# Stability-AI/stable-audio-tools

Measured on AMD Instinct MI355X. Metric: train-step samples/sec (47s@44.1kHz), higher is better.
Workload: dtype f32(bf16x3)

## Files before the change

### include/sat_amd.h

```cpp
#ifndef SAT_AMD_H
#define SAT_AMD_H

#ifdef __cplusplus
extern "C" {
#endif

int sat_abi_version(void);
int sat_is_simulator(void);
const char* sat_last_error(void);


int sat_conv1d(const float* x, const float* w_packed, const float* bias, const float* alpha, const float* beta,
               const float* res, float* y, const float* x2, const float* alpha2, const float* beta2,
               float* part_da, float* part_db, int B, int Cin, int Cout, int Tin, int Tout, int K, int stride,
               int dil, int pad, int tanh_out, void* stream);
int sat_conv1d_partial_rows(int B, int Tout);

int sat_conv1d_bf16x3(const float* x, const short* w_hi, const short* w_lo, const float* bias, const float* snake_a,
                      const float* snake_ib, const float* res, float* y, const float* x2, const float* alpha2,
                      const float* beta2, float* part_da, float* part_db, int B, int Cin, int Cout, int Tin, int Tout,
                      int K, int stride, int dil, int pad, int tanh_out, void* stream);
int sat_conv1d_bf16x3_emit(const float* x, const short* w_hi, const short* w_lo, const float* bias, const float* snake_a,
                      const float* snake_ib, const float* res, float* y, const float* x2, const float* alpha2,
                      const float* beta2, float* part_da, float* part_db, int B, int Cin, int Cout, int Tin, int Tout,
                      int K, int stride, int dil, int pad, int tanh_out, void* em_hi, void* em_lo,
                           const float* em_a, const float* em_ib, int em_rows, void* stream);
int sat_residual_unit_fwd(const short* xp_hi, const short* xp_lo, int rows, const short* w7_hi, const short* w7_lo,
                          const float* bias1, const float* a2, const float* ib2, const short* w1_hi, const short* w1_lo,
                          const float* bias2, const float* x, float* h, float* y, int B, int C, int T, int K, int dil, int pad,
                          void* em_hi, void* em_lo, const float* em_a, const float* em_ib, int em_rows, void* stream);
int sat_convtr1d_bf16x3(const float* x, const short* w_hi, const short* w_lo, const float* bias, const float* snake_a,
                        const float* snake_ib, const float* res, float* y, const float* x2, const float* alpha2,
                        const float* beta2, float* part_da, float* part_db, int B, int Cin, int Cout, int Tin, int Tout,
                        int K, int stride, int pad, int tanh_out, void* stream);
int sat_conv1d_bf16x3_partial_rows(int B, int Tout, int K, int stride);

int sat_rows_pack(const float* x, float* buf, int B, int C, int T, int W, int kh, int dil_t, int pad_t, int pad_w, int pitch, int lead,
                  void* stream);
int sat_rows_pack_bwd(const float* dbuf, float* dx, int B, int C, int T, int W, int kh, int dil_t, int pad_t, int pad_w, int pitch,
                      int lead, void* stream);
int sat_rows_unpack(const float* y, float* out, int B, int C, int T, int W, int pad_w, int pitch, float slope, void* stream);
int sat_rows_unpack_bwd(const float* dout, const float* out, float* dy, int B, int C, int T, int W, int pad_w, int pitch, float slope,
                        void* stream);

int sat_disc_geom(int frames, int W, int* P, int* L, int* lead, int* rows);
int sat_disc_planes(const float* src, const float* out, const signed char* fm_sign, const float* fm_coef, float* dst, void* hi, void* lo, int B,
                    int C, int frames, int W, int pitched, float slope, void* stream);
int sat_disc_l1_blocks(void);
int sat_disc_l1_sum(const float* a, const float* b, float* partial, signed char* sign, long long n, void* stream);
long long sat_disc_pack_size(int Cout, int Cin, int kh, int kw, int mode);
int sat_disc_pack_weights(const float* w, short* wq, int Cout, int Cin, int kh, int kw, int mode, void* stream);
int sat_disc_conv(const void* xp_hi, const void* xp_lo, const void* wq, const float* bias, float* y, void* em_hi,
                  void* em_lo, int B, int Cin, int Cout, int frames, int W, int kh, int kw, int dil_t, float slope, const float* lk_src,
                  float lk_slope, void* stream);
int sat_disc_wgrad_nsplit(int B, int M, int Cin, int kh, int frames, int W);
int sat_disc_wgrad(const float* dy, const float* x, float* partial, int B, int M, int Cin, int frames, int W, int kh, int kw, int dil_t,
                   void* stream);

int sat_conv1d_k7_plane_rows(int Tin, int Tout, int pad);
int sat_conv1d_k7_planes(const float* x, const float* snake_a, const float* snake_ib, short* xp_hi, short* xp_lo, int B, int Cin, int Tin,
                         int rows, void* stream);
long long sat_pack_weights_k7q_size(int D0, int D1, int K, int mode);
int sat_pack_weights_k7q(const float* w, short* hi, short* lo, int D0, int D1, int K, int mode, void* stream);
int sat_conv1d_bf16x3_planesq(const short* xp_hi, const short* xp_lo, int rows, const short* w_hi, const short* w_lo, const float* bias,
                             const float* res, float* y, const float* x2, const float* alpha2, const float* beta2, float* part_da,
                             float* part_db, int B, int Cin, int Cout, int Tin, int Tout, int K, int dil, int pad, int tanh_out,
                             int flags, void* stream);
int sat_convtr1d_bf16x3_partial_rows(int B, int Tout, int stride, int pad);
int sat_pack_weights_bf16x3(const float* w, short* hi, short* lo, int D0, int D1, int K, int stride, int mode, void* stream);
long long sat_pack_weights_bf16x3_size(int D0, int D1, int K, int stride, int mode);
int sat_snake_consts(const float* alpha, const float* beta, float* a, float* ib, int C, void* stream);

int sat_convtr1d(const float* x, const float* w_packed, const float* bias, const float* alpha, const float* beta,
                 const float* res, float* y, const float* x2, const float* alpha2, const float* beta2,
                 float* part_da, float* part_db, int B, int Cin, int Cout, int Tin, int Tout, int K, int stride,
                 int pad, int tanh_out, void* stream);
int sat_convtr1d_partial_rows(int B, int Tout, int stride, int pad);

int sat_conv_wgrad(const float* lo, const float* hi, const float* alpha, const float* beta, int snake_on,
                   float* partial, long long so_m, long long so_n, long long so_k, int B, int M, int N, int Tlo,
                   int Thi, int K, int stride, int dil, int pad, void* stream);
int sat_conv_wgrad_nsplit(int B, int M, int N, int Tlo, int K, int stride, int dil);

int sat_conv_wgrad7_bf16x3(const float* dy, const float* x, const float* alpha, const float* beta, float* partial,
                           long long so_m, long long so_n, long long so_k, int B, int M, int N, int T, int dil, int pad,
                           float* dy_rowsum, void* stream);
int sat_conv_wgrad7_bf16x3_nsplit(int B, int M, int N, int T);
int sat_conv_wgrad7_bf16x3_fuses_rowsum(int B, int M, int N, int T);

int sat_conv_wgrad7_planes_ok(int B, int M, int N, int T, int dil, int pad, int rows_dy, int rows_act);
int sat_conv_wgrad7_planes_nsplit(int B, int M, int N, int T);
int sat_conv_wgrad7_planes(const short* dy_hi, const short* dy_lo, int rows_dy, const short* act_hi, const short* act_lo, int rows_act,
                           float* partial, long long so_m, long long so_n, long long so_k, int B, int M, int N, int T, int dil, int pad,
                           void* stream);
int sat_lds_read_tr16_probe(const short* image, const int* lane_off, short* out, void* stream);

int sat_conv_wgrad_bf16x3(const float* lo, const float* hi, const float* alpha, const float* beta, int snake_on,
                          float* partial, long long so_m, long long so_n, long long so_k, int B, int M, int N, int Tlo,
                          int Thi, int K, int stride, int pad, float* lo_rowsum, void* stream);
int sat_conv_wgrad_bf16x3_nsplit(int B, int M, int N, int Tlo, int K, int stride);

int sat_ru_k1_bwd_nsplit(int B, int C, int T);
int sat_ru_k1_pack(const float* w, short* hi, short* lo, int C, void* stream);
int sat_ru_k1_bwd(const float* dy, const float* h, const short* wt_hi, const short* wt_lo, const float* alpha2, const float* beta2,
                  float* dh, short* em_hi, short* em_lo, int em_rows, float* dw_partial, float* part, int B, int C, int T,
                  void* stream);

int sat_reduce_splits(const float* partial, float* out, long long count, int nsplit, float scale, int accumulate,
                      void* stream);
int sat_rowsum(const float* x, float* partial, int B, int C, int T, void* stream);
int sat_rowsum_nsplit(int T);

int sat_wn_fold(const float* v, const float* g, float* w, float* norm, int D0, int R, void* stream);
int sat_wn_grad(const float* v, const float* g, const float* norm, const float* dw, float* dv, float* dg, int D0,
                int R, void* stream);
int sat_wn_grad_splits(const float* partial, int nsplit, long long count, long long so_m, long long so_n, long long so_k,
                       const float* v, const float* g, const float* norm, float* dv, float* dg, int D0, int N, int K,
                       const float* bias_partial, int bias_cols, float* dbias, void* stream);
int sat_edge_conv_ok(int cin, int cout, int k, int stride, int dil, int pad);
int sat_edge_conv_partial_rows(int B, int T);
int sat_edge_conv(const float* x, const float* w, const float* bias, const float* alpha, const float* beta, float* y, const float* x2,
                  const float* alpha2, const float* beta2, float* part_da, float* part_db, short* em_hi, short* em_lo,
                  const float* em_alpha, const float* em_beta, int em_rows, int B, int Cin, int Cout, int T, int K, int pad, int mode,
                  int tanh_out, void* stream);
int sat_edge_conv_wgrad_nsplit(int B, int M, int N, int T);
int sat_edge_conv_wgrad(const float* dy, const float* x, const float* alpha, const float* beta, float* partial, float* rowsum, int B,
                        int M, int N, int T, int K, int pad, void* stream);
int sat_pack_weights(const float* w, float* out, int D0, int D1, int K, int S, int mode, void* stream);

int sat_vae_nblocks(long long n);
int sat_vae_sample_fwd(const float* pre, const float* noise, float* z, float* kl_partial, int B, int C, int T,
                       void* stream);
int sat_vae_sample_bwd(const float* pre, const float* noise, const float* dz, const float* dkl, float* dpre, int B,
                       int C, int T, void* stream);

int sat_fir(const float* x, const float* taps, float* y, int N, int T, int ntaps, int adjoint, void* stream);
int sat_stft_tiles(int n_fft, int hop, int T);
int sat_stft_fwd(const float* x, const float* y, const float* views, float* partial, int NI, int C, int T, int NV,
                 int n_fft, int hop, void* stream);
int sat_stft_bwd(const float* x, const float* y, const float* views, const float* coef, float* dy, int NI, int C,
                 int T, int NV, int n_fft, int hop, int wrt_x, void* stream);

int sat_adamw_step(float* p, const float* g, float* m, float* v, long long n, float lr, float beta1, float beta2,
                   float eps, float weight_decay, int step, float grad_scale, float* ema, float ema_decay,
                   void* stream);
int sat_adamw_step_dev(float* p, const float* g, float* m, float* v, long long n, const float* hyper, float beta1, float beta2,
                       float eps, float weight_decay, float* ema, void* stream);

int sat_multi_copy(const void* entries, int nent, void* stream);

int sat_allreduce_available(void);
int sat_allreduce_unique_id(void* id128);
int sat_allreduce_init(const void* id128, int world, int rank, void** comm);
int sat_allreduce_bucket(void* comm, void* buf, long long count, int dtype, int mode, void* stream);
int sat_allreduce_finalize(void* comm);

int sat_attn_prepare(const void* src, long long sb, long long sh, long long sn, short* rm_hi, short* rm_lo,
                     short* tr_hi, short* tr_lo, int B, int H, int N, int Np, int dtype, void* stream);
int sat_attention_fwd(const short* q_hi, const short* q_lo, const short* k_hi, const short* k_lo, const short* vt_hi,
                      const short* vt_lo, void* o, float* lse, int B, int H, int Hkv, int Nq, int Nk, int Nqp, int Nkp,
                      int head_dim, float scale, int dtype, void* stream);
int sat_attention_rowdot(const void* dout, const void* out, float* dsum, int B, int H, int Nq, int dtype, void* stream);
int sat_attention_bwd(const short* const* planes, const float* lse, const float* dsum, void* dq, void* dk, void* dv,
                      int B, int H, int Hkv, int Nq, int Nk, int Nqp, int Nkp, int head_dim, float scale, int dtype,
                      void* stream);
int sat_attention_cross_ok(int H, int Hkv, int Nk, int head_dim, int dtype);
int sat_attention_cross_fwd(const short* q_rm, const short* k_rm, const short* v_tr, void* o, float* lse, int B, int H, int Hkv,
                            int Nq, int Nk, int Nqp, int Nkp, int head_dim, float scale, void* stream);
long long sat_attention_cross_bwd_ws(int B, int H, int Hkv, int Nq, int Nk);
int sat_attention_cross_bwd(const short* const* planes, const float* lse, const float* dsum, void* dq, void* dk, void* dv,
                            void* ws, long long ws_bytes, int B, int H, int Hkv, int Nq, int Nk, int Nqp, int Nkp, int head_dim,
                            float scale, void* stream);

int sat_layernorm_fwd(const void* x, const float* gamma, const float* beta, const void* scale, const void* shift,
                      long long mod_stride, void* y, float* mean, float* rstd, int rows, int D, int rows_per_batch,
                      float eps, int dtype, void* stream);
int sat_layernorm_fwd_fp8(const void* x, const float* gamma, const float* beta, const void* scale, const void* shift,
                          long long mod_stride, void* q, float* qscale, int rows, int D, int rows_per_batch, float eps,
                          int dtype, void* stream);
int sat_layernorm_bwd_nblocks(int rows, int rows_per_batch);
int sat_layernorm_bwd(const void* dy, const void* x, const float* gamma, const float* beta, const void* scale,
                      long long mod_stride, const float* mean, const float* rstd, void* dx, float* part, int rows, int D,
                      int rows_per_batch, int dtype, void* stream);
int sat_layernorm_bwd_res(const void* dy, const void* x, const float* gamma, const float* beta, const void* scale,
                          long long mod_stride, const float* mean, const float* rstd, const void* dres, void* dx, float* part,
                          int rows, int D, int rows_per_batch, int dtype, void* stream);

int sat_rope_tables(const float* inv_freq, float* cs, int N, int half, float pos_scale, void* stream);
int sat_rope_apply(void* t, const float* cs, long long sb, long long sn, long long sh, int B, int N, int H, int half,
                   int tab_off, int transpose, int dtype, void* stream);

int sat_qk_norm_fwd(const void* x, long long xs, void* y, long long ys, const float* q_gamma, const float* q_beta,
                    const float* k_gamma, const float* k_beta, const float* cs, int tab_off, float* stat, int tokens, int ntok,
                    int nh, int hq, int mode, float eps, int dtype, void* stream);
int sat_qk_norm_bwd_nblocks(long long rows);
int sat_qk_norm_bwd(void* dy, long long ys, const void* x, long long xs, const float* q_gamma, const float* k_gamma,
                    const float* cs, int tab_off, const float* stat, float* part, int tokens, int ntok, int nh, int hq,
                    int mode, int dtype, void* stream);

int sat_swiglu(const void* xin, const void* dout, void* out, long long rows, int F, int backward, int dtype,
               void* stream);
int sat_gate_residual(const void* x, const void* gate, long long gstride, const void* res, void* y, int B, int N, int D,
                      int dtype, void* stream);
int sat_gate_residual_bwd_nchunks(int N);
int sat_gate_residual_bwd(const void* dy, const void* x, const void* gate, long long gstride, void* dx, float* part,
                          int B, int N, int D, int dtype, void* stream);

int sat_cfg_step(const void* out2, const void* x, void* y0, void* y1, int B, int C, int T, int ncond, float scale,
                 float phi, float c0x, float c0v, float c1x, float c1v, int dtype, void* stream);
int sat_sampler_step(const void* out2, const void* x, const void* prev, void* y0, void* y1, int B, int C, int T, int ncond,
                     float scale, float phi, const float* coef, int dtype, void* stream);
int sat_sampler_step_dev(const void* out2, const void* x, const void* prev, void* y0, void* y1, int B, int C, int T, int ncond,
                         float scale, float phi, const float* coef, int dtype, void* stream);
int sat_spec_frames(int n_fft, int hop, int T);
int sat_spec_fwd(const float* x, float* z, int NI, int C, int T, int n_fft, int hop, void* stream);
int sat_spec_bwd(const float* dz, float* dx, int NI, int C, int T, int n_fft, int hop, void* stream);


int sat_gemm_bf16(const void* A, long long lda, const void* B, long long ldb, void* C, long long ldc, const float* bias,
                  const void* res, long long ldr, const void* gate, long long ldg, int rows_per_gate, void* pre,
                  long long ldp, const void* zeros, int M, int N, int K, int epilogue, int out_f32, int splits, int tile,
                  void* stream);

int sat_gemm_qkv_bf16(const void* A, long long lda, const void* B, long long ldb, const float* rope_cs, int rope_off,
                      void* q_rm, void* k_rm, void* v_tr, const void* zeros, int nb, int ntok, int npad, int heads,
                      int K, int sec0, int nsec, int tile, void* stream);
int sat_gemm_qkv_norm_bf16(const void* A, long long lda, const void* B, long long ldb, const float* rope_cs, int rope_off,
                           void* q_rm, void* k_rm, void* v_tr, const void* zeros, int nb, int ntok, int npad, int heads,
                           int K, int sec0, int nsec, int tile, int mode, const float* q_gamma, const float* q_beta,
                           const float* k_gamma, const float* k_beta, float eps, void* stream);

int sat_splitk_epilogue(const float* slabs, int S, const float* bias, const void* res, long long ldr, void* out, long long ldo,
                        int M, int N, int out_f32, void* stream);

int sat_gemm_fp8(const void* A, long long lda, const void* B, long long ldb, void* C, long long ldc, const float* bias,
                 const void* res, long long ldr, const void* gate, long long ldg, int rows_per_gate, void* pre,
                 long long ldp, const void* zeros, const float* alpha, const float* row_alpha, const float* col_alpha, int M, int N,
                 int K, int epilogue, int out_f32, int tile, void* stream);
int sat_gemm_qkv_fp8(const void* A, long long lda, const void* B, long long ldb, const float* rope_cs, int rope_off,
                     void* q_rm, void* k_rm, void* v_tr, const void* zeros, const float* alpha, const float* row_alpha,
                     const float* col_alpha, int nb, int ntok, int npad, int heads, int K, int sec0, int nsec, int tile, void* stream);
int sat_absmax_scale_blocks(int R, int C);
int sat_absmax_scale(const void* src, long long lds, float* work, float* scales, int R, int C, int src_f32, void* stream);
int sat_quant_fp8(const void* src, long long lds, void* dst, long long ldd, const float* qscale, int R, int C, int src_f32,
                  void* stream);
int sat_quant_fp8_rows(const void* src, long long lds, void* dst, long long ldd, float* scale, int R, int C, int src_f32,
                       void* stream);

int sat_cast_bf16(const void* src, long long lds, void* dst, long long ldd, int R, int C, int Rpad, int src_f32,
                  int transpose, void* stream);
int sat_cast_bf16_tpair(const void* src_a, long long lds_a, void* dst_a, long long ldd_a, int Ra, int Ca, int Rpad_a, int a_f32,
                        const void* src_b, long long lds_b, void* dst_b, long long ldd_b, int Rb, int Cb, int Rpad_b, int b_f32,
                        void* stream);
int sat_cast_bf16_dual(const void* src, long long lds, void* dst, long long ldd, void* dst_t, long long ldd_t, int R, int C, int Rpad,
                       int src_f32, void* stream);

int sat_split_bf16x3(const float* src, long long lds, void* dst, long long ldd, int R, int C, int side, void* stream);

#ifdef __cplusplus
}
#endif
#endif
```

### stable_audio_tools_amd/_lib.py

```python
import ctypes
import os

_P = ctypes.c_void_p
_I = ctypes.c_int
_L = ctypes.c_longlong
_F = ctypes.c_float

SIGNATURES = {
    "sat_abi_version": (_I, []),
    "sat_is_simulator": (_I, []),
    "sat_last_error": (ctypes.c_char_p, []),
    "sat_conv1d": (_I, [_P] * 12 + [_I] * 10 + [_P]),
    "sat_conv1d_partial_rows": (_I, [_I, _I]),
    "sat_conv1d_bf16x3": (_I, [_P] * 13 + [_I] * 10 + [_P]),
    "sat_conv1d_bf16x3_emit": (_I, [_P] * 13 + [_I] * 10 + [_P] * 4 + [_I, _P]),
    "sat_convtr1d_bf16x3": (_I, [_P] * 13 + [_I] * 9 + [_P]),
    "sat_conv1d_bf16x3_partial_rows": (_I, [_I] * 4),
    "sat_rows_pack": (_I, [_P, _P] + [_I] * 10 + [_P]),
    "sat_rows_pack_bwd": (_I, [_P, _P] + [_I] * 10 + [_P]),
    "sat_rows_unpack": (_I, [_P, _P] + [_I] * 6 + [_F, _P]),
    "sat_rows_unpack_bwd": (_I, [_P, _P, _P] + [_I] * 6 + [_F, _P]),
    "sat_disc_geom": (_I, [_I, _I, _P, _P, _P, _P]),
    "sat_disc_planes": (_I, [_P] * 7 + [_I] * 5 + [_F, _P]),
    "sat_disc_l1_blocks": (_I, []),
    "sat_disc_l1_sum": (_I, [_P, _P, _P, _P, _L, _P]),
    "sat_disc_pack_size": (_L, [_I] * 5),
    "sat_disc_pack_weights": (_I, [_P] * 2 + [_I] * 5 + [_P]),
    "sat_disc_conv": (_I, [_P] * 7 + [_I] * 8 + [_F, _P, _F, _P]),
    "sat_disc_wgrad_nsplit": (_I, [_I] * 6),
    "sat_disc_wgrad": (_I, [_P] * 3 + [_I] * 8 + [_P]),
    "sat_conv1d_k7_plane_rows": (_I, [_I] * 3),
    "sat_conv1d_k7_planes": (_I, [_P] * 5 + [_I] * 4 + [_P]),
    "sat_conv1d_bf16x3_planesq": (_I, [_P, _P, _I] + [_P] * 10 + [_I] * 10 + [_P]),
    "sat_pack_weights_k7q": (_I, [_P, _P, _P, _I, _I, _I, _I, _P]),
    "sat_residual_unit_fwd": (_I, [_P, _P, _I] + [_P] * 11 + [_I] * 6 + [_P] * 4 + [_I, _P]),
    "sat_pack_weights_k7q_size": (_L, [_I, _I, _I, _I]),
    "sat_convtr1d_bf16x3_partial_rows": (_I, [_I] * 4),
    "sat_pack_weights_bf16x3": (_I, [_P, _P, _P, _I, _I, _I, _I, _I, _P]),
    "sat_pack_weights_bf16x3_size": (_L, [_I, _I, _I, _I, _I]),
    "sat_snake_consts": (_I, [_P, _P, _P, _P, _I, _P]),
    "sat_conv_wgrad7_bf16x3": (_I, [_P] * 5 + [_L] * 3 + [_I] * 6 + [_P, _P]),
    "sat_conv_wgrad7_bf16x3_nsplit": (_I, [_I] * 4),
    "sat_conv_wgrad7_bf16x3_fuses_rowsum": (_I, [_I] * 4),
    "sat_conv_wgrad7_planes_ok": (_I, [_I] * 8),
    "sat_conv_wgrad7_planes_nsplit": (_I, [_I] * 4),
    "sat_conv_wgrad7_planes": (_I, [_P, _P, _I, _P, _P, _I, _P] + [_L] * 3 + [_I] * 6 + [_P]),
    "sat_lds_read_tr16_probe": (_I, [_P] * 4),
    "sat_conv_wgrad_bf16x3": (_I, [_P] * 4 + [_I, _P] + [_L] * 3 + [_I] * 8 + [_P, _P]),
    "sat_conv_wgrad_bf16x3_nsplit": (_I, [_I] * 6),
    "sat_convtr1d": (_I, [_P] * 12 + [_I] * 9 + [_P]),
    "sat_convtr1d_partial_rows": (_I, [_I, _I, _I, _I]),
    "sat_conv_wgrad": (_I, [_P, _P, _P, _P, _I, _P, _L, _L, _L] + [_I] * 9 + [_P]),
    "sat_conv_wgrad_nsplit": (_I, [_I] * 7),
    "sat_reduce_splits": (_I, [_P, _P, _L, _I, _F, _I, _P]),
    "sat_ru_k1_bwd_nsplit": (_I, [_I] * 3),
    "sat_ru_k1_pack": (_I, [_P, _P, _P, _I, _P]),
    "sat_ru_k1_bwd": (_I, [_P] * 9 + [_I, _P, _P, _I, _I, _I, _P]),
    "sat_rowsum": (_I, [_P, _P, _I, _I, _I, _P]),
    "sat_rowsum_nsplit": (_I, [_I]),
    "sat_wn_fold": (_I, [_P, _P, _P, _P, _I, _I, _P]),
    "sat_wn_grad": (_I, [_P, _P, _P, _P, _P, _P, _I, _I, _P]),
    "sat_wn_grad_splits": (_I, [_P, _I, _L, _L, _L, _L, _P, _P, _P, _P, _P, _I, _I, _I, _P, _I, _P, _P]),
    "sat_pack_weights": (_I, [_P, _P, _I, _I, _I, _I, _I, _P]),
    "sat_vae_nblocks": (_I, [_L]),
    "sat_vae_sample_fwd": (_I, [_P, _P, _P, _P, _I, _I, _I, _P]),
    "sat_vae_sample_bwd": (_I, [_P, _P, _P, _P, _P, _I, _I, _I, _P]),
    "sat_multi_copy": (_I, [_P, _I, _P]),
    "sat_adamw_step": (_I, [_P, _P, _P, _P, _L, _F, _F, _F, _F, _F, _I, _F, _P, _F, _P]),
    "sat_adamw_step_dev": (_I, [_P, _P, _P, _P, _L, _P, _F, _F, _F, _F, _P, _P]),
    "sat_allreduce_available": (_I, []),
    "sat_allreduce_unique_id": (_I, [_P]),
    "sat_allreduce_init": (_I, [_P, _I, _I, _P]),
    "sat_allreduce_bucket": (_I, [_P, _P, _L, _I, _I, _P]),
    "sat_allreduce_finalize": (_I, [_P]),
    "sat_fir": (_I, [_P, _P, _P, _I, _I, _I, _I, _P]),
    "sat_stft_tiles": (_I, [_I, _I, _I]),
    "sat_stft_fwd": (_I, [_P, _P, _P, _P, _I, _I, _I, _I, _I, _I, _P]),
    "sat_stft_bwd": (_I, [_P, _P, _P, _P, _P, _I, _I, _I, _I, _I, _I, _I, _P]),
    "sat_spec_frames": (_I, [_I, _I, _I]),
    "sat_spec_fwd": (_I, [_P, _P, _I, _I, _I, _I, _I, _P]),
    "sat_spec_bwd": (_I, [_P, _P, _I, _I, _I, _I, _I, _P]),
    "sat_attn_prepare": (_I, [_P, _L, _L, _L, _P, _P, _P, _P, _I, _I, _I, _I, _I, _P]),
    "sat_attention_fwd": (_I, [_P] * 8 + [_I] * 8 + [_F, _I, _P]),
    "sat_attention_rowdot": (_I, [_P, _P, _P, _I, _I, _I, _I, _P]),
    "sat_attention_bwd": (_I, [_P] * 6 + [_I] * 8 + [_F, _I, _P]),
    "sat_edge_conv_ok": (_I, [_I] * 6),
    "sat_edge_conv_partial_rows": (_I, [_I] * 2),
    "sat_edge_conv": (_I, [_P] * 15 + [_I] * 9 + [_P]),
    "sat_edge_conv_wgrad_nsplit": (_I, [_I] * 4),
    "sat_edge_conv_wgrad": (_I, [_P] * 6 + [_I] * 6 + [_P]),
    "sat_attention_cross_ok": (_I, [_I] * 5),
    "sat_attention_cross_fwd": (_I, [_P] * 5 + [_I] * 8 + [_F, _P]),
    "sat_attention_cross_bwd_ws": (_L, [_I] * 5),
    "sat_attention_cross_bwd": (_I, [_P] * 7 + [_L] + [_I] * 8 + [_F, _P]),
    "sat_gemm_bf16": (_I, [_P, _L, _P, _L, _P, _L, _P, _P, _L, _P, _L, _I, _P, _L, _P] + [_I] * 7 + [_P]),
    "sat_gemm_qkv_bf16": (_I, [_P, _L, _P, _L, _P, _I, _P, _P, _P, _P] + [_I] * 8 + [_P]),
    "sat_gemm_qkv_norm_bf16": (_I, [_P, _L, _P, _L, _P, _I, _P, _P, _P, _P] + [_I] * 9 + [_P] * 4 + [_F, _P]),
    "sat_gemm_fp8": (_I, [_P, _L, _P, _L, _P, _L, _P, _P, _L, _P, _L, _I, _P, _L, _P, _P, _P, _P] + [_I] * 6 + [_P]),
    "sat_gemm_qkv_fp8": (_I, [_P, _L, _P, _L, _P, _I, _P, _P, _P, _P, _P, _P, _P] + [_I] * 8 + [_P]),
    "sat_quant_fp8": (_I, [_P, _L, _P, _L, _P, _I, _I, _I, _P]),
    "sat_quant_fp8_rows": (_I, [_P, _L, _P, _L, _P, _I, _I, _I, _P]),
    "sat_absmax_scale": (_I, [_P, _L, _P, _P, _I, _I, _I, _P]),
    "sat_absmax_scale_blocks": (_I, [_I, _I]),
    "sat_splitk_epilogue": (_I, [_P, _I, _P, _P, _L, _P, _L, _I, _I, _I, _P]),
    "sat_cast_bf16": (_I, [_P, _L, _P, _L, _I, _I, _I, _I, _I, _P]),
    "sat_cast_bf16_tpair": (_I, [_P, _L, _P, _L, _I, _I, _I, _I, _P, _L, _P, _L, _I, _I, _I, _I, _P]),
    "sat_cast_bf16_dual": (_I, [_P, _L, _P, _L, _P, _L, _I, _I, _I, _I, _P]),
    "sat_split_bf16x3": (_I, [_P, _L, _P, _L, _I, _I, _I, _P]),
    "sat_layernorm_fwd": (_I, [_P] * 5 + [_L] + [_P] * 3 + [_I] * 3 + [_F, _I, _P]),
    "sat_layernorm_fwd_fp8": (_I, [_P] * 5 + [_L] + [_P] * 2 + [_I] * 3 + [_F, _I, _P]),
    "sat_layernorm_bwd_nblocks": (_I, [_I, _I]),
    "sat_layernorm_bwd": (_I, [_P] * 5 + [_L] + [_P] * 4 + [_I] * 4 + [_P]),
    "sat_layernorm_bwd_res": (_I, [_P] * 5 + [_L] + [_P] * 5 + [_I] * 4 + [_P]),
    "sat_rope_tables": (_I, [_P, _P, _I, _I, _F, _P]),
    "sat_rope_apply": (_I, [_P, _P, _L, _L, _L] + [_I] * 7 + [_P]),
    "sat_qk_norm_fwd": (_I, [_P, _L, _P, _L, _P, _P, _P, _P, _P, _I, _P] + [_I] * 5 + [_F, _I, _P]),
    "sat_qk_norm_bwd_nblocks": (_I, [_L]),
    "sat_qk_norm_bwd": (_I, [_P, _L, _P, _L, _P, _P, _P, _I, _P, _P] + [_I] * 6 + [_P]),
    "sat_swiglu": (_I, [_P, _P, _P, _L, _I, _I, _I, _P]),
    "sat_gate_residual": (_I, [_P, _P, _L, _P, _P, _I, _I, _I, _I, _P]),
    "sat_gate_residual_bwd_nchunks": (_I, [_I]),
    "sat_cfg_step": (_I, [_P, _P, _P, _P, _I, _I, _I, _I, _F, _F, _F, _F, _F, _F, _I, _P]),
    "sat_sampler_step": (_I, [_P, _P, _P, _P, _P, _I, _I, _I, _I, _F, _F, _P, _I, _P]),
    "sat_sampler_step_dev": (_I, [_P, _P, _P, _P, _P, _I, _I, _I, _I, _F, _F, _P, _I, _P]),
    "sat_gate_residual_bwd": (_I, [_P, _P, _P, _L, _P, _P, _I, _I, _I, _I, _P]),
}

LIB_PATH = os.path.join(os.path.dirname(os.path.abspath(__file__)), "csrc", "libsat_amd.so")


def bind(cdll):
    for name, (res, args) in SIGNATURES.items():
        fn = getattr(cdll, name)
        fn.restype = res
        fn.argtypes = args
    return cdll


_lib = None


def load():
    global _lib
    if _lib is not None:
        return _lib
    if not os.path.exists(LIB_PATH):
        raise RuntimeError(
            f"stable_audio_tools_amd: HIP library not built: {LIB_PATH} is missing. "
            "Run `python -c 'import __graft_entry__ as g; g.build()'` (hipcc --offload-arch=gfx950). "
            "There is no CPU fallback.")
    try:
        cdll = ctypes.CDLL(LIB_PATH)
    except OSError as e:
        raise RuntimeError(f"stable_audio_tools_amd: cannot load {LIB_PATH}: {e}. There is no CPU fallback.") from e
    bind(cdll)
    if cdll.sat_is_simulator():
        raise RuntimeError("stable_audio_tools_amd: refusing to use a simulator build as the product library")
    _lib = cdll
    return _lib
```

### stable_audio_tools_amd/autoencoders.py

```python
import copy
import math

import torch
from torch import nn
from torch.nn.utils.weight_norm import WeightNorm as _TorchWeightNorm

from . import functional as Fn
from .bottleneck import VAEBottleneck


class SnakeBeta(nn.Module):

    def __init__(self, in_features, alpha=1.0, alpha_trainable=True, alpha_logscale=True):
        super().__init__()
        if not alpha_logscale:
            raise NotImplementedError("only alpha_logscale=True (the reference default used by Oobleck) is implemented")
        self.in_features = in_features
        self.alpha_logscale = alpha_logscale
        self.alpha = nn.Parameter(torch.zeros(in_features) * alpha)
        self.beta = nn.Parameter(torch.zeros(in_features) * alpha)
        self.alpha.requires_grad = alpha_trainable
        self.beta.requires_grad = alpha_trainable
        self.no_div_by_zero = 0.000000001

    def forward(self, x):
        c = x.shape[1]
        eye = torch.eye(c, device=x.device, dtype=x.dtype).unsqueeze(-1)
        a, b = (self.alpha, self.beta) if self.alpha.dtype == torch.float32 else (self.alpha.detach().float(), self.beta.detach().float())
        return Fn.SnakeConv1dFn.apply(x, a, b, eye, None, None, 1, 1, 0, False)


class _NativeWeightNorm(_TorchWeightNorm):

    def __init__(self, name="weight", dim=0):
        super().__init__(name, dim)

    def compute_weight(self, module):
        return module._fold_host()

    def remove(self, module):
        if not module.is_folded:
            module._to_folded(module._fold_host().detach())

    def __call__(self, module, inputs):
        return None


def _inference_pass(*tensors):
    return (not torch.is_grad_enabled()) or not any(t is not None and t.requires_grad for t in tensors)


class _WNConvBase(nn.Module):

    transposed = False

    def __init__(self, in_channels, out_channels, kernel_size, stride=1, padding=0, dilation=1, bias=True):
        super().__init__()
        self.in_channels, self.out_channels = in_channels, out_channels
        self.kernel_size, self.stride, self.padding, self.dilation = kernel_size, stride, padding, dilation
        if self.transposed:
            wshape = (in_channels, out_channels, kernel_size)
        else:
            wshape = (out_channels, in_channels, kernel_size)
        v = torch.empty(wshape)
        nn.init.kaiming_uniform_(v, a=math.sqrt(5))
        self.weight_g = nn.Parameter(v.flatten(1).norm(dim=1).view(-1, 1, 1).clone())
        self.weight_v = nn.Parameter(v)
        if bias:
            fan_in = wshape[1] * kernel_size
            bound = 1.0 / math.sqrt(fan_in)
            self.bias = nn.Parameter(torch.empty(out_channels).uniform_(-bound, bound))
        else:
            self.register_parameter("bias", None)
        self.register_forward_pre_hook(_NativeWeightNorm("weight", 0))
        self.__dict__["_derived"] = Fn.DerivedCache()

    @property
    def is_folded(self):
        return "weight" in self._parameters

    def __getattr__(self, name):
        if name == "weight" and "weight_v" in self.__dict__.get("_parameters", ()):
            return self._fold_host()
        return super().__getattr__(name)

    def __deepcopy__(self, memo):
        cls = self.__class__
        new = cls.__new__(cls)
        memo[id(self)] = new
        for k, v in self.__dict__.items():
            new.__dict__[k] = Fn.DerivedCache() if k == "_derived" else copy.deepcopy(v, memo)
        return new

    def _fold_host(self):
        v, g = self._parameters["weight_v"], self._parameters["weight_g"]
        return v * (g / v.flatten(1).norm(dim=1).view(-1, 1, 1))

    def _to_folded(self, w):
        rg = self._parameters["weight_v"].requires_grad
        del self._parameters["weight_g"], self._parameters["weight_v"]
        self._parameters["weight"] = nn.Parameter(w.clone(), requires_grad=rg)

    def _load_from_state_dict(self, state_dict, prefix, local_metadata, strict, missing_keys, unexpected_keys, error_msgs):
        kw, kg, kv = prefix + "weight", prefix + "weight_g", prefix + "weight_v"
        if not self.is_folded and kw in state_dict and kv not in state_dict:
            self._to_folded(torch.empty_like(self._parameters["weight_v"]))
        elif self.is_folded and kw not in state_dict and kv in state_dict and kg in state_dict:
            v, g = state_dict.pop(kv), state_dict.pop(kg)
            state_dict[kw] = v * (g / v.flatten(1).norm(dim=1).view(-1, 1, 1))
        super()._load_from_state_dict(state_dict, prefix, local_metadata, strict, missing_keys, unexpected_keys, error_msgs)

    def p32(self, name, t):
        if t is None or t.dtype == torch.float32:
            return t
        if t.requires_grad and torch.is_grad_enabled():
            raise NotImplementedError("16-bit parameters are inference-only on the HIP conv stack (freeze the model: AutoencoderPretransform does)")
        return self._derived.get("f32/" + name, (t,), lambda: t.detach().float())

    def bias32(self):
        return self.p32("bias", self.bias)

    def folded_weight(self):
        if self.is_folded:
            return self.p32("weight", self._parameters["weight"])
        v, g = self.p32("weight_v", self.weight_v), self.p32("weight_g", self.weight_g)
        if _inference_pass(v, g):
            return self._derived.get("folded", (v, g), lambda: Fn.WeightNormFn.apply(v.detach(), g.detach()))
        return Fn.WeightNormFn.apply(v, g)

    def weight_args(self):
        if not self.is_folded and Fn._ops(None).wn_fused:
            v, g = self.p32("weight_v", self.weight_v), self.p32("weight_g", self.weight_g)
            if not _inference_pass(v, g):
                return v, g
        return self.folded_weight(), None

    def derived_cache(self, *others):
        ps = list(self._parameters.values()) + list(others)
        return self._derived if _inference_pass(*ps) else None


class WNConv1d(_WNConvBase):
    def forward(self, x, snake=None, res=None, tanh_out=False, next_snake=None):
        a, b = (self.p32("alpha", snake.alpha), self.p32("beta", snake.beta)) if snake is not None else (None, None)
        if next_snake is not None and next_snake[0].dtype != torch.float32:
            next_snake = (self.p32("next_alpha", next_snake[0]), self.p32("next_beta", next_snake[1]), next_snake[2])
        w, g = self.weight_args()
        return Fn.SnakeConv1dFn.apply(x, a, b, w, self.bias32(), res, self.stride, self.dilation,
                                      self.padding, tanh_out, None, self.derived_cache(a, b), next_snake, g)


class WNConvTranspose1d(_WNConvBase):
    transposed = True

    def forward(self, x, snake=None):
        a, b = (self.p32("alpha", snake.alpha), self.p32("beta", snake.beta)) if snake is not None else (None, None)
        w, g = self.weight_args()
        return Fn.SnakeConvTr1dFn.apply(x, a, b, w, self.bias32(), self.stride, self.padding, None,
                                        self.derived_cache(a, b), g)


def _require_snake(use_snake, antialias_activation=False):
    if not use_snake:
        raise NotImplementedError("only use_snake=True (SnakeBeta, the Stable Audio Open / 2.0 VAE configuration) is "
                                  "implemented on the HIP path; the ELU variant is out of scope (SURVEY.md §8a V3)")
    if antialias_activation:
        raise NotImplementedError("antialias_activation (alias_free_torch) is out of scope")


class ResidualUnit(nn.Module):
    checkpointing = False
    fuse = None

    def __init__(self, in_channels, out_channels, dilation, use_snake=False, antialias_activation=False):
        super().__init__()
        _require_snake(use_snake, antialias_activation)
        self.dilation = dilation
        padding = (dilation * (7 - 1)) // 2
        self.layers = nn.Sequential(
            SnakeBeta(out_channels),
            WNConv1d(in_channels, out_channels, kernel_size=7, dilation=dilation, padding=padding),
            SnakeBeta(out_channels),
            WNConv1d(out_channels, out_channels, kernel_size=1),
        )

    def entry_snake(self):
        s1 = self.layers[0]
        return (s1.alpha, s1.beta, self.dilation)

    def forward(self, x, next_snake=None):
        s1, c1, s2, c2 = self.layers
        ca, cb = c1.derived_cache(s1.alpha, s1.beta), c2.derived_cache(s2.alpha, s2.beta)
        if next_snake is not None and next_snake[0].dtype != torch.float32:
            next_snake = (c2.p32("next_alpha", next_snake[0]), c2.p32("next_beta", next_snake[1]), next_snake[2])
        (w1, g1), (w2, g2) = c1.weight_args(), c2.weight_args()
        return Fn.ResidualUnitFn.apply(x, c1.p32("alpha", s1.alpha), c1.p32("beta", s1.beta), w1, c1.bias32(),
                                       c2.p32("alpha", s2.alpha), c2.p32("beta", s2.beta), w2, c2.bias32(), self.dilation, None,
                                       self.checkpointing and torch.is_grad_enabled(), (ca, cb) if ca is not None and cb is not None else None,
                                       next_snake, self.fuse if self.fuse is not None else ("nokeep" if not torch.is_grad_enabled() else False),
                                       g1, g2)


class EncoderBlock(nn.Module):
    def __init__(self, in_channels, out_channels, stride, use_snake=False, antialias_activation=False):
        super().__init__()
        _require_snake(use_snake, antialias_activation)
        self.layers = nn.Sequential(
            ResidualUnit(in_channels, in_channels, dilation=1, use_snake=use_snake),
            ResidualUnit(in_channels, in_channels, dilation=3, use_snake=use_snake),
            ResidualUnit(in_channels, in_channels, dilation=9, use_snake=use_snake),
            SnakeBeta(in_channels),
            WNConv1d(in_channels, out_channels, kernel_size=2 * stride, stride=stride, padding=math.ceil(stride / 2)),
        )

    def forward(self, x, next_snake=None):
        r1, r2, r3, snake, down = self.layers
        x = r1(x, next_snake=r2.entry_snake())
        x = r2(x, next_snake=r3.entry_snake())
        return down(r3(x), snake=snake, next_snake=next_snake)


class DecoderBlock(nn.Module):
    def __init__(self, in_channels, out_channels, stride, use_snake=False, antialias_activation=False,
                 use_nearest_upsample=False):
        super().__init__()
        _require_snake(use_snake, antialias_activation)
        if use_nearest_upsample:
            raise NotImplementedError("use_nearest_upsample is out of scope (no in-repo Oobleck config enables it)")
        self.layers = nn.Sequential(
            SnakeBeta(in_channels),
            WNConvTranspose1d(in_channels, out_channels, kernel_size=2 * stride, stride=stride,
                              padding=math.ceil(stride / 2)),
            ResidualUnit(out_channels, out_channels, dilation=1, use_snake=use_snake),
            ResidualUnit(out_channels, out_channels, dilation=3, use_snake=use_snake),
            ResidualUnit(out_channels, out_channels, dilation=9, use_snake=use_snake),
        )

    def forward(self, x):
        snake, up, r1, r2, r3 = self.layers
        x = r1(up(x, snake=snake), next_snake=r2.entry_snake())
        return r3(r2(x, next_snake=r3.entry_snake()))


class OobleckEncoder(nn.Module):
    def __init__(self, in_channels=2, channels=128, latent_dim=32, c_mults=[1, 2, 4, 8], strides=[2, 4, 8, 8],
                 use_snake=False, antialias_activation=False):
        super().__init__()
        _require_snake(use_snake, antialias_activation)
        self.in_channels = in_channels
        c_mults = [1] + list(c_mults)
        self.depth = len(c_mults)
        layers = [WNConv1d(in_channels, c_mults[0] * channels, kernel_size=7, padding=3)]
        for i in range(self.depth - 1):
            layers += [EncoderBlock(c_mults[i] * channels, c_mults[i + 1] * channels, stride=strides[i], use_snake=use_snake)]
        layers += [SnakeBeta(c_mults[-1] * channels),
                   WNConv1d(c_mults[-1] * channels, latent_dim, kernel_size=3, padding=1)]
        self.layers = nn.Sequential(*layers)

    def forward(self, x):
        mods = list(self.layers)
        blocks = mods[1:-2]
        x = mods[0](x, next_snake=blocks[0].layers[0].entry_snake() if blocks else None)
        for i, blk in enumerate(blocks):
            nxt = blocks[i + 1].layers[0].entry_snake() if i + 1 < len(blocks) else None
            x = blk(x, next_snake=nxt)
        return mods[-1](x, snake=mods[-2])


class OobleckDecoder(nn.Module):
    def __init__(self, out_channels=2, channels=128, latent_dim=32, c_mults=[1, 2, 4, 8], strides=[2, 4, 8, 8],
                 use_snake=False, antialias_activation=False, use_nearest_upsample=False, final_tanh=True):
        super().__init__()
        _require_snake(use_snake, antialias_activation)
        self.out_channels = out_channels
        c_mults = [1] + list(c_mults)
        self.depth = len(c_mults)
        layers = [WNConv1d(latent_dim, c_mults[-1] * channels, kernel_size=7, padding=3)]
        for i in range(self.depth - 1, 0, -1):
            layers += [DecoderBlock(c_mults[i] * channels, c_mults[i - 1] * channels, stride=strides[i - 1],
                                    use_snake=use_snake, antialias_activation=antialias_activation,
                                    use_nearest_upsample=use_nearest_upsample)]
        layers += [SnakeBeta(c_mults[0] * channels),
                   WNConv1d(c_mults[0] * channels, out_channels, kernel_size=7, padding=3, bias=False),
                   nn.Tanh() if final_tanh else nn.Identity()]
        self.final_tanh = final_tanh
        self.layers = nn.Sequential(*layers)

    def forward(self, x):
        mods = list(self.layers)
        x = mods[0](x)
        for blk in mods[1:-3]:
            x = blk(x)
        return mods[-2](x, snake=mods[-3], tanh_out=self.final_tanh)


class AudioAutoencoder(nn.Module):

    def __init__(self, encoder, decoder, latent_dim, downsampling_ratio, sample_rate, io_channels=2, bottleneck=None,
                 pretransform=None, in_channels=None, out_channels=None, soft_clip=False):
        super().__init__()
        if pretransform is not None:
            raise NotImplementedError("AudioAutoencoder(pretransform=...) is out of scope for the HIP path")
        self.downsampling_ratio = downsampling_ratio
        self.sample_rate = sample_rate
        self.latent_dim = latent_dim
        self.io_channels = io_channels
        self.in_channels = io_channels if in_channels is None else in_channels
        self.out_channels = io_channels if out_channels is None else out_channels
        self.min_length = self.downsampling_ratio
        self.bottleneck = bottleneck
        self.encoder = encoder
        self.decoder = decoder
        self.pretransform = None
        self.soft_clip = soft_clip
        self.is_discrete = self.bottleneck is not None and self.bottleneck.is_discrete

    def encode(self, audio, skip_bottleneck=False, return_info=False, skip_pretransform=False, iterate_batch=False, **kwargs):
        info = {}
        if iterate_batch:
            latents = torch.cat([self.encoder(audio[i:i + 1]) for i in range(audio.shape[0])], dim=0)
        else:
            latents = self.encoder(audio)
        info["pre_bottleneck_latents"] = latents
        if self.bottleneck is not None and not skip_bottleneck:
            latents, binfo = self.bottleneck.encode(latents, return_info=True, **kwargs)
            info.update(binfo)
        if return_info:
            return latents, info
        return latents

    def decode(self, latents, skip_bottleneck=False, iterate_batch=False, **kwargs):
        if self.bottleneck is not None and not skip_bottleneck:
            latents = self.bottleneck.decode(latents)
        if iterate_batch:
            decoded = torch.cat([self.decoder(latents[i:i + 1]) for i in range(latents.shape[0])], dim=0)
        else:
            decoded = self.decoder(latents, **kwargs)
        if self.soft_clip:
            decoded = torch.tanh(decoded)
        return decoded

    def encode_audio(self, audio, chunked=False, overlap=32, chunk_size=128, **kwargs):
        if not chunked:
            return self.encode(audio, **kwargs)
        r = int(self.downsampling_ratio)
        total = audio.shape[2]
        csz, hop = chunk_size * r, (chunk_size - overlap) * r
        starts = list(range(0, total - csz + 1, hop))
        if not starts:
            raise ValueError("chunked encode needs at least chunk_size latent frames of audio")
        if starts[-1] + csz != total:
            starts.append(total - csz)
        y_size = total // r
        out = torch.zeros((audio.shape[0], self.latent_dim, y_size), device=audio.device, dtype=audio.dtype)
        half = overlap // 2
        chunk_noise = kwargs.pop("noise", None)
        if isinstance(chunk_noise, (list, tuple)) and len(chunk_noise) != len(starts):
            raise ValueError(f"chunked encode: {len(starts)} chunks but {len(chunk_noise)} noise tensors")
        for i, s0 in enumerate(starts):
            if chunk_noise is not None:
                kwargs["noise"] = chunk_noise[i] if isinstance(chunk_noise, (list, tuple)) else chunk_noise
            y = self.encode(audio[:, :, s0:s0 + csz], **kwargs)
            last = i == len(starts) - 1
            t1 = y_size if last else i * hop // r + chunk_size
            t0 = t1 - y.shape[2] if last else i * hop // r
            k0, k1 = 0, y.shape[2]
            if i > 0:
                t0, k0 = t0 + half, k0 + half
            if not last:
                t1, k1 = t1 - half, k1 - half
            out[:, :, t0:t1] = y[:, :, k0:k1]
        return out

    def decode_audio(self, latents, chunked=False, overlap=32, chunk_size=128, **kwargs):
        if not chunked:
            return self.decode(latents, **kwargs)
        r = int(self.downsampling_ratio)
        out = torch.zeros((latents.shape[0], self.out_channels, latents.shape[2] * r), device=latents.device,
                          dtype=latents.dtype)
        for win in _chunk_windows(latents.shape[2], chunk_size, overlap):
            y = self.decode(latents[:, :, win.src0:win.src1])
            out[:, :, win.dst0 * r:win.dst1 * r] = y[:, :, win.keep0 * r:win.keep1 * r]
        return out


class _Win:
    __slots__ = ("src0", "src1", "dst0", "dst1", "keep0", "keep1")


def _chunk_windows(total, chunk, overlap):
    hop = chunk - overlap
    starts = list(range(0, total - chunk + 1, hop))
    if not starts:
        raise ValueError("chunked encode/decode needs at least chunk_size latent frames")
    if starts[-1] + chunk != total:
        starts.append(total - chunk)
    half = overlap // 2
    wins = []
    for n, s0 in enumerate(starts):
        w = _Win()
        last = n == len(starts) - 1
        w.src0, w.src1 = s0, s0 + chunk
        d0 = (total - chunk) if last else n * hop
        w.keep0 = half if n > 0 else 0
        w.keep1 = chunk if last else chunk - half
        w.dst0, w.dst1 = d0 + w.keep0, d0 + w.keep1
        wins.append(w)
    return wins


def create_encoder_from_config(cfg):
    if cfg.get("type") != "oobleck":
        raise NotImplementedError(f"encoder type {cfg.get('type')!r} is out of scope (only 'oobleck' is on the hot path)")
    enc = OobleckEncoder(**cfg["config"])
    if not cfg.get("requires_grad", True):
        for p in enc.parameters():
            p.requires_grad = False
    return enc


def create_decoder_from_config(cfg):
    if cfg.get("type") != "oobleck":
        raise NotImplementedError(f"decoder type {cfg.get('type')!r} is out of scope (only 'oobleck' is on the hot path)")
    dec = OobleckDecoder(**cfg["config"])
    if not cfg.get("requires_grad", True):
        for p in dec.parameters():
            p.requires_grad = False
    return dec


def create_autoencoder_from_config(config):
    ae = config["model"]
    if ae.get("pretransform") is not None:
        raise NotImplementedError("autoencoder-level pretransform is out of scope")
    encoder = create_encoder_from_config(ae["encoder"])
    decoder = create_decoder_from_config(ae["decoder"])
    bottleneck = None
    if ae.get("bottleneck") is not None:
        if ae["bottleneck"]["type"] != "vae":
# ... 7 lines not shown
```

### stable_audio_tools_amd/csrc/conv1d_bf16x3.hip

```cpp
#include "conv_common.h"
#include <type_traits>

#define SAT_K7P_LEAD_ROWS 32
#define SAT_BF_AROWS1 192
#define SAT_BF_AROWSN 136

struct SatConvBfLaunch {
    SatConvParams p;
    const short* w_hi;
    const short* w_lo;
    int cout_pad;
    int cin_v, cout_v;
    int sin_log2;
    int sout_log2;
    int in_shift, out_shift;
    int nq;
    const short* xp_hi = nullptr;
    const short* xp_lo = nullptr;
    int xp_rows = 0, xp_c8 = 0;
    int wq = 0;
    int stagger = 0;
    int persist = 0;
    int dma_in_mfma = 0;
    short* em_hi = nullptr;
    short* em_lo = nullptr;
    const float* em_a = nullptr;
    const float* em_ib = nullptr;
    int em_rows = 0, em_c8 = 0;
    const short* ru_w1_hi = nullptr;
    const short* ru_w1_lo = nullptr;
    const float* ru_bias2 = nullptr;
    const float* ru_a2 = nullptr;
    const float* ru_ib2 = nullptr;
    float* ru_h = nullptr;
};

SAT_DEVICE void sat_split2(float x, short* hi, short* lo) {
    const short h = sat_f32_to_bf16(x);
    *hi = h;
    *lo = sat_f32_to_bf16(x - sat_bf16_to_f32(h));
}

template <int NG, int CS, bool GATHER>
__global__ void __launch_bounds__(256)
#if !defined(SAT_HIPEMU)
__attribute__((amdgpu_waves_per_eu(NG == 4 ? 3 : 2)))
#endif
sat_conv1d_bf16x3_kernel(SatConvBfLaunch a) {
    constexpr int KT = NG / CS;
    constexpr int KROW = NG * 8 + 8;
    constexpr int AROWS = (CS == 1) ? SAT_BF_AROWS1 : SAT_BF_AROWSN;
    constexpr int WPS = 4 / CS;
    constexpr int NU = (CS == 1) ? 1 : 128 / (64 * WPS);
    const SatConvParams& p = a.p;
    constexpr int W_BYTES = 2 * SAT_CO_T * KROW * 2, A_BYTES = 2 * CS * AROWS * 8 * 2, T_BYTES = 4 * 32 * 68 * 4;
    constexpr int POOL = (W_BYTES + A_BYTES) > T_BYTES ? (W_BYTES + A_BYTES) : T_BYTES;
    __shared__ __attribute__((aligned(16))) char lds_pool[POOL];
    short (*w_lds)[SAT_CO_T][KROW] = reinterpret_cast<short (*)[SAT_CO_T][KROW]>(lds_pool);
    short (*a_lds)[CS][AROWS][8] = reinterpret_cast<short (*)[CS][AROWS][8]>(lds_pool + W_BYTES);
    __shared__ float red_lds[2][2][SAT_CO_T];
    __shared__ float ep_lds[5][SAT_CO_T];
    constexpr int SN_MAX = (NG == 4) ? 1024 : 2048;
    __shared__ float sn_lds[2][SN_MAX];

    const int tid = threadIdx.x;
    const int lane = tid & 63, wave = tid >> 6;
    const int l31 = lane & 31, hi = lane >> 5;
    int co_tile, win;
    sat_xcd_tile(blockIdx.x + gridDim.x * (blockIdx.y + gridDim.y * blockIdx.z), gridDim.y, gridDim.x * gridDim.z, &co_tile, &win);
    const int b = win / (int)gridDim.x, t_tile = win - b * (int)gridDim.x;
    const int t0 = t_tile * SAT_T_T;
    const int co0 = co_tile * SAT_CO_T;
    const int co_w = (wave >> 1) * 64, t_w = (wave & 1) * 64;
    const int K = p.K, dil = p.dil;
    const int nrows = SAT_T_T + (K - 1) * dil;
    const int q_in0 = t0 - p.pad;
    const int si = GATHER ? a.sin_log2 : 0, so = a.sout_log2;
    const int smask_i = (1 << si) - 1, smask_o = (1 << so) - 1;
    const float* xb = p.x + (size_t)b * p.Cin * p.Tin;
    const bool wave_on = (co0 + co_w) < a.cout_v;
    const bool mi1_on = (co0 + co_w + 32) < a.cout_v;
    const bool has_snake = p.alpha != nullptr;

    f32x16 acc[2][2];
#pragma unroll
    for (int i = 0; i < 2; ++i)
#pragma unroll
        for (int j = 0; j < 2; ++j)
#pragma unroll
            for (int r = 0; r < 16; ++r) acc[i][j][r] = 0.0f;

    if (tid < SAT_CO_T) {
        const int m = co0 + tid;
        const bool ok = m < a.cout_v;
        const int co = m >> so;
        ep_lds[0][tid] = (ok && p.bias) ? p.bias[co] : 0.0f;
        ep_lds[1][tid] = (ok && p.x2) ? expf(p.alpha2[co]) : 1.0f;
        ep_lds[2][tid] = (ok && p.x2) ? expf(p.beta2[co]) : 1.0f;
        ep_lds[3][tid] = (ok && a.em_a) ? a.em_a[co] : 0.0f;
        ep_lds[4][tid] = (ok && a.em_a) ? a.em_ib[co] : 0.0f;
    }
    if (has_snake) {
        const int nsn = p.Cin < SN_MAX ? p.Cin : SN_MAX;
        for (int i = tid; i < nsn; i += 256) {
            sn_lds[0][i] = p.alpha[i];
            sn_lds[1][i] = p.beta[i];
        }
    }
    __syncthreads();

    const int nchunks = (a.cin_v + 8 * CS - 1) / (8 * CS);
    const int cs_w = SAT_UNIFORM(wave / WPS);
    const int row0 = (wave % WPS) * 64 + lane;
    const int nhalo = (CS > 1) ? (nrows - SAT_T_T) * 8 : 0;
    const bool halo_on = (CS > 1) && (wave % WPS) == 0 && lane < nhalo;
    const int h_row = SAT_T_T + (lane >> 3), h_e = lane & 7;
    constexpr bool DEEP = (NG == 8 && CS == 4);
    constexpr int NSET = DEEP ? 2 : 1;
    float av[NSET][NU][8];
    float hv[NSET];
    bf16x8 wv[NG];
#pragma unroll
    for (int s_ = 0; s_ < NSET; ++s_) hv[s_] = 0.0f;
    auto load_elem = [&](int v, int row, bool* okp) -> float {
        int ch = v >> si;
        ch = ch < p.Cin ? ch : p.Cin - 1;
        const int tin = ((q_in0 + row) << si) + (v & smask_i) - (GATHER ? a.in_shift : 0);
        const bool ok = (unsigned)tin < (unsigned)p.Tin;
        *okp = ok;
        return xb[(size_t)ch * p.Tin + (ok ? tin : 0)];
    };
    unsigned okm[NSET];
#pragma unroll
    for (int s_ = 0; s_ < NSET; ++s_) okm[s_] = 0u;
    auto issue_loads = [&](int c, auto set_c) {
        constexpr int ST = decltype(set_c)::value;
        const int v0 = (c * CS + cs_w) * 8;
        unsigned m = 0u;
#pragma unroll
        for (int u = 0; u < NU; ++u) {
            const int row = row0 + u * 64 * WPS;
            if (CS == 1 && row >= nrows) continue;
#pragma unroll
            for (int e = 0; e < 8; ++e) {
                bool ok;
                av[ST][u][e] = load_elem(v0 + e, row, &ok);
                m |= ok ? (1u << (u * 8 + e)) : 0u;
            }
        }
        static_assert(NU * 8 < 31, "the in-range flags of a staging set are one 32-bit mask (bit 31: the halo element)");
        if (CS > 1 && halo_on) {
            bool ok;
            hv[ST] = load_elem(v0 + h_e, h_row, &ok);
            m |= ok ? (1u << 31) : 0u;
        }
        okm[ST] = m;
    };
    auto issue_w = [&](int c) {
#pragma unroll
        for (int u = 0; u < NG; ++u) {
            const int idx = tid + u * 256;
            const int part = idx % NG, co = (idx / NG) & 127, pl = idx / (NG * 128);
            const short* src = (pl ? a.w_lo : a.w_hi) + (((size_t)c * a.cout_pad + co0 + co) * NG + part) * 8;
            wv[u] = *reinterpret_cast<const bf16x8*>(src);
        }
    };
    auto write_lds = [&](int c, auto set_c) {
        constexpr int ST = decltype(set_c)::value;
        const int v0 = (c * CS + cs_w) * 8;
        float sa[8], sib[8];
        if (has_snake) {
#pragma unroll
            for (int e = 0; e < 8; ++e) {
                int ch = (v0 + e) >> si;
                ch = ch < p.Cin ? ch : p.Cin - 1;
                sa[e] = sn_lds[0][ch];
                sib[e] = sn_lds[1][ch];
            }
        }
#pragma unroll
        for (int u = 0; u < NU; ++u) {
            const int row = row0 + u * 64 * WPS;
            if (CS == 1 && row >= nrows) continue;
            uint32_t ph[4], pl[4];
#pragma unroll
            for (int e = 0; e < 8; e += 2) {
                float o0 = (okm[ST] >> (u * 8 + e)) & 1u ? av[ST][u][e] : 0.0f, o1 = (okm[ST] >> (u * 8 + e + 1)) & 1u ? av[ST][u][e + 1] : 0.0f;
                if (has_snake) {
                    o0 = sat_snake(o0, sa[e], sib[e]);
                    o1 = sat_snake(o1, sa[e + 1], sib[e + 1]);
                }
                sat_split2_pk(o0, o1, &ph[e >> 1], &pl[e >> 1]);
            }
            *reinterpret_cast<u32x4*>(&a_lds[0][cs_w][row][0]) = u32x4{ph[0], ph[1], ph[2], ph[3]};
            *reinterpret_cast<u32x4*>(&a_lds[1][cs_w][row][0]) = u32x4{pl[0], pl[1], pl[2], pl[3]};
// ... 288 lines not shown
#pragma unroll
                for (int ni = 0; ni < 2; ++ni) {
                    const int q = t0 + t_w + ni * 32 + l31;
                    const int t = (q << so) + (m & smask_o) - a.out_shift;
                    const bool ok = m_ok && t >= 0 && t < p.Tout;
                    okb |= ok ? (1u << (2 * r + ni)) : 0u;
                    const size_t o = ((size_t)b * p.Cout + (ok ? co : 0)) * p.Tout + (ok ? t : 0);
                    xv[r][ni] = bwd ? p.x2[o] : 0.0f;
                    rv[r][ni] = p.res ? p.res[o] : 0.0f;
                }
            }
#pragma unroll
            for (int r = 0; r < 16; ++r) {
                const int col = co_w + mi * 32 + (r & 3) + 8 * (r >> 2) + 4 * hi;
                const int m = co0 + col;
                const int co = m >> so;
                const float bias = ep_lds[0][col];
                const float a2 = ep_lds[1][col], b2 = ep_lds[2][col];
                float pda = 0.f, pdb = 0.f;
#pragma unroll
                for (int ni = 0; ni < 2; ++ni) {
                    const int q = t0 + t_w + ni * 32 + l31;
                    const int t = (q << so) + (m & smask_o) - a.out_shift;
                    const bool ok = (okb >> (2 * r + ni)) & 1u;
                    float v = acc[mi][ni][r] + bias;
                    if (bwd) {
                        const SatSnakeGrad g = sat_snake_grad(xv[r][ni], a2, b2);
                        pda += ok ? v * g.dla : 0.0f;
                        pdb += ok ? v * g.dlb : 0.0f;
                        v *= g.dx;
                    }
                    v += rv[r][ni];
                    if (p.tanh_out) v = tanhf(v);
                    if (ok) p.y[((size_t)b * p.Cout + co) * p.Tout + t] = v;
                }
                if (bwd) {
                    pda = sat_half_sum(pda);
                    pdb = sat_half_sum(pdb);
                    if (l31 == 0) {
                        red_lds[0][wave & 1][col] = pda;
                        red_lds[1][wave & 1][col] = pdb;
                    }
                }
            }
        }
    }
    if (bwd) {
        __syncthreads();
        const int m = co0 + tid;
        if (tid < SAT_CO_T && (tid & smask_o) == 0 && m < a.cout_v) {
            float sa = 0.f, sb = 0.f;
            for (int r = 0; r <= smask_o; ++r) {
                sa += red_lds[0][0][tid + r] + red_lds[0][1][tid + r];
                sb += red_lds[1][0][tid + r] + red_lds[1][1][tid + r];
            }
            const size_t row = (size_t)b * gridDim.x + t_tile;
            const size_t nrows_p = (size_t)p.B * gridDim.x;
            p.part_da[(size_t)(m >> so) * nrows_p + row] = sa;
            p.part_db[(size_t)(m >> so) * nrows_p + row] = sb;
        }
    }
}

struct SatBfPlan { int ng, cs, kv; };
static bool sat_bf_plan(int K, int stride, int mode, SatBfPlan* pl) {
    if (mode == 2 || stride > 1) {
        if (K != 2 * stride || (stride & (stride - 1)) || stride > 64) return false;
        *pl = SatBfPlan{8, 4, 2};
        return true;
    }
    if (stride != 1 || K < 1 || K > 8) return false;
    if (K == 1) *pl = SatBfPlan{4, 4, 1};
    else if (K == 2) *pl = SatBfPlan{8, 4, K};
    else if (K <= 4) *pl = SatBfPlan{8, 2, K};
    else *pl = SatBfPlan{8, 1, K};
    return true;
}
static int sat_log2i(int s) { int l = 0; while ((1 << l) < s) ++l; return l; }

struct SatPackBfParams {
    const float* w;
    short* hi;
    short* lo;
    int D0, D1, K, S, mode, ng, cs, kv, m_v, v_v, out_pad;
    long long total;
};
__global__ void __launch_bounds__(256) sat_pack_bf16x3_kernel(SatPackBfParams p) {
    const long long o = (long long)blockIdx.x * 256 + threadIdx.x;
    if (o >= p.total) return;
    const int e = (int)(o & 7);
    long long q = o >> 3;
    const int g = (int)(q % p.ng);
    q /= p.ng;
    const int m = (int)(q % p.out_pad), chunk = (int)(q / p.out_pad);
    const int kt = p.ng / p.cs;
    const int v = (chunk * p.cs + g / kt) * 8 + e, tap = g % kt;
    float val = 0.0f;
    if (tap < p.kv && m < p.m_v && v < p.v_v) {
        if (p.mode == 0) val = p.w[((size_t)m * p.D1 + v / p.S) * p.K + tap * p.S + v % p.S];
        else if (p.mode == 1) val = p.w[((size_t)v * p.D1 + m) * p.K + (p.K - 1 - tap)];
        else val = p.w[((size_t)v * p.D1 + m / p.S) * p.K + (m % p.S) + (tap == 0 ? p.S : 0)];
    }
    short h, l;
    sat_split2(val, &h, &l);
    p.hi[o] = h;
    p.lo[o] = l;
}

static bool sat_pack_bf_geometry(int D0, int D1, int K, int stride, int mode, SatPackBfParams* p) {
    SatBfPlan pl;
    if (mode < 0 || mode > 2 || D0 <= 0 || D1 <= 0 || !sat_bf_plan(K, stride, mode, &pl)) return false;
    if (mode == 1 && stride != 1) return false;
    p->D0 = D0; p->D1 = D1; p->K = K; p->S = stride; p->mode = mode;
    p->ng = pl.ng; p->cs = pl.cs; p->kv = pl.kv;
    if (mode == 0) { p->m_v = D0; p->v_v = D1 * stride; }
    else if (mode == 1) { p->m_v = D1; p->v_v = D0; }
    else { p->m_v = D1 * stride; p->v_v = D0; }
    p->out_pad = sat_cdiv(p->m_v, SAT_CO_T) * SAT_CO_T;
    p->total = (long long)sat_cdiv(p->v_v, 8 * pl.cs) * p->out_pad * pl.ng * 8;
    return true;
}
extern "C" long long sat_pack_weights_bf16x3_size(int D0, int D1, int K, int stride, int mode) {
    SatPackBfParams p{};
    return sat_pack_bf_geometry(D0, D1, K, stride, mode, &p) ? p.total : -1;
}
extern "C" int sat_pack_weights_bf16x3(const float* w, short* hi, short* lo, int D0, int D1, int K, int stride, int mode, void* stream) {
    SatPackBfParams p{};
    if (!sat_pack_bf_geometry(D0, D1, K, stride, mode, &p)) {
        sat_set_error("sat_pack_weights_bf16x3: needs stride 1 with K <= 8, or K == 2*stride with a power-of-two stride; mode 0|1|2");
        return 1;
    }
    p.w = w; p.hi = hi; p.lo = lo;
    SAT_LAUNCH(sat_pack_bf16x3_kernel, dim3((unsigned)sat_cdivll(p.total, 256)), dim3(256), stream, p);
    return sat_check_launch("sat_pack_weights_bf16x3");
}

struct SatSnakeConstParams { const float* alpha; const float* beta; float* a; float* ib; int C; };
__global__ void __launch_bounds__(256) sat_snake_consts_kernel(SatSnakeConstParams p) {
    const int i = blockIdx.x * 256 + threadIdx.x;
    if (i >= p.C) return;
    p.a[i] = expf(p.alpha[i]);
    p.ib[i] = 1.0f / (expf(p.beta[i]) + 1e-9f);
}
extern "C" int sat_snake_consts(const float* alpha, const float* beta, float* a, float* ib, int C, void* stream) {
    if (C <= 0) { sat_set_error("sat_snake_consts: empty"); return 1; }
    SatSnakeConstParams p{alpha, beta, a, ib, C};
    SAT_LAUNCH(sat_snake_consts_kernel, dim3(sat_cdiv(C, 256)), dim3(256), stream, p);
    return sat_check_launch("sat_snake_consts");
}

#include "conv1d_bf16x3_k7.h"
#include "conv1d_planes.h"
#include "conv1d_bf16x3_k7q.h"

static int sat_bf_launch(const char* what, SatConvBfLaunch& a, const SatBfPlan& pl, void* stream) {
    if (pl.ng == 8 && pl.cs == 1 && a.sin_log2 == 0 && a.sout_log2 == 0) {
        if (a.xp_hi && a.wq) sat_bf_launch_k7q(a, stream);
        else sat_bf_launch_k7(a, stream);
        return sat_check_launch(what);
    }
    if (a.p.alpha && a.p.Cin > ((pl.ng == 4) ? 1024 : 2048)) {
        sat_set_error("conv1d_bf16x3: an activated input of more than 2048 channels (1024 for K <= 4 at stride 1) is not served by the bf16x3 kernels (ops.use_bf16x3 = False takes the fp32-MFMA ones)");
        return 1;
    }
    dim3 grid(sat_cdiv(a.nq, SAT_T_T), a.cout_pad / SAT_CO_T, a.p.B);
    if (a.sin_log2 > 0) { SAT_LAUNCH((sat_conv1d_bf16x3_kernel<8, 4, true>), grid, dim3(256), stream, a); }
    else if (pl.ng == 8 && pl.cs == 1) { SAT_LAUNCH((sat_conv1d_bf16x3_kernel<8, 1, false>), grid, dim3(256), stream, a); }
    else if (pl.ng == 8 && pl.cs == 2) { SAT_LAUNCH((sat_conv1d_bf16x3_kernel<8, 2, false>), grid, dim3(256), stream, a); }
    else if (pl.ng == 8 && pl.cs == 4) { SAT_LAUNCH((sat_conv1d_bf16x3_kernel<8, 4, false>), grid, dim3(256), stream, a); }
    else { SAT_LAUNCH((sat_conv1d_bf16x3_kernel<4, 4, false>), grid, dim3(256), stream, a); }
    return sat_check_launch(what);
}

static int sat_conv1d_bf16x3_impl(const char* what, const float* x, const short* w_hi, const short* w_lo, const float* bias,
                                  const float* snake_a, const float* snake_ib, const float* res, float* y,
                                  const float* x2, const float* alpha2, const float* beta2, float* part_da,
                                  float* part_db, int B, int Cin, int Cout, int Tin, int Tout, int K, int stride, int dil,
                                  int pad, int tanh_out, short* em_hi, short* em_lo, const float* em_a, const float* em_ib, int em_rows,
                                  void* stream) {
    if (B <= 0 || Cin <= 0 || Cout <= 0 || Tin <= 0 || Tout <= 0) { sat_set_error("sat_conv1d_bf16x3: empty shape"); return 1; }
    SatBfPlan pl;
    if (!sat_bf_plan(K, stride, 0, &pl) || dil < 1 || (stride > 1 && dil != 1)) {
        sat_set_error("sat_conv1d_bf16x3: needs stride 1 with K <= 8, or K == 2*stride (power-of-two stride, dilation 1)");
        return 1;
    }
    if ((pl.kv - 1) * dil > (pl.cs == 1 ? 62 : SAT_BF_AROWSN - SAT_T_T)) { sat_set_error("sat_conv1d_bf16x3: receptive field too large for the LDS slab"); return 1; }
    if ((snake_a == nullptr) != (snake_ib == nullptr)) { sat_set_error("sat_conv1d_bf16x3: snake constants must both be given"); return 1; }
    if (x2 && (!alpha2 || !beta2 || !part_da || !part_db)) { sat_set_error("sat_conv1d_bf16x3: backward epilogue needs alpha2/beta2/partials"); return 1; }
    SatConvBfLaunch a;
    a.p = SatConvParams{x, nullptr, bias, snake_a, snake_ib, res, y, x2, alpha2, beta2, part_da, part_db,
                        B, Cin, Cout, Tin, Tout, pl.kv, 1, dil, stride == 1 ? pad : 0, tanh_out};
    a.w_hi = w_hi;
    a.w_lo = w_lo;
    a.cout_v = Cout;
    a.cout_pad = sat_cdiv(Cout, SAT_CO_T) * SAT_CO_T;
    a.cin_v = Cin * stride;
    a.sin_log2 = sat_log2i(stride);
    a.sout_log2 = 0;
    a.in_shift = stride == 1 ? 0 : pad;
    a.out_shift = 0;
    a.nq = Tout;
    if (em_hi) {
        const bool generic = !(pl.ng == 8 && pl.cs == 1);
        const bool vec4 = (Tout & 3) == 0 && (((uintptr_t)y | (uintptr_t)x2 | (uintptr_t)res) & 15) == 0;
        if (!generic || !vec4 || !em_lo || (em_a == nullptr) != (em_ib == nullptr) || em_rows < SAT_K7P_LEAD_ROWS + Tout ||
            (((uintptr_t)em_hi | (uintptr_t)em_lo) & 15)) {
            sat_set_error("sat_conv1d_bf16x3_emit: emission needs K <= 4 or a strided conv, Tout % 4 == 0, 16-byte aligned tensors, rows >= 32 + Tout");
            return 1;
        }
        a.em_hi = em_hi; a.em_lo = em_lo; a.em_a = em_a; a.em_ib = em_ib; a.em_rows = em_rows; a.em_c8 = sat_cdiv(Cout, 8);
    }
    return sat_bf_launch(what, a, pl, stream);
}
extern "C" int sat_conv1d_bf16x3(const float* x, const short* w_hi, const short* w_lo, const float* bias,
                                 const float* snake_a, const float* snake_ib, const float* res, float* y,
                                 const float* x2, const float* alpha2, const float* beta2, float* part_da,
                                 float* part_db, int B, int Cin, int Cout, int Tin, int Tout, int K, int stride, int dil,
                                 int pad, int tanh_out, void* stream) {
    return sat_conv1d_bf16x3_impl("sat_conv1d_bf16x3", x, w_hi, w_lo, bias, snake_a, snake_ib, res, y, x2, alpha2, beta2, part_da, part_db,
                                  B, Cin, Cout, Tin, Tout, K, stride, dil, pad, tanh_out, nullptr, nullptr, nullptr, nullptr, 0, stream);
}
extern "C" int sat_conv1d_bf16x3_emit(const float* x, const short* w_hi, const short* w_lo, const float* bias,
                                      const float* snake_a, const float* snake_ib, const float* res, float* y,
                                      const float* x2, const float* alpha2, const float* beta2, float* part_da,
                                      float* part_db, int B, int Cin, int Cout, int Tin, int Tout, int K, int stride, int dil,
                                      int pad, int tanh_out, void* em_hi, void* em_lo, const float* em_a, const float* em_ib, int em_rows,
                                      void* stream) {
    if (!em_hi) { sat_set_error("sat_conv1d_bf16x3_emit: planes missing"); return 1; }
    return sat_conv1d_bf16x3_impl("sat_conv1d_bf16x3_emit", x, w_hi, w_lo, bias, snake_a, snake_ib, res, y, x2, alpha2, beta2, part_da, part_db,
                                  B, Cin, Cout, Tin, Tout, K, stride, dil, pad, tanh_out, (short*)em_hi, (short*)em_lo, em_a, em_ib, em_rows, stream);
}

extern "C" int sat_conv1d_k7_plane_rows(int Tin, int Tout, int pad) {
    if (Tin <= 0 || Tout <= 0 || pad < 0 || pad > SAT_K7P_LEAD) return -1;
    const int need = sat_cdiv(Tout, SAT_K7_T) * SAT_K7_T - pad + SAT_K7_AROWS;
    const int body = need > Tin ? need : Tin;
    return SAT_K7P_LEAD + sat_cdiv(body, 64) * 64;
}
extern "C" int sat_conv1d_k7_planes(const float* x, const float* snake_a, const float* snake_ib, short* xp_hi, short* xp_lo, int B,
                                    int Cin, int Tin, int rows, void* stream) {
    if (B <= 0 || Cin <= 0 || Tin <= 0 || rows < SAT_K7P_LEAD + Tin) { sat_set_error("sat_conv1d_k7_planes: bad shape"); return 1; }
    if ((snake_a == nullptr) != (snake_ib == nullptr)) { sat_set_error("sat_conv1d_k7_planes: snake constants must both be given"); return 1; }
    SatK7PlaneParams p{x, snake_a, snake_ib, xp_hi, xp_lo, B, Cin, Tin, rows, sat_cdiv(Cin, 8)};
    SAT_LAUNCH(sat_k7_planes_kernel, dim3(sat_cdiv(rows, 256), p.c8, B), dim3(256), stream, p);
    return sat_check_launch("sat_conv1d_k7_planes");
}
extern "C" int sat_conv1d_bf16x3_planesq(const short* xp_hi, const short* xp_lo, int rows, const short* w_hi, const short* w_lo,
                                         const float* bias, const float* res, float* y, const float* x2, const float* alpha2,
                                         const float* beta2, float* part_da, float* part_db, int B, int Cin, int Cout, int Tin, int Tout,
                                         int K, int dil, int pad, int tanh_out, int flags, void* stream) {
    if (B <= 0 || Cin <= 0 || Cout <= 0 || Tin <= 0 || Tout <= 0) { sat_set_error("sat_conv1d_bf16x3_planesq: empty shape"); return 1; }
    if (K < 5 || K > SAT_K7Q_TAPS || dil < 1 || (K - 1) * dil > 62) {
        sat_set_error("sat_conv1d_bf16x3_planesq: needs stride 1, 5 <= K <= 7, (K-1)*dil <= 62");
        return 1;
    }
    if (rows < sat_conv1d_k7_plane_rows(Tin, Tout, pad)) { sat_set_error("sat_conv1d_bf16x3_planesq: rows must be >= sat_conv1d_k7_plane_rows(Tin, Tout, pad)"); return 1; }
    if (x2 && (!alpha2 || !beta2 || !part_da || !part_db)) { sat_set_error("sat_conv1d_bf16x3_planesq: backward epilogue needs alpha2/beta2/partials"); return 1; }
    SatConvBfLaunch a;
    a.p = SatConvParams{nullptr, nullptr, bias, nullptr, nullptr, res, y, x2, alpha2, beta2, part_da, part_db,
                        B, Cin, Cout, Tin, Tout, K, 1, dil, pad, tanh_out};
    a.w_hi = w_hi;
    a.w_lo = w_lo;
    a.cout_v = Cout;
    a.cout_pad = sat_cdiv(Cout, SAT_CO_T) * SAT_CO_T;
    a.cin_v = Cin;
    a.sin_log2 = 0;
    a.sout_log2 = 0;
    a.in_shift = 0;
    a.out_shift = 0;
    a.nq = Tout;
    a.xp_hi = xp_hi;
    a.xp_lo = xp_lo;
    a.xp_rows = rows;
    a.xp_c8 = sat_cdiv(Cin, 8);
    a.wq = 1;
    a.dma_in_mfma = (flags & 4) ? 1 : 0;
    a.persist = (flags & 1) ? 0 : ((flags & 2) ? 2 : 1);
    SatBfPlan pl{8, 1, K};
    return sat_bf_launch("sat_conv1d_bf16x3_planesq", a, pl, stream);
}

extern "C" int sat_residual_unit_fwd(const short* xp_hi, const short* xp_lo, int rows, const short* w7_hi, const short* w7_lo,
                                     const float* bias1, const float* a2, const float* ib2, const short* w1_hi, const short* w1_lo,
                                     const float* bias2, const float* x, float* h, float* y, int B, int C, int T, int K, int dil, int pad,
                                     void* em_hi, void* em_lo, const float* em_a, const float* em_ib, int em_rows, void* stream) {
    if (B <= 0 || C <= 0 || T <= 0 || C > SAT_K7_CO) { sat_set_error("sat_residual_unit_fwd: needs 1 <= C <= 128"); return 1; }
    if (K < 5 || K > SAT_K7Q_TAPS || dil < 1 || (K - 1) * dil > 62 || 2 * pad != (K - 1) * dil) {
        sat_set_error("sat_residual_unit_fwd: needs 5 <= K <= 7, (K-1)*dil <= 62, 'same' padding");
        return 1;
    }
    if (rows < sat_conv1d_k7_plane_rows(T, T, pad)) { sat_set_error("sat_residual_unit_fwd: rows must be >= sat_conv1d_k7_plane_rows(T, T, pad)"); return 1; }
    if (!xp_hi || !xp_lo || !w7_hi || !w7_lo || !w1_hi || !w1_lo || !a2 || !ib2 || !x || !y) { sat_set_error("sat_residual_unit_fwd: missing operand"); return 1; }
    if ((T & 3) || (((uintptr_t)y | (uintptr_t)x) & 15)) { sat_set_error("sat_residual_unit_fwd: T % 4 == 0 and 16-byte aligned x / y"); return 1; }
    SatConvBfLaunch a;
    a.p = SatConvParams{nullptr, nullptr, bias1, nullptr, nullptr, x, y, nullptr, nullptr, nullptr, nullptr, nullptr,
                        B, C, C, T, T, K, 1, dil, pad, 0};
    a.w_hi = w7_hi;
    a.w_lo = w7_lo;
    a.cout_v = C;
    a.cout_pad = SAT_CO_T;
    a.cin_v = C;
    a.sin_log2 = 0; a.sout_log2 = 0; a.in_shift = 0; a.out_shift = 0;
    a.nq = T;
    a.xp_hi = xp_hi; a.xp_lo = xp_lo; a.xp_rows = rows; a.xp_c8 = sat_cdiv(C, 8);
    a.wq = 1;
    a.ru_w1_hi = w1_hi; a.ru_w1_lo = w1_lo; a.ru_bias2 = bias2; a.ru_a2 = a2; a.ru_ib2 = ib2; a.ru_h = h;
// ... 47 lines not shown
```

### stable_audio_tools_amd/csrc/elementwise.hip

```cpp
#include "sat_device.h"

#include <string.h>

static thread_local char g_sat_err[512] = "";
void sat_set_error(const char* msg) {
    strncpy(g_sat_err, msg, sizeof(g_sat_err) - 1);
    g_sat_err[sizeof(g_sat_err) - 1] = 0;
}
int sat_check_launch(const char* what) {
    const auto e = hipGetLastError();
    if (e != hipSuccess) {
        char buf[512];
        snprintf(buf, sizeof(buf), "%s: kernel launch failed: %s", what, hipGetErrorString(e));
        sat_set_error(buf);
        return 2;
    }
    return 0;
}
extern "C" const char* sat_last_error() { return g_sat_err; }
#if defined(SAT_HIPEMU)
static int g_sat_emu_cus = 256;
extern "C" void sat_emu_set_cu_count(int n) { g_sat_emu_cus = n > 0 ? n : 256; }
#endif
int sat_cu_count() {
#if defined(SAT_HIPEMU)
    return g_sat_emu_cus;
#else
    static thread_local int dev_cached = -1, cus = 0;
    int dev = 0;
    if (hipGetDevice(&dev) != hipSuccess) return 256;
    if (dev != dev_cached) {
        int n = 0;
        if (hipDeviceGetAttribute(&n, hipDeviceAttributeMultiprocessorCount, dev) != hipSuccess || n <= 0) n = 256;
        cus = n;
        dev_cached = dev;
    }
    return cus;
#endif
}

extern "C" int sat_abi_version() { return 1; }
extern "C" int sat_is_simulator() {
#if defined(SAT_HIPEMU)
    return 1;
#else
    return 0;
#endif
}

struct SatWnParams {
    const float* v;
    const float* g;
    const float* dw;
    float* w;
    float* norm;
    float* dg;
    int D0, R;
};

SAT_DEVICE float sat_block_sum_256(float s, float* red) {
    s = sat_wave_sum(s);
    __syncthreads();
    if ((threadIdx.x & 63) == 0) red[threadIdx.x >> 6] = s;
    __syncthreads();
    return red[0] + red[1] + red[2] + red[3];
}

__global__ void __launch_bounds__(256) sat_wn_fold_kernel(SatWnParams p) {
    __shared__ float red[4];
    const int d = blockIdx.x;
    const float* v = p.v + (size_t)d * p.R;
    float s = 0.f;
    for (int i = threadIdx.x; i < p.R; i += 256) s += v[i] * v[i];
    s = sat_block_sum_256(s, red);
    const float nrm = sqrtf(s);
    const float sc = p.g[d] / nrm;
    float* w = p.w + (size_t)d * p.R;
    for (int i = threadIdx.x; i < p.R; i += 256) w[i] = v[i] * sc;
    if (threadIdx.x == 0) p.norm[d] = nrm;
}

__global__ void __launch_bounds__(256) sat_wn_grad_kernel(SatWnParams p) {
    __shared__ float red[4];
    const int d = blockIdx.x;
    const float* v = p.v + (size_t)d * p.R;
    const float* dw = p.dw + (size_t)d * p.R;
    float s = 0.f;
    for (int i = threadIdx.x; i < p.R; i += 256) s += v[i] * dw[i];
    s = sat_block_sum_256(s, red);
    const float nrm = p.norm[d];
    const float g = p.g[d];
    const float dgv = s / nrm;
    const float c1 = g / nrm, c2 = g * s / (nrm * nrm * nrm);
    float* dv = p.w + (size_t)d * p.R;
    for (int i = threadIdx.x; i < p.R; i += 256) dv[i] = c1 * dw[i] - c2 * v[i];
    if (threadIdx.x == 0) p.dg[d] = dgv;
}

#define SAT_WN_ROW_CAP 16384
struct SatWnSplitParams {
    const float* partial;
    const float* v;
    const float* g;
    const float* norm;
    float* dv;
    float* dg;
    long long count, so_m, so_n, so_k;
    int nsplit, D0, N, K;
    const float* bias_partial;
    float* dbias;
    int bias_cols;
};
#define SAT_WN_THREADS 1024
SAT_DEVICE float sat_wn_slab_sum(const float* base, long long count, int z0, int zstep, int nsplit) {
    float s0 = 0.f, s1 = 0.f, s2 = 0.f, s3 = 0.f;
    int z = z0;
    for (; z + 3 * zstep < nsplit; z += 4 * zstep) {
        s0 += base[(size_t)z * count];
        s1 += base[(size_t)(z + zstep) * count];
        s2 += base[(size_t)(z + 2 * zstep) * count];
        s3 += base[(size_t)(z + 3 * zstep) * count];
    }
    for (; z < nsplit; z += zstep) s0 += base[(size_t)z * count];
    return (s0 + s1) + (s2 + s3);
}
SAT_DEVICE f32x4 sat_wn_slab_sum4(const float* base, long long count, int z0, int zstep, int nsplit) {
    const f32x4 zero = {0.f, 0.f, 0.f, 0.f};
    f32x4 s[8] = {zero, zero, zero, zero, zero, zero, zero, zero};
    int z = z0;
    for (; z + 7 * zstep < nsplit; z += 8 * zstep) {
#pragma unroll
        for (int u = 0; u < 8; ++u) s[u] += *reinterpret_cast<const f32x4*>(base + (size_t)(z + u * zstep) * count);
    }
    for (; z < nsplit; z += zstep) s[0] += *reinterpret_cast<const f32x4*>(base + (size_t)z * count);
    return ((s[0] + s[1]) + (s[2] + s[3])) + ((s[4] + s[5]) + (s[6] + s[7]));
}
SAT_DEVICE float sat_block_sum_1024(float s, float* red) {
    s = sat_wave_sum(s);
    __syncthreads();
    if ((threadIdx.x & 63) == 0) red[threadIdx.x >> 6] = s;
    __syncthreads();
    float t = 0.f;
#pragma unroll
    for (int w = 0; w < SAT_WN_THREADS / 64; ++w) t += red[w];
    return t;
}
__global__ void __launch_bounds__(SAT_WN_THREADS) sat_wn_grad_splits_kernel(SatWnSplitParams p) {
    __shared__ float row[SAT_WN_ROW_CAP];
    __shared__ float red[SAT_WN_THREADS / 64];
    const int d = blockIdx.x;
    const int R = p.N * p.K;
    const float* base = p.partial + (size_t)d * p.so_m;
    const float* v = p.v + (size_t)d * R;
    const bool staged = R <= SAT_WN_ROW_CAP;
    const bool tap_major = p.so_n == 1 && p.K > 1;
    const bool torch_order = p.so_k == 1 && p.so_n == p.K;
    const bool vec = ((p.count | p.so_m) & 3) == 0 && (((uintptr_t)p.partial) & 15) == 0 &&
                     (tap_major ? ((p.N | p.so_k) & 3) == 0 : (torch_order && (R & 3) == 0));
    float s = 0.f;
    if (staged) {
        const int items = vec ? (R >> 2) : R;
        int nparts = SAT_WN_THREADS / items;
        if (nparts > 8) nparts = 8;
        if (nparts > p.nsplit) nparts = p.nsplit;
        if (nparts < 1) nparts = 1;
        while (nparts > 1 && (long long)nparts * R > SAT_WN_ROW_CAP) --nparts;
        for (int idx = threadIdx.x; idx < items * nparts; idx += SAT_WN_THREADS) {
            const int zp = idx / items, it = idx - zp * items;
            float* dst = row + (size_t)zp * R;
            if (vec) {
                if (tap_major) {
                    const int nq = p.N >> 2;
                    const int k = it / nq, n = (it - k * nq) << 2;
                    const f32x4 a = sat_wn_slab_sum4(base + (size_t)k * p.so_k + n, p.count, zp, nparts, p.nsplit);
                    dst[(n + 0) * p.K + k] = a[0];
                    dst[(n + 1) * p.K + k] = a[1];
                    dst[(n + 2) * p.K + k] = a[2];
                    dst[(n + 3) * p.K + k] = a[3];
                } else {
                    const f32x4 a = sat_wn_slab_sum4(base + 4 * it, p.count, zp, nparts, p.nsplit);
                    *reinterpret_cast<f32x4*>(dst + 4 * it) = a;
                }
            } else {
                int n, k;
                if (tap_major) { k = it / p.N; n = it - k * p.N; }
                else           { n = it / p.K; k = it - n * p.K; }
                dst[n * p.K + k] = sat_wn_slab_sum(base + (size_t)n * p.so_n + (size_t)k * p.so_k, p.count, zp, nparts, p.nsplit);
            }
        }
        __syncthreads();
        for (int r = threadIdx.x; r < R; r += SAT_WN_THREADS) {
            float a = row[r];
            for (int zp = 1; zp < nparts; ++zp) a += row[(size_t)zp * R + r];
            row[r] = a;
            s += v[r] * a;
        }
    } else {
        for (int r = threadIdx.x; r < R; r += SAT_WN_THREADS) {
            const int n = r / p.K, k = r - n * p.K;
            s += v[r] * sat_wn_slab_sum(base + (size_t)n * p.so_n + (size_t)k * p.so_k, p.count, 0, 1, p.nsplit);
        }
    }
    s = sat_block_sum_1024(s, red);
    const float nrm = p.norm[d];
    const float g = p.g[d];
    const float c1 = g / nrm, c2 = g * s / (nrm * nrm * nrm);
    float* dv = p.dv + (size_t)d * R;
    for (int r = threadIdx.x; r < R; r += SAT_WN_THREADS) {
        float dw;
        if (staged) dw = row[r];
        else {
            const int n = r / p.K, k = r - n * p.K;
            dw = sat_wn_slab_sum(base + (size_t)n * p.so_n + (size_t)k * p.so_k, p.count, 0, 1, p.nsplit);
        }
        dv[r] = c1 * dw - c2 * v[r];
    }
    if (threadIdx.x == 0) p.dg[d] = s / nrm;
    if (p.bias_partial) {
        const float* bp = p.bias_partial + (size_t)d * p.bias_cols;
// ... 429 lines not shown
```

### stable_audio_tools_amd/csrc/sat_device.h

```cpp
#pragma once

#if defined(SAT_HIPEMU)
#include "hipemu.h"
#define SAT_DEVICE static inline
#else
#include <hip/hip_runtime.h>
#define SAT_DEVICE __device__ __forceinline__
#endif

#include <stdint.h>

typedef float f32x4 __attribute__((ext_vector_type(4)));
typedef float f32x16 __attribute__((ext_vector_type(16)));
typedef short bf16x8 __attribute__((ext_vector_type(8)));
typedef uint32_t u32x4 __attribute__((ext_vector_type(4)));
typedef int i32x8 __attribute__((ext_vector_type(8)));

#define SAT_WAVE 64

#if defined(SAT_HIPEMU)
static inline float hipemu_bf16_to_f32(short s) {
    uint32_t u = ((uint32_t)(uint16_t)s) << 16;
    float f;
    memcpy(&f, &u, 4);
    return f;
}
static inline f32x16 sat_mfma_32x32x2_f32(float a, float b, f32x16 c) {
    struct { float a, b; } mine = {a, b};
    const char* all = hipemu::wave_exchange(&mine, sizeof(mine));
    const int l = hipemu::lane_id();
    const int col = l & 31, hi = l >> 5;
    f32x16 d = c;
    for (int r = 0; r < 16; ++r) {
        const int row = (r & 3) + 8 * (r >> 2) + 4 * hi;
        float acc = c[r];
        for (int k = 0; k < 2; ++k) {
            float av, bv;
            memcpy(&av, all + (size_t)(row + 32 * k) * hipemu::kSlotBytes, 4);
            memcpy(&bv, all + (size_t)(col + 32 * k) * hipemu::kSlotBytes + 4, 4);
            acc = fmaf(av, bv, acc);
        }
        d[r] = acc;
    }
    return d;
}
static inline f32x16 sat_mfma_32x32x16_bf16(bf16x8 a, bf16x8 b, f32x16 c) {
    struct { bf16x8 a, b; } mine = {a, b};
    const char* all = hipemu::wave_exchange(&mine, sizeof(mine));
    const int l = hipemu::lane_id();
    const int col = l & 31, hi = l >> 5;
    f32x16 d = c;
    for (int r = 0; r < 16; ++r) {
        const int row = (r & 3) + 8 * (r >> 2) + 4 * hi;
        float acc = c[r];
        for (int g = 0; g < 2; ++g) {
            bf16x8 av, bv;
            memcpy(&av, all + (size_t)(row + 32 * g) * hipemu::kSlotBytes, 16);
            memcpy(&bv, all + (size_t)(col + 32 * g) * hipemu::kSlotBytes + 16, 16);
            for (int e = 0; e < 8; ++e) acc += hipemu_bf16_to_f32(av[e]) * hipemu_bf16_to_f32(bv[e]);
        }
        d[r] = acc;
    }
    return d;
}
static inline f32x4 sat_mfma_16x16x32_bf16(bf16x8 a, bf16x8 b, f32x4 c) {
    struct { bf16x8 a, b; } mine = {a, b};
    const char* all = hipemu::wave_exchange(&mine, sizeof(mine));
    const int l = hipemu::lane_id();
    const int col = l & 15, grp = l >> 4;
    f32x4 d = c;
    for (int r = 0; r < 4; ++r) {
        const int row = 4 * grp + r;
        float acc = c[r];
        for (int g = 0; g < 4; ++g) {
            bf16x8 av, bv;
            memcpy(&av, all + (size_t)(row + 16 * g) * hipemu::kSlotBytes, 16);
            memcpy(&bv, all + (size_t)(col + 16 * g) * hipemu::kSlotBytes + 16, 16);
            for (int e = 0; e < 8; ++e) acc += hipemu_bf16_to_f32(av[e]) * hipemu_bf16_to_f32(bv[e]);
        }
        d[r] = acc;
    }
    return d;
}
static inline float hipemu_e4m3_to_f32(uint8_t v) {
    const int s = v >> 7, e = (v >> 3) & 15, m = v & 7;
    float f;
    if (e == 15 && m == 7) f = NAN;
    else if (e == 0) f = ldexpf((float)m, -9);
    else f = ldexpf((float)(8 + m), e - 10);
    return s ? -f : f;
}
static inline f32x16 sat_mfma_32x32x64_fp8(i32x8 a, i32x8 b, f32x16 c) {
    struct { i32x8 a, b; } mine = {a, b};
    const char* all = hipemu::wave_exchange(&mine, sizeof(mine));
    const int l = hipemu::lane_id();
    const int col = l & 31, hi = l >> 5;
    f32x16 d = c;
    for (int r = 0; r < 16; ++r) {
        const int row = (r & 3) + 8 * (r >> 2) + 4 * hi;
        float acc = c[r];
        for (int g = 0; g < 2; ++g) {
            uint8_t av[32], bv[32];
            memcpy(av, all + (size_t)(row + 32 * g) * hipemu::kSlotBytes, 32);
            memcpy(bv, all + (size_t)(col + 32 * g) * hipemu::kSlotBytes + 32, 32);
            for (int e = 0; e < 32; ++e) acc += hipemu_e4m3_to_f32(av[e]) * hipemu_e4m3_to_f32(bv[e]);
        }
        d[r] = acc;
    }
    return d;
}
#else
SAT_DEVICE f32x16 sat_mfma_32x32x64_fp8(i32x8 a, i32x8 b, f32x16 c) {
    return __builtin_amdgcn_mfma_scale_f32_32x32x64_f8f6f4(a, b, c, 0, 0, 0, 127, 0, 127);
}
SAT_DEVICE f32x16 sat_mfma_32x32x2_f32(float a, float b, f32x16 c) {
    return __builtin_amdgcn_mfma_f32_32x32x2f32(a, b, c, 0, 0, 0);
}
SAT_DEVICE f32x16 sat_mfma_32x32x16_bf16(bf16x8 a, bf16x8 b, f32x16 c) {
    typedef __bf16 bf16x8_t __attribute__((ext_vector_type(8)));
    return __builtin_amdgcn_mfma_f32_32x32x16_bf16(__builtin_bit_cast(bf16x8_t, a), __builtin_bit_cast(bf16x8_t, b), c, 0, 0, 0);
}
SAT_DEVICE f32x4 sat_mfma_16x16x32_bf16(bf16x8 a, bf16x8 b, f32x4 c) {
    typedef __bf16 bf16x8_t __attribute__((ext_vector_type(8)));
    return __builtin_amdgcn_mfma_f32_16x16x32_bf16(__builtin_bit_cast(bf16x8_t, a), __builtin_bit_cast(bf16x8_t, b), c, 0, 0, 0);
}
#endif

SAT_DEVICE uint32_t sat_f32x4_to_fp8(float a, float b, float c, float d) {
#if defined(SAT_HIPEMU)
    auto enc = [](float x) -> uint32_t {
        if (x != x) return 0x7fu;
        const uint32_t sign = x < 0.f ? 0x80u : 0u;
        float ax = fabsf(x);
        if (ax > 448.f) ax = 448.f;
        if (ax < ldexpf(1.0f, -10)) return sign;
        int e;
        frexpf(ax, &e);
        int ue = e - 1;
        if (ue < -6) ue = -6;
        const float q = ldexpf(1.0f, ue - 3);
        float m = nearbyintf(ax / q);
        float v = m * q;
        if (v > 448.f) v = 448.f;
        if (v == 0.f) return sign;
        frexpf(v, &e);
        ue = e - 1;
        uint32_t bits;
        if (ue < -6) bits = (uint32_t)nearbyintf(v / ldexpf(1.0f, -9));
        else bits = ((uint32_t)(ue + 7) << 3) | ((uint32_t)nearbyintf(v / ldexpf(1.0f, ue - 3)) - 8u);
        return sign | bits;
    };
    return enc(a) | (enc(b) << 8) | (enc(c) << 16) | (enc(d) << 24);
#else
    const float lim = 448.0f;
    a = fminf(fmaxf(a, -lim), lim); b = fminf(fmaxf(b, -lim), lim); c = fminf(fmaxf(c, -lim), lim); d = fminf(fmaxf(d, -lim), lim);
    int w = 0;
    w = __builtin_amdgcn_cvt_pk_fp8_f32(a, b, w, false);
    w = __builtin_amdgcn_cvt_pk_fp8_f32(c, d, w, true);
    return (uint32_t)w;
#endif
}

SAT_DEVICE short sat_f32_to_bf16(float f) {
    uint32_t u;
    memcpy(&u, &f, 4);
    if ((u & 0x7fffffffu) > 0x7f800000u) return (short)0x7fc0;
    u += 0x7fffu + ((u >> 16) & 1u);
    return (short)(u >> 16);
}
SAT_DEVICE float sat_bf16_to_f32(short s) {
    uint32_t u = ((uint32_t)(uint16_t)s) << 16;
    float f;
    memcpy(&f, &u, 4);
    return f;
}

SAT_DEVICE void sat_split2_pk(float a, float b, uint32_t* hi, uint32_t* lo) {
#if defined(SAT_HIPEMU)
    const short ha = sat_f32_to_bf16(a), hb = sat_f32_to_bf16(b);
    const short la = sat_f32_to_bf16(a - sat_bf16_to_f32(ha)), lb = sat_f32_to_bf16(b - sat_bf16_to_f32(hb));
    *hi = ((uint32_t)(uint16_t)hb << 16) | (uint16_t)ha;
    *lo = ((uint32_t)(uint16_t)lb << 16) | (uint16_t)la;
#else
    typedef __bf16 sat_bf2 __attribute__((ext_vector_type(2)));
    typedef float sat_f2 __attribute__((ext_vector_type(2)));
    const sat_f2 v = {a, b};
    const sat_bf2 h = __builtin_convertvector(v, sat_bf2);
    const sat_f2 d = v - __builtin_convertvector(h, sat_f2);
    const sat_bf2 l = __builtin_convertvector(d, sat_bf2);
    *hi = __builtin_bit_cast(uint32_t, h);
    *lo = __builtin_bit_cast(uint32_t, l);
#endif
}

SAT_DEVICE uint32_t sat_cvt2_pk(float a, float b) {
#if defined(SAT_HIPEMU)
    return ((uint32_t)(uint16_t)sat_f32_to_bf16(b) << 16) | (uint16_t)sat_f32_to_bf16(a);
#else
    typedef __bf16 sat_bf2 __attribute__((ext_vector_type(2)));
    typedef float sat_f2 __attribute__((ext_vector_type(2)));
    const sat_f2 v = {a, b};
    return __builtin_bit_cast(uint32_t, __builtin_convertvector(v, sat_bf2));
#endif
}

#if defined(SAT_HIPEMU)
#define SAT_UNIFORM(x) (x)
#else
#define SAT_UNIFORM(x) __builtin_amdgcn_readfirstlane(x)
#endif

SAT_DEVICE void sat_xcd_tile(int L, int nshare, int nouter, int* share_idx, int* outer_idx) {
    const int ngroups = nouter >> 3;
    const int per_group = 8 * nshare;
    if (L < ngroups * per_group) {
        const int grp = L / per_group, rem = L - grp * per_group;
        *share_idx = rem >> 3;
        *outer_idx = grp * 8 + (rem & 7);
    } else {
        const int R = L - ngroups * per_group;
        *share_idx = R % nshare;
        *outer_idx = ngroups * 8 + R / nshare;
    }
}

template <int B, class T>
SAT_DEVICE T& sat_pick(T& a, T& b) {
    if constexpr (B == 0) return a;
    else return b;
}

SAT_DEVICE float sat_wave_sum(float v) {
    for (int m = 32; m >= 1; m >>= 1) v += __shfl_xor(v, m);
    return v;
}
SAT_DEVICE float sat_half_sum(float v) {
    for (int m = 16; m >= 1; m >>= 1) v += __shfl_xor(v, m);
    return v;
}

SAT_DEVICE void sat_sincos2(float y, float* s2y, float* c2y) {
    const float hi = y * 0.31830987334251404f;
    float lo = fmaf(y, 0.31830987334251404f, -hi);
    lo = fmaf(y, 1.2841276486e-08f, lo);
#if defined(SAT_HIPEMU)
    const float f = (hi - floorf(hi)) + lo;
    *s2y = sinf(6.283185307179586f * f);
    *c2y = cosf(6.283185307179586f * f);
#else
    const float f = __builtin_amdgcn_fractf(hi) + lo;
    *s2y = __builtin_amdgcn_sinf(f);
    *c2y = __builtin_amdgcn_cosf(f);
#endif
}
SAT_DEVICE float sat_sin2(float y) {
    float s, c;
    sat_sincos2(y, &s, &c);
    return fmaf(-0.5f, c, 0.5f);
}

SAT_DEVICE float sat_snake(float x, float a, float ib) {
    return fmaf(ib, sat_sin2(x * a), x);
}
SAT_DEVICE float sat_snake_sc(float x, float ib, float c2) {
    return fmaf(ib, fmaf(-0.5f, c2, 0.5f), x);
}

#if defined(SAT_HIPEMU)
static inline void sat_glds16(const void* g, void* lds_wave_base) { memcpy((char*)lds_wave_base + 16 * hipemu::lane_id(), g, 16); }
static inline void sat_glds4(const void* g, void* lds_wave_base) { memcpy((char*)lds_wave_base + 4 * hipemu::lane_id(), g, 4); }
static inline void sat_glds16_raw(const void* g, void* lds_wave_base) { sat_glds16(g, lds_wave_base); }
#define SAT_WAIT_VMCNT(n)
#define SAT_RAW_BARRIER() hipemu::block_barrier()
#define SAT_WAIT_LGKM0()
#define SAT_SCHED_FENCE()
static inline void sat_wave_sync() { int z = 0; (void)hipemu::wave_exchange(&z, sizeof(z)); }
#define SAT_SETPRIO(x)
#define SAT_SCHED_GROUP(mask, n)
static inline bool sat_wave_any(bool v) {
    int x = v ? 1 : 0;
    for (int m = 32; m >= 1; m >>= 1) x |= __shfl_xor(x, m);
    return x != 0;
}
#else
SAT_DEVICE void sat_glds16(const void* g, void* lds_wave_base) {
    __builtin_amdgcn_global_load_lds((const __attribute__((address_space(1))) void*)g,
                                     (__attribute__((address_space(3))) void*)lds_wave_base, 16, 0, 0);
}
SAT_DEVICE void sat_glds4(const void* g, void* lds_wave_base) {
    __builtin_amdgcn_global_load_lds((const __attribute__((address_space(1))) void*)g,
                                     (__attribute__((address_space(3))) void*)lds_wave_base, 4, 0, 0);
}
SAT_DEVICE void sat_glds16_raw(const void* g, void* lds_wave_base) {
    const unsigned m0v = __builtin_amdgcn_readfirstlane((unsigned)(uintptr_t)(__attribute__((address_space(3))) void*)lds_wave_base);
    unsigned keep;
    asm volatile("s_mov_b32 %0, m0\n\ts_mov_b32 m0, %2\n\ts_nop 0\n\tglobal_load_lds_dwordx4 %1, off\n\ts_mov_b32 m0, %0" : "=&s"(keep) : "v"(g), "s"(m0v) : "memory");
}
#define SAT_WAIT_VMCNT(n) asm volatile("s_waitcnt vmcnt(%0)" ::"n"(n) : "memory")
#define SAT_RAW_BARRIER() __builtin_amdgcn_s_barrier()
#define SAT_WAIT_LGKM0() asm volatile("s_waitcnt lgkmcnt(0)" ::: "memory")
#define SAT_SCHED_FENCE() __builtin_amdgcn_sched_barrier(0)
SAT_DEVICE void sat_wave_sync() { __builtin_amdgcn_wave_barrier(); }
#define SAT_SETPRIO(x) __builtin_amdgcn_s_setprio(x)
#define SAT_SCHED_GROUP(mask, n) __builtin_amdgcn_sched_group_barrier(mask, n, 0)
SAT_DEVICE bool sat_wave_any(bool v) { return __builtin_amdgcn_ballot_w64(v) != 0; }
#endif

typedef short bf16x4 __attribute__((ext_vector_type(4)));
#if defined(SAT_HIPEMU)
static inline bf16x4 sat_lds_read_tr16_b64(const void* lane_addr) {
    const void* mine = lane_addr;
    const char* all = hipemu::wave_exchange(&mine, (int)sizeof(mine));
    const int l = hipemu::lane_id(), g0 = l & ~15, i = l & 15;
    bf16x4 r;
    for (int q = 0; q < 4; ++q) {
        const char* src;
        memcpy(&src, all + (size_t)(g0 + 4 * q + (i >> 2)) * hipemu::kSlotBytes, sizeof(src));
        short v;
        memcpy(&v, src + 2 * (i & 3), 2);
        r[q] = v;
    }
    return r;
}
#else
SAT_DEVICE bf16x4 sat_lds_read_tr16_b64(const void* lane_addr) {
    return __builtin_amdgcn_ds_read_tr16_b64_v4i16((__attribute__((address_space(3))) bf16x4*)lane_addr);
}
#endif

#if defined(SAT_WITH_MFMA_PRIO)
#define SAT_MFMA_PRIO(x) SAT_SETPRIO(x)
#else
#define SAT_MFMA_PRIO(x)
#endif

void sat_set_error(const char* msg);
int sat_check_launch(const char* what);
int sat_cu_count();

#if defined(SAT_HIPEMU)
#define SAT_LAUNCH(kernel, grid, block, stream, params) \
    hipemu::launch((grid), (block), [=]() { kernel(params); })
#else
#define SAT_LAUNCH(kernel, grid, block, stream, params) \
    hipLaunchKernelGGL(kernel, (grid), (block), 0, (hipStream_t)(stream), params)
#endif

static inline int sat_cdiv(int a, int b) { return (a + b - 1) / b; }
static inline long long sat_cdivll(long long a, long long b) { return (a + b - 1) / b; }
```

### stable_audio_tools_amd/functional.py

```python
import torch

from . import ops as _ops_mod
from .ops import PACK_CONV_DGRAD, PACK_CONV_FWD, PACK_POLYPHASE


def _ops(ops):
    return ops if ops is not None else _ops_mod.get_ops()


class SumAllFn(torch.autograd.Function):

    @staticmethod
    def forward(ctx, x, ops=None):
        ctx.in_shape, ctx.in_dtype = x.shape, x.dtype
        return _ops(ops).sum_all(x.detach())

    @staticmethod
    def backward(ctx, g):
        return g.to(ctx.in_dtype).expand(ctx.in_shape), None


def sum_all(x, ops=None):
    return SumAllFn.apply(x, ops)


def mean_all(x, ops=None):
    return SumAllFn.apply(x, ops) / x.numel()


class DerivedCache:

    def __init__(self):
        self.items = {}

    def get(self, name, sources, make):
        from . import _caches
        if not _caches.trackable(*sources):
            return make()
        key = tuple((t.data_ptr(), _caches.version_of(t), t.device) for t in sources if t is not None) + _caches.epoch_of(*sources)
        hit = self.items.get(name)
        if hit is None or hit[0] != key:
            hit = (key, make())
            self.items[name] = hit
        return hit[1]


def _cached(cache, name, sources, make):
    return make() if cache is None else cache.get(name, sources, make)


class WeightNormFn(torch.autograd.Function):
    @staticmethod
    def forward(ctx, v, g, ops=None):
        ops = _ops(ops)
        v = v.contiguous()
        gf = g.contiguous().view(-1)
        w, norm = ops.wn_fold(v, gf)
        ctx.save_for_backward(v, gf, norm)
        ctx.ops = ops
        ctx.g_shape = g.shape
        return w

    @staticmethod
    def backward(ctx, dw):
        v, gf, norm = ctx.saved_tensors
        dv, dg = ctx.ops.wn_grad(v, gf, norm, dw.contiguous())
        return dv, dg.view(ctx.g_shape), None


def _conv_dgrad(ops, dy, w, k, stride, dil, pad, cin, tin, dsnake, res=None, out=None, emit=None):
    if stride == 1:
        if (res is None and out is None and not emit and ops.edge_ok(w.shape[0], cin, k, 1, dil, (k - 1) * dil - pad) and tin == dy.shape[2]
                and (dsnake is None or w.shape[0] <= 2)):
            return ops.edge_conv(dy, w, (k - 1) * dil - pad, mode=1, dsnake=dsnake)
        if ops.bf16x3_ok(k, 1, dil):
            q = ops.k7q_applicable(w.shape[0], k, 1, dil, (k - 1) * dil - pad, cin)
            return ops.conv1d_bf16x3(dy, ops.pack_bf16x3(w, mode=1, q=q), cin, k, 1, dil, (k - 1) * dil - pad, tout=tin,
                                     dsnake=dsnake, res=res, out=out, emit=emit)
        wpb = ops.pack(w, PACK_CONV_DGRAD)
        return ops.conv1d(dy, wpb, cin, k, 1, dil, (k - 1) * dil - pad, tout=tin, dsnake=dsnake, res=res, out=out)
    if out is not None:
        raise NotImplementedError("_conv_dgrad(out=...) is only plumbed through the stride-1 kernels")
    if ops.bf16x3_ok(k, stride, dil, transposed=True):
        return ops.convtr1d_bf16x3(dy, ops.pack_bf16x3(w, mode=2, stride=stride), cin, k, stride, pad, tout=tin,
                                   dsnake=dsnake, res=res)
    wpb = ops.pack(w, PACK_POLYPHASE, stride)
    return ops.convtr1d(dy, wpb, cin, k, stride, pad, tout=tin, dsnake=dsnake, res=res)


def _conv_wgrad(ops, dy, x, k, stride, dil, pad, snake, bias_grad=False, raw=False):
    if ops.edge_ok(x.shape[1], dy.shape[1], k, stride, dil, pad) and dy.shape[2] == x.shape[2] and (snake is None or dy.shape[1] <= 2):
        return ops.edge_conv_wgrad(dy, x, k, pad, snake=snake, dy_rowsum=bias_grad, raw=raw)
    if ops.wgrad7_bf16x3_ok(x.shape[1], k, stride, dil):
        return ops.conv_wgrad7_bf16x3(dy, x, dil, pad, snake=snake, dy_rowsum=bias_grad, raw=raw)
    return ops.conv_wgrad(dy, x, k, stride, dil, pad, snake=snake, snake_on=2, lo_rowsum=bias_grad, raw=raw)


def _wn_forward(ops, v, g):
    v = v.contiguous()
    gf = g.contiguous().view(-1)
    w, norm = ops.wn_fold(v, gf)
    return w, (v, gf, norm)


def _wn_backward(ops, slabs, saved, g_shape, bias_partial=None):
    v, gf, norm = saved
    out = ops.wn_grad_splits(slabs, v, gf, norm, bias_partial=bias_partial)
    return (out[0], out[1].view(g_shape)) + tuple(out[2:])


def _conv_fwd(ops, x, w, stride, dil, pad, bias=None, snake=None, res=None, tanh_out=False, dsnake=None, tout=None, cache=None, emit=None,
              keep_planes=False):
    cout, cin, k = w.shape
    if (res is None and ops.edge_ok(cin, cout, k, stride, dil, pad) and (tout is None or tout == x.shape[2])
            and (snake is None or cout <= 2) and (dsnake is None or cin <= 2) and (not emit or cin <= 2)):
        y = ops.edge_conv(x, w, pad, bias=bias, snake=snake, tanh_out=tanh_out, dsnake=dsnake, emit=emit)
    elif ops.bf16x3_ok(k, stride, dil):
        q = ops.k7q_applicable(cin, k, stride, dil, pad, cout)
        planes = _cached(cache, "pack_fwd_q" if q else "pack_fwd", (w,), lambda: ops.pack_bf16x3(w, stride=stride, q=q))
        sconsts = _cached(cache, "snake", snake, lambda: ops.snake_consts(snake[0], snake[1])) if snake is not None else None
        return ops.conv1d_bf16x3(x, planes, cout, k, stride, dil, pad, tout=tout, bias=bias,
                                 snake=snake, res=res, tanh_out=tanh_out, dsnake=dsnake, sconsts=sconsts, emit=emit, keep_planes=keep_planes)
    else:
        y = ops.conv1d(x, _cached(cache, "pack_fwd32", (w,), lambda: ops.pack(w, PACK_CONV_FWD)), cout, k, stride, dil, pad, tout=tout,
                       bias=bias, snake=snake, res=res, tanh_out=tanh_out, dsnake=dsnake)
    return (y, None) if keep_planes else y


def _convtr_fwd(ops, x, w, stride, pad, bias=None, snake=None, cache=None):
    cin, cout, k = w.shape
    if ops.bf16x3_ok(k, stride, 1, transposed=True):
        planes = _cached(cache, "pack_tr", (w,), lambda: ops.pack_bf16x3(w, mode=2, stride=stride))
        sconsts = _cached(cache, "snake", snake, lambda: ops.snake_consts(snake[0], snake[1])) if snake is not None else None
        return ops.convtr1d_bf16x3(x, planes, cout, k, stride, pad, bias=bias, snake=snake, sconsts=sconsts)
    return ops.convtr1d(x, _cached(cache, "pack_tr32", (w,), lambda: ops.pack(w, PACK_POLYPHASE, stride)), cout, k, stride, pad,
                        bias=bias, snake=snake)


class SnakeConv1dFn(torch.autograd.Function):

    @staticmethod
    def forward(ctx, x, alpha, beta, w, bias, res, stride, dil, pad, tanh_out, ops=None, cache=None, next_snake=None, g=None):
        ops = _ops(ops)
        x = x.contiguous()
        wn = ()
        if g is not None:
            w, wn = _wn_forward(ops, w, g)
        w = w.contiguous()
        cout, cin, k = w.shape
        snake = (alpha.contiguous(), beta.contiguous()) if alpha is not None else None
        emit = None
        if next_snake is not None and not tanh_out:
            tout_ = (x.shape[2] + 2 * pad - dil * (k - 1) - 1) // stride + 1
            if ((ops.emit_ok(cout, k, stride, tout_, next_snake[2]) and ops.bf16x3_ok(k, stride, dil))
                    or (res is None and snake is None and ops.edge_emit_ok(cin, cout, k, stride, dil, pad, next_snake[2]))):
                emit = (next_snake[0].detach(), next_snake[1].detach())
        y = _conv_fwd(ops, x, w, stride, dil, pad, bias=bias, snake=snake,
                      res=res.contiguous() if res is not None else None, tanh_out=tanh_out, cache=cache, emit=emit)
        ctx.ops = ops
        ctx.cfg = (stride, dil, pad, tanh_out, bias is not None, res is not None, alpha is not None)
        ctx.g_shape = g.shape if g is not None else None
        ctx.save_for_backward(x, alpha, beta, w, y if tanh_out else None, *wn)
        return y

    @staticmethod
    def backward(ctx, dy):
        ops = ctx.ops
        stride, dil, pad, tanh_out, has_bias, has_res, has_snake = ctx.cfg
        x, alpha, beta, w, y = ctx.saved_tensors[:5]
        wn = ctx.saved_tensors[5:]
        cout, cin, k = w.shape
        dy = dy.contiguous()
        if tanh_out:
            dy = dy * (1.0 - y * y)
        snake = (alpha, beta) if has_snake else None
        dres = dy if has_res else None
        dw = dbias = dg = None
        if ctx.needs_input_grad[3] or (wn and ctx.needs_input_grad[13]):
            dw = _conv_wgrad(ops, dy, x, k, stride, dil, pad, snake, bias_grad=has_bias, raw=bool(wn))
            if has_bias:
                dw, dbias = dw
            if wn:
                dw, dg, *rest = _wn_backward(ops, dw, wn, ctx.g_shape, bias_partial=dbias)
                if has_bias:
                    dbias = rest[0]
        elif has_bias:
            dbias = ops.rowsum(dy)
        dx = da = db = None
        if has_snake:
            dx, da, db = _conv_dgrad(ops, dy, w, k, stride, dil, pad, cin, x.shape[2], (x, alpha, beta))
        elif ctx.needs_input_grad[0]:
            dx = _conv_dgrad(ops, dy, w, k, stride, dil, pad, cin, x.shape[2], None)
        return dx, da, db, dw, dbias, dres, None, None, None, None, None, None, None, dg


class SnakeConvTr1dFn(torch.autograd.Function):

    @staticmethod
    def forward(ctx, x, alpha, beta, w, bias, stride, pad, ops=None, cache=None, g=None):
        ops = _ops(ops)
        x = x.contiguous()
        wn = ()
        if g is not None:
            w, wn = _wn_forward(ops, w, g)
        w = w.contiguous()
        cin, cout, k = w.shape
        snake = (alpha.contiguous(), beta.contiguous()) if alpha is not None else None
        y = _convtr_fwd(ops, x, w, stride, pad, bias=bias, snake=snake, cache=cache)
        ctx.ops = ops
        ctx.cfg = (stride, pad, bias is not None, alpha is not None)
        ctx.g_shape = g.shape if g is not None else None
        ctx.save_for_backward(x, alpha, beta, w, *wn)
        return y

    @staticmethod
    def backward(ctx, dy):
        ops = ctx.ops
        stride, pad, has_bias, has_snake = ctx.cfg
        x, alpha, beta, w = ctx.saved_tensors[:4]
        wn = ctx.saved_tensors[4:]
        cin, cout, k = w.shape
        dy = dy.contiguous()
        snake = (alpha, beta) if has_snake else None
        dbias = ops.rowsum(dy) if has_bias else None
        dw = ops.conv_wgrad(x, dy, k, stride, 1, pad, snake=snake, snake_on=1, raw=bool(wn))
        dg = None
        if wn:
            dw, dg = _wn_backward(ops, dw, wn, ctx.g_shape)
        dx = da = db = None
        if has_snake:
            dx, da, db = _conv_fwd(ops, dy, w, stride, 1, pad, dsnake=(x, alpha, beta), tout=x.shape[2])
        elif ctx.needs_input_grad[0]:
            dx = _conv_fwd(ops, dy, w, stride, 1, pad, tout=x.shape[2])
        return dx, da, db, dw, dbias, None, None, None, None, dg


class ResidualUnitFn(torch.autograd.Function):

    @staticmethod
    def forward(ctx, x, a1, b1, w1, bias1, a2, b2, w2, bias2, dil, ops=None, recompute=False, caches=None, next_snake=None, fuse=False,
                g1=None, g2=None):
        ops = _ops(ops)
        x = x.contiguous()
        wn1 = wn2 = ()
        if g1 is not None:
            w1, wn1 = _wn_forward(ops, w1, g1)
        if g2 is not None:
            w2, wn2 = _wn_forward(ops, w2, g2)
        w1 = w1.contiguous()
        w2 = w2.contiguous()
        c = x.shape[1]
        k1 = w1.shape[2]
        pad = dil * (k1 - 1) // 2
        c1, c2 = caches if caches is not None else (None, None)
        emit = ctx.k7_planes = None
        if next_snake is not None and ops.emit_ok(c, w2.shape[2], 1, x.shape[2], next_snake[2]):
            emit = (next_snake[0].detach(), next_snake[1].detach())
        if fuse and w2.shape[2] == 1 and w1.shape[0] == c and ops.ru_fused_ok(c, k1, dil, x.shape[2]):
            w7q = _cached(c1, "pack_q7", (w1,), lambda: ops.pack_k7q(w1))
            w1q = _cached(c2, "pack_q1", (w2,), lambda: ops.pack_k7q(w2))
            sc = None
            if c1 is not None and c2 is not None:
                sc = (_cached(c1, "snake", (a1, b1), lambda: ops.snake_consts(a1, b1)), _cached(c2, "snake", (a2, b2), lambda: ops.snake_consts(a2, b2)))
            h, y = ops.residual_unit_fwd(x, (a1, b1), w7q, bias1, (a2, b2), w1q, bias2, k1, dil, keep_h=ctx is not None and not recompute and fuse != "nokeep",
                                         emit=emit, sconsts=sc)
        else:
            keep = bool(ops.wgrad7_planes and not recompute and any(ctx.needs_input_grad))
            h = _conv_fwd(ops, x, w1, 1, dil, pad, bias=bias1, snake=(a1, b1), cache=c1, keep_planes=keep)
            if keep:
                h, ctx.k7_planes = h
            y = _conv_fwd(ops, h, w2, 1, 1, 0, bias=bias2, snake=(a2, b2), res=x, cache=c2, emit=emit)
        ctx.ops = ops
        ctx.dil = dil
        ctx.recompute = bool(recompute)
        ctx.g_shapes = (g1.shape if g1 is not None else None, g2.shape if g2 is not None else None)
        ctx.save_for_backward(x, None if recompute else h, a1, b1, w1, a2, b2, w2, bias1 if recompute else None, *wn1, *wn2)
        return y

    @staticmethod
    def backward(ctx, dy):
        ops = ctx.ops
        x, h, a1, b1, w1, a2, b2, w2, bias1 = ctx.saved_tensors[:9]
        gs1, gs2 = ctx.g_shapes
        rest = ctx.saved_tensors[9:]
        wn1 = rest[:3] if gs1 is not None else ()
        wn2 = rest[len(wn1):] if gs2 is not None else ()
        dil = ctx.dil
        c = x.shape[1]
        k1, k2 = w1.shape[2], w2.shape[2]
        pad1 = dil * (k1 - 1) // 2
        t = x.shape[2]
        dy = dy.contiguous()
        if ctx.recompute:
            h = _conv_fwd(ops, x, w1, 1, dil, pad1, bias=bias1, snake=(a1, b1))
        want_emit = ops.emit_ok(w1.shape[0], k2, 1, t, dil) and ops.k7q_applicable(w1.shape[0], k1, 1, dil, pad1, c)
        kept = ctx.k7_planes if not ctx.recompute and want_emit and ops.kept_planes_valid(ctx.k7_planes, x, (a1, b1), dil, pad1) else None
        skip_dh = False

        def wgrad1(dh, bias_grad):
            dw = ops.conv_wgrad7_from_planes(dh, kept, x, (a1, b1), dil, pad1, raw=bool(wn1))
            if dw is None:
                return _conv_wgrad(ops, dh, x, k1, 1, dil, pad1, (a1, b1), bias_grad=bias_grad, raw=bool(wn1))
            return (dw, ops.rowsum(dh, partial=bool(wn1))) if bias_grad else dw
        if k2 == 1 and w2.shape[0] == c and w1.shape[0] == c and ops.ru_k1_bwd_ok(dy.shape[0], c, t):
            skip_dh = bool(kept is not None and ops.ru_k1_bwd_skip_dh)
            dh, da2, db2, dw2, dbias2, dbias1 = ops.ru_k1_bwd(dy, h, w2, (a2, b2), emit=want_emit, raw=bool(wn2), skip_dh=skip_dh)
            try:
                dw1 = wgrad1(dh, False)
                if skip_dh:
                    dx, da1, db1 = _conv_dgrad(ops, dh, w1, k1, 1, dil, pad1, c, t, (x, a1, b1), res=dy)
            finally:
                ops.dh_written()
        else:
            dw2, dbias2 = ops.conv_wgrad(dy, h, k2, 1, 1, 0, snake=(a2, b2), snake_on=2, lo_rowsum=True, raw=bool(wn2))
            dh, da2, db2 = _conv_dgrad(ops, dy, w2, k2, 1, 1, 0, c, t, (h, a2, b2), emit=want_emit)
            dw1, dbias1 = wgrad1(dh, True)
        dg1 = dg2 = None
        if wn1:
            if dbias1.dim() == 2:
                dw1, dg1, dbias1 = _wn_backward(ops, dw1, wn1, gs1, bias_partial=dbias1)
            else:
                dw1, dg1 = _wn_backward(ops, dw1, wn1, gs1)
        if wn2:
            if dbias2.dim() == 2:
                dw2, dg2, dbias2 = _wn_backward(ops, dw2, wn2, gs2, bias_partial=dbias2)
            else:
                dw2, dg2 = _wn_backward(ops, dw2, wn2, gs2)
        if not skip_dh:
            dx, da1, db1 = _conv_dgrad(ops, dh, w1, k1, 1, dil, pad1, c, t, (x, a1, b1), res=dy)
        return dx, da1, db1, dw1, dbias1, da2, db2, dw2, dbias2, None, None, None, None, None, None, dg1, dg2


class VaeSampleFn(torch.autograd.Function):

    @staticmethod
    def forward(ctx, pre, noise, ops=None):
        ops = _ops(ops)
        pre = pre.contiguous()
        noise = noise.contiguous()
        z, kl = ops.vae_sample_fwd(pre, noise)
        ctx.ops = ops
        ctx.save_for_backward(pre, noise)
        return z, kl

    @staticmethod
    def backward(ctx, dz, dkl):
        pre, noise = ctx.saved_tensors
        dpre = ctx.ops.vae_sample_bwd(pre, noise, dz.contiguous() if dz is not None else None,
                                      dkl.contiguous() if dkl is not None else None)
        return dpre, None, None
```

### stable_audio_tools_amd/ops.py

```python
import ctypes

import torch

from . import _caches, _lib

PACK_CONV_FWD = 0
PACK_CONV_DGRAD = 1
PACK_POLYPHASE = 2


def _ptr(t):
    if t is None:
        return None
    return ctypes.c_void_p(t.data_ptr())


def _keep_zeros(shape, dtype, device):
    with torch.inference_mode(False):
        return torch.zeros(shape, dtype=dtype, device=device)


def _keep_empty(shape, dtype, device):
    with torch.inference_mode(False):
        return torch.empty(shape, dtype=dtype, device=device)
# ... 194 lines not shown
        rows = self.lib.sat_edge_conv_partial_rows(b, t) if dsnake is not None else 0
        x2, a2, b2, pda, pdb = self._dsnake_args(dsnake, cout, rows, x.device)
        ep, ela, elb = self._emit_args(emit, b, cout, t, x.device, self._stream(x), consts=False)
        self._chk(self.lib.sat_edge_conv(_ptr(x), _ptr(w), _ptr(bias), _ptr(alpha), _ptr(beta), _ptr(y), _ptr(x2), _ptr(a2), _ptr(b2),
                                         _ptr(pda), _ptr(pdb), _ptr(ep.hi), _ptr(ep.lo), _ptr(ela), _ptr(elb), ep.rows, b, cin, cout, t, k, pad, mode,
                                         int(tanh_out), self._stream(x)))
        self._emit_done(emit, y, ep)
        return self._dsnake_result(y, pda, pdb)

    def edge_conv_wgrad(self, dy, x, k, pad, snake=None, dy_rowsum=False, raw=False):
        b, m, t = dy.shape
        n = x.shape[1]
        alpha, beta = snake if snake is not None else (None, None)
        self._f32(dy, x, alpha, beta)
        nsplit = self.lib.sat_edge_conv_wgrad_nsplit(b, m, n, t)
        partial = torch.empty(nsplit, m * n * k, dtype=torch.float32, device=dy.device)
        fused = dy_rowsum and n <= 2
        rs = torch.empty(m, nsplit, dtype=torch.float32, device=dy.device) if fused else None
        self._chk(self.lib.sat_edge_conv_wgrad(_ptr(dy), _ptr(x), _ptr(alpha), _ptr(beta), _ptr(partial), _ptr(rs), b, m, n, t, k, pad,
                                               self._stream(dy)))
        return self._wgrad_result(WgradSlabs(partial, nsplit, (m, n, k), (n * k, k, 1)), raw, dy, dy_rowsum, rs)

    def _wgrad_result(self, slabs, raw, dy, dy_rowsum, rs):
        dw = slabs if raw else slabs.reduce(self)
        if not dy_rowsum:
            return dw
        if raw:
            return dw, (rs if rs is not None else self.rowsum(dy, partial=True))
        return dw, (self._sum_last(rs) if rs is not None else self.rowsum(dy))

    def bf16x3_ok(self, k, stride, dil, transposed=False):
        if not self.use_bf16x3:
            return False
        if transposed or stride > 1:
            return k == 2 * stride and stride & (stride - 1) == 0 and dil == 1
        return k == 1 or (2 <= k <= 4 and dil == 1) or (5 <= k <= 8 and (k - 1) * dil <= 62)

    k7q = True
    k7q_persist = True
    k7q_dma_in_mfma = True
    k7q_min_cin = 64
    k7q_min_cout = 128
    k7q_wide_cin = 512

    def k7q_applicable(self, cin, k, stride, dil, pad, cout=None):
        return (self.k7q and self.use_bf16x3 and stride == 1 and 5 <= k <= 7 and 0 <= pad <= 32
                and (k - 1) * dil <= 62 and cin >= self.k7q_min_cin
                and (cout is None or cout >= self.k7q_min_cout or cin >= self.k7q_wide_cin))

    def pack_bf16x3(self, w, mode=0, stride=1, q=False):
        if q:
            if stride != 1:
                raise RuntimeError("sat_pack_weights_k7q: unsupported shape")
            return (*self.pack_k7q(w, mode), "q")
        self._f32(w)
        d0, d1, k = w.shape
        n = self.lib.sat_pack_weights_bf16x3_size(d0, d1, k, stride, mode)
        if n <= 0:
            raise RuntimeError("sat_pack_weights_bf16x3: unsupported shape")
        hi = torch.empty(n, dtype=torch.int16, device=w.device)
        lo = torch.empty(n, dtype=torch.int16, device=w.device)
        self._chk(self.lib.sat_pack_weights_bf16x3(_ptr(w), _ptr(hi), _ptr(lo), d0, d1, k, stride, mode, self._stream(w)))
        return hi, lo

    def snake_consts(self, alpha, beta):
        self._f32(alpha, beta)
        a = torch.empty_like(alpha)
        ib = torch.empty_like(beta)
        self._chk(self.lib.sat_snake_consts(_ptr(alpha), _ptr(beta), _ptr(a), _ptr(ib), alpha.numel(), self._stream(alpha)))
        return a, ib

    def _conv_out(self, out, b, cout, tout, device):
        if out is None:
            return torch.empty(b, cout, tout, dtype=torch.float32, device=device)
        if tuple(out.shape) != (b, cout, tout) or not out.is_contiguous():
            raise ValueError("conv out= must be a dense (B, Cout, Tout) tensor")
        self._f32(out)
        return out

    def _bf16x3_call(self, fn, rows, x, w_planes, cout, tout, dims, bias, snake, res, tanh_out, dsnake, out=None, sconsts=None, emit=None):
        b, cin, tin = x.shape
        self._f32(x, bias, res)
        sa = sib = None
        if snake is not None:
            sa, sib = sconsts if sconsts is not None else self.snake_consts(snake[0], snake[1])
        y = self._conv_out(out, b, cout, tout, x.device)
        x2, a2, b2, pda, pdb = self._dsnake_args(dsnake, cout, rows, x.device)
        ep, ea, eib = self._emit_args(emit, b, cout, tout, x.device, self._stream(x))
        args = (_ptr(x), _ptr(w_planes[0]), _ptr(w_planes[1]), _ptr(bias), _ptr(sa), _ptr(sib),
                _ptr(res), _ptr(y), _ptr(x2), _ptr(a2), _ptr(b2), _ptr(pda), _ptr(pdb),
                b, cin, cout, tin, tout, *dims, int(tanh_out))
        if emit:
            self._chk(self.lib.sat_conv1d_bf16x3_emit(*args, _ptr(ep.hi), _ptr(ep.lo), _ptr(ea), _ptr(eib), ep.rows, self._stream(x)))
        else:
            self._chk(fn(*args, self._stream(x)))
        self._emit_done(emit, y, ep)
        return self._dsnake_result(y, pda, pdb)

    ru_fused = True

    def ru_fused_ok(self, c, k, dil, t):
        return (self.ru_fused and self.use_bf16x3 and self.k7q and self.k7q_min_cin <= c <= 128
                and 5 <= k <= 7 and (k - 1) * dil <= 62 and (k - 1) * dil % 2 == 0 and (k - 1) * dil // 2 <= 32 and t % 4 == 0)

    def pack_k7q(self, w, mode=0):
        self._f32(w)
        d0, d1, k = w.shape
        n = self.lib.sat_pack_weights_k7q_size(d0, d1, k, mode)
        if n <= 0:
            raise RuntimeError("sat_pack_weights_k7q: unsupported shape")
        hi = torch.empty(n, dtype=torch.int16, device=w.device)
        lo = torch.empty(n, dtype=torch.int16, device=w.device)
        self._chk(self.lib.sat_pack_weights_k7q(_ptr(w), _ptr(hi), _ptr(lo), d0, d1, k, mode, self._stream(w)))
        return hi, lo

    def residual_unit_fwd(self, x, snake1, w7q, bias1, snake2, w1q, bias2, k, dil, keep_h=True, emit=None, sconsts=None):
        b, c, t = x.shape
        self._f32(x, bias1, bias2)
        pad = (k - 1) * dil // 2
        st = self._stream(x)
        sa1, sib1 = sconsts[0] if sconsts is not None else self.snake_consts(snake1[0], snake1[1])
        sa2, sib2 = sconsts[1] if sconsts is not None else self.snake_consts(snake2[0], snake2[1])
        xp = self._take_emitted(x, snake1) or self._k7_prepass(x, sa1, sib1, t, pad, st)
        h = torch.empty_like(x) if keep_h else None
        y = torch.empty_like(x)
        ep, ea, eib = self._emit_args(emit, b, c, t, x.device, st, owned=False)
        if emit and ep.hi.data_ptr() == xp.hi.data_ptr():
            ep = self._emit_planes(b, c, t, x.device, st, alt=True)
        self._chk(self.lib.sat_residual_unit_fwd(_ptr(xp.hi), _ptr(xp.lo), xp.rows, _ptr(w7q[0]), _ptr(w7q[1]), _ptr(bias1), _ptr(sa2), _ptr(sib2),
                                                 _ptr(w1q[0]), _ptr(w1q[1]), _ptr(bias2), _ptr(x), _ptr(h), _ptr(y), b, c, t, k, dil, pad,
                                                 _ptr(ep.hi), _ptr(ep.lo), _ptr(ea), _ptr(eib), ep.rows, st))
        self._emit_done(emit, y, ep)
        return h, y

    _NO_PLANES = Planes(None, None, 0)
    k7_emit = True
    wgrad7_planes = True
    wgrad7_planes_budget_gib = 16.0
    ru_k1_bwd_skip_dh = True

    def emit_ok(self, cout, k, stride, tout, consumer_dil):
        if not (self.k7_emit and self.use_bf16x3 and self.k7q_applicable(cout, 7, 1, consumer_dil, 3 * consumer_dil, cout)):
            return False
        generic = (stride == 1 and k <= 4) or stride > 1
        return generic and tout % 4 == 0

    def edge_emit_ok(self, cin, cout, k, stride, dil, pad, consumer_dil):
        return (self.k7_emit and self.use_bf16x3 and cin <= 2 and self.edge_ok(cin, cout, k, stride, dil, pad)
                and self.k7q_applicable(cout, 7, 1, consumer_dil, 3 * consumer_dil, cout))

    def _emit_args(self, emit, b, c, t, device, st, consts=True, owned=True):
        if not emit:
            return self._NO_PLANES, None, None
        snake = None if emit is True else emit
        ea, eb = (None, None) if snake is None else self.snake_consts(*snake) if consts else snake
        self._f32(ea, eb)
        return self._emit_planes(b, c, t, device, st, owner=snake if owned else None), ea, eb

    def _emit_done(self, emit, y, planes):
        if emit:
            snake = None if emit is True else emit
            self._emitted = planes.of(y, snake) if _caches.trackable(y, *(snake or ())) else None

    def _take_emitted(self, x, snake, peek=False):
        e = self._emitted
        if not peek:
            self._emitted = None
        return e if e is not None and e.holds(x, snake) else None

    def _emit_planes(self, b, c, t, device, st, alt=False, owner=None):
        own = self._owned_planes(owner, b, c, t, device, st)
        if own is not None:
            return own.rewrite()
        rows = self.lib.sat_conv1d_k7_plane_rows(t, t, 0)
        key = ("emit", b, c, t, device, st.value if st is not None else 0, alt)
        n = b * ((c + 7) // 8) * rows * 8
        return Planes(self._workspace(key + ("hi",), n, torch.int16, device, zero=True),
                      self._workspace(key + ("lo",), n, torch.int16, device, zero=True), rows)

    def _k7_prepass(self, x, sa, sib, tout, pad, st):
        b, c, t = x.shape
        rows = self.lib.sat_conv1d_k7_plane_rows(t, tout, pad)
        need = 2 * b * ((c + 7) // 8) * rows * 8
        ws = self._workspace(("k7p", x.device, st.value if st is not None else 0), need, torch.int16, x.device, grow=True)
        hi, lo = ws[:need // 2], ws[need // 2:need]
        self._chk(self.lib.sat_conv1d_k7_planes(_ptr(x), _ptr(sa), _ptr(sib), _ptr(hi), _ptr(lo), b, c, t, rows, st))
        return Planes(hi, lo, rows)

    def _owned_planes(self, snake, b, c, t, device, st, create=False):
        if snake is None or not self.wgrad7_planes:
            return None
        key = (snake[0].data_ptr(), snake[1].data_ptr(), b, c, t, device)
        own = self._own_planes.get(key)
        capturing = device.type == "cuda" and torch.cuda.is_current_stream_capturing()
        sv = st.value if st is not None else 0
        if own is not None and own.stream != sv and not capturing:
            return None
        if own is None and create and not capturing:
            rows = self.lib.sat_conv1d_k7_plane_rows(t, t, 0)
            n = b * ((c + 7) // 8) * rows * 8
            if sum(4 * o.hi.numel() for o in self._own_planes.values()) + 4 * n <= self.wgrad7_planes_budget_gib * 2 ** 30:
                own = self._own_planes[key] = OwnedPlanes(n, rows, device, sv)
        return own

    def release_owned_planes(self):
        self._own_planes.clear()

    def kept_planes_valid(self, kept, x, snake, dil, pad):
        b, c, t = x.shape
        return bool(kept is not None and self.wgrad7_planes and kept.holds(x, snake) and self.conv_wgrad7_planes_ok(b, c, c, t, dil, pad, kept.rows, kept.rows))

    def conv_wgrad7_from_planes(self, dh, kept, x, snake, dil, pad, raw=False):
        em = self._take_emitted(dh, None, peek=True) if kept is not None and self.wgrad7_planes and kept.holds(x, snake) else None
        b, c, t = x.shape
        if em is None or not self.conv_wgrad7_planes_ok(b, c, c, t, dil, pad, em.rows, kept.rows):
            return None
        return self.conv_wgrad7_planes((em.hi, em.lo, em.rows), (kept.hi, kept.lo, kept.rows), b, c, c, t, dil, pad, raw=raw)

    def _check_written(self, t):
        if t is not None and self._dh_unwritten is not None and t.data_ptr() == self._dh_unwritten:
            raise RuntimeError("this tensor is a dh that sat_ru_k1_bwd did not write (skip_dh): only its planes exist")

    def dh_written(self):
        self._dh_unwritten = None

    def conv1d_bf16x3(self, x, w_planes, cout, k, stride=1, dil=1, pad=0, tout=None, bias=None, snake=None, res=None,
                      tanh_out=False, dsnake=None, out=None, sconsts=None, emit=None, keep_planes=False):
        b, cin, tin = x.shape
        if tout is None:
            tout = (tin + 2 * pad - dil * (k - 1) - 1) // stride + 1
        rows = self.lib.sat_conv1d_bf16x3_partial_rows(b, tout, k, stride)
        if len(w_planes) == 3:
            if not (stride == 1 and 5 <= k <= 7 and 0 <= pad <= 32 and (k - 1) * dil <= 62):
                raise ValueError("conv1d_bf16x3: q-packed weights need stride 1, 5 <= K <= 7, pad <= 32, (K-1)*dil <= 62")
            return self._k7_planes_call(rows, x, w_planes, cout, tout, k, dil, pad, bias, snake, res, tanh_out, dsnake, out, sconsts, keep_planes)
        y = self._bf16x3_call(self.lib.sat_conv1d_bf16x3, rows, x, w_planes, cout, tout, (k, stride, dil, pad),
                              bias, snake, res, tanh_out, dsnake, out, sconsts, emit)
        return (y, None) if keep_planes else y

    def _k7_planes_call(self, prows, x, w_planes, cout, tout, k, dil, pad, bias, snake, res, tanh_out, dsnake, out=None, sconsts=None,
                        keep_planes=False):
        b, cin, tin = x.shape
        self._f32(x, bias, res)
        sa = sib = None
        if snake is not None:
            sa, sib = sconsts if sconsts is not None else self.snake_consts(snake[0], snake[1])
        st = self._stream(x)
        xp = self._take_emitted(x, snake)
        if xp is None:
            self._check_written(x)
        own = self._owned_planes(snake, b, cin, tin, x.device, st, create=True) if keep_planes and tin == tout and _caches.trackable(x) else None
        if xp is None and own is not None:
            xp = own.rewrite().of(x, snake)
            self._chk(self.lib.sat_conv1d_k7_planes(_ptr(x), _ptr(sa), _ptr(sib), _ptr(xp.hi), _ptr(xp.lo), b, cin, tin, xp.rows, st))
        elif xp is None:
            xp = self._k7_prepass(x, sa, sib, tout, pad, st)
        kept = xp if own is not None and xp.own is own and k == 7 and cout == cin else None
        y = self._conv_out(out, b, cout, tout, x.device)
        x2, a2, b2, pda, pdb = self._dsnake_args(dsnake, cout, prows, x.device)
        self._chk(self.lib.sat_conv1d_bf16x3_planesq(_ptr(xp.hi), _ptr(xp.lo), xp.rows, _ptr(w_planes[0]), _ptr(w_planes[1]), _ptr(bias), _ptr(res),
                                                     _ptr(y), _ptr(x2), _ptr(a2), _ptr(b2), _ptr(pda), _ptr(pdb), b, cin, cout, tin, tout,
                                                     k, dil, pad, int(tanh_out), {True: 0, False: 1, "force": 2}[self.k7q_persist] | (4 if self.k7q_dma_in_mfma else 0), st))
        y = self._dsnake_result(y, pda, pdb)
        return (y, kept) if keep_planes else y

    def convtr1d_bf16x3(self, x, w_planes, cout, k, stride, pad, tout=None, bias=None, snake=None, res=None,
                        tanh_out=False, dsnake=None, sconsts=None):
        b, cin, tin = x.shape
        if tout is None:
            tout = (tin - 1) * stride - 2 * pad + k
        rows = self.lib.sat_convtr1d_bf16x3_partial_rows(b, tout, stride, pad)
        return self._bf16x3_call(self.lib.sat_convtr1d_bf16x3, rows, x, w_planes, cout, tout, (k, stride, pad),
                                 bias, snake, res, tanh_out, dsnake, None, sconsts)

    def convtr1d(self, x, w_packed, cout, k, stride, pad, tout=None, bias=None, snake=None, res=None,
                 tanh_out=False, dsnake=None):
        b, cin, tin = x.shape
        if tout is None:
            tout = (tin - 1) * stride - 2 * pad + k
        alpha, beta = snake if snake is not None else (None, None)
        self._f32(x, w_packed, bias, alpha, beta, res)
        y = torch.empty(b, cout, tout, dtype=torch.float32, device=x.device)
        rows = self.lib.sat_convtr1d_partial_rows(b, tout, stride, pad) if dsnake is not None else 0
        if rows < 0:
            raise RuntimeError("sat_convtr1d: unsupported stride")
        x2, a2, b2, pda, pdb = self._dsnake_args(dsnake, cout, rows, x.device)
        self._chk(self.lib.sat_convtr1d(_ptr(x), _ptr(w_packed), _ptr(bias), _ptr(alpha), _ptr(beta), _ptr(res), _ptr(y),
                                        _ptr(x2), _ptr(a2), _ptr(b2), _ptr(pda), _ptr(pdb),
                                        b, cin, cout, tin, tout, k, stride, pad, int(tanh_out), self._stream(x)))
        return self._dsnake_result(y, pda, pdb)

    def conv_wgrad(self, lo, hi, k, stride=1, dil=1, pad=0, snake=None, snake_on=0, lo_rowsum=False, raw=False):
        bsz, m, tlo = lo.shape
        _, n, thi = hi.shape
        alpha, beta = snake if snake is not None else (None, None)
        self._f32(lo, hi, alpha, beta)
        x3 = self.use_bf16x3 and dil == 1 and self.lib.sat_conv_wgrad_bf16x3_nsplit(bsz, m, n, tlo, k, stride) > 0
        if x3:
            nsplit = self.lib.sat_conv_wgrad_bf16x3_nsplit(bsz, m, n, tlo, k, stride)
        else:
            nsplit = self.lib.sat_conv_wgrad_nsplit(bsz, m, n, tlo, k, stride, dil)
        if nsplit < 0:
            raise RuntimeError("sat_conv_wgrad: receptive field too large")
        partial = torch.empty(nsplit, m * n * k, dtype=torch.float32, device=lo.device)
        so_m, so_n, so_k = n * k, k, 1
        rs = None
        if x3:
            fused = lo_rowsum and not (snake is not None and snake_on == 1)
            rs = torch.empty(m, nsplit, dtype=torch.float32, device=lo.device) if fused else None
            self._chk(self.lib.sat_conv_wgrad_bf16x3(_ptr(lo), _ptr(hi), _ptr(alpha), _ptr(beta),
                                                     snake_on if snake is not None else 0, _ptr(partial), so_m, so_n, so_k,
                                                     bsz, m, n, tlo, thi, k, stride, pad, _ptr(rs), self._stream(lo)))
        else:
            self._chk(self.lib.sat_conv_wgrad(_ptr(lo), _ptr(hi), _ptr(alpha), _ptr(beta), snake_on if snake is not None else 0,
# ... 736 lines not shown

    def quant_fp8_rows(self, src):
        dt = self._dt(src)
        if src.dim() != 2 or src.stride(1) != 1 or src.shape[1] % 8 or src.stride(0) % 8 or src.shape[1] > 8192:
            raise ValueError("quant_fp8_rows takes a 2-D tensor with a contiguous last dim, C % 8 == 0, C <= 8192")
        q = torch.empty(src.shape, dtype=torch.uint8, device=src.device)
        scale = torch.empty(src.shape[0], dtype=torch.float32, device=src.device)
        self._chk(self.lib.sat_quant_fp8_rows(_ptr(src), src.stride(0), _ptr(q), q.stride(0), _ptr(scale), src.shape[0], src.shape[1],
                                              int(dt == 0), self._stream(src)))
        return q, scale

    gemm_fp8_tile = None

    def _pick_tile_fp8(self, m, n, k):
        if self.gemm_fp8_tile is not None:
            return self.gemm_fp8_tile
        return min(self._TILE_MODEL, key=lambda t: (self._tile_cost(t, m, n, (k + 1) // 2), t))

    def gemm_fp8(self, a, b, alpha, bias=None, res=None, gate=None, rows_per_gate=0, epilogue=0, out_dtype=torch.bfloat16, want_pre=False,
                 out=None, row_alpha=None, col_alpha=None):
        if a.dtype != torch.uint8 or b.dtype != torch.uint8 or a.stride(1) != 1 or b.stride(1) != 1 or a.shape[1] != b.shape[1]:
            raise TypeError("gemm_fp8 takes (rows, K) uint8 operands")
        m, k = a.shape
        n = b.shape[0]
        f32 = out_dtype == torch.float32
        if bias is not None:
            self._f32(bias)
        nout = n // 2 if epilogue == self.EPI_SWIGLU else n
        c = out if out is not None else torch.empty(m, nout, dtype=out_dtype, device=a.device)
        pre = torch.empty(m, n, dtype=out_dtype, device=a.device) if (want_pre and epilogue == self.EPI_SWIGLU) else None
        alpha, col_alpha = self._fp8_alphas(alpha, col_alpha, n)
        if row_alpha is not None and (row_alpha.dtype != torch.float32 or row_alpha.numel() != m or not row_alpha.is_contiguous()):
            raise TypeError("gemm_fp8: row_alpha is (M,) fp32")
        self._chk(self.lib.sat_gemm_fp8(_ptr(a), a.stride(0), _ptr(b), b.stride(0), _ptr(c), nout, _ptr(bias),
                                        _ptr(res), res.stride(0) if res is not None else 0, _ptr(gate), gate.stride(0) if gate is not None else 0,
                                        rows_per_gate, _ptr(pre), n, _ptr(self._zeros_page(a.device)), _ptr(alpha), _ptr(row_alpha), _ptr(col_alpha),
                                        m, n, k, epilogue, int(f32), self._pick_tile_fp8(m, n, k), self._stream(a)))
        return (c, pre) if want_pre and epilogue == self.EPI_SWIGLU else c

    @staticmethod
    def _fp8_alphas(alpha, col_alpha, n):
        if alpha is None and col_alpha is None:
            raise TypeError("fp8 GEMM: alpha (per-tensor de-quantisation scale) or col_alpha (per output channel) is required")
        if alpha is not None:
            alpha = alpha.float().reshape(1).contiguous()
        if col_alpha is not None and (col_alpha.dtype != torch.float32 or col_alpha.numel() != n or not col_alpha.is_contiguous()):
            raise TypeError("fp8 GEMM: col_alpha is (N,) fp32, one factor per row of b")
        return alpha, col_alpha

    def gemm_heads_fp8(self, x, w, alpha, cs, heads, nb, ntok, sec0, nsec, reuse=None, row_alpha=None, col_alpha=None):
        out = self._head_planes(nb, heads, ntok, sec0, nsec, reuse, x.device)
        npad = out["np"]
        alpha, col_alpha = self._fp8_alphas(alpha, col_alpha, w.shape[0])
        self._chk(self.lib.sat_gemm_qkv_fp8(_ptr(x), x.stride(0), _ptr(w), w.stride(0), _ptr(cs), (cs.shape[0] - ntok) if cs is not None else 0,
                                            _ptr(out.get("q")), _ptr(out.get("k")), _ptr(out.get("v_tr")), _ptr(self._zeros_page(x.device)),
                                            _ptr(alpha), _ptr(row_alpha), _ptr(col_alpha), nb, ntok, npad, heads, x.shape[1], sec0, nsec,
                                            self._pick_tile_fp8(nb * ntok, nsec * heads * 64, x.shape[1]), self._stream(x)))
        return out

    def cast_bf16(self, src, transpose=False, row_pad=1, out=None):
        dt = self._dt(src)
        if src.dim() != 2 or src.stride(1) != 1:
            raise ValueError("cast_bf16 takes a 2-D tensor with a contiguous last dim")
        r, c = src.shape
        rp = (r + row_pad - 1) // row_pad * row_pad
        shape = (c, rp) if transpose else (r, c)
        dst = out if out is not None else torch.empty(shape, dtype=torch.bfloat16, device=src.device)
        if tuple(dst.shape) != shape or dst.dtype != torch.bfloat16 or dst.stride(1) != 1:
            raise ValueError("cast_bf16: bad destination")
        self._chk(self.lib.sat_cast_bf16(_ptr(src), src.stride(0), _ptr(dst), dst.stride(0), r, c, rp, int(dt == 0), int(transpose),
                                         self._stream(src)))
        return dst

    def cast_bf16_tpair(self, a, b, row_pad=8, out_b=None):
        da, db = self._dt(a), self._dt(b)
        if a.dim() != 2 or b.dim() != 2 or a.stride(1) != 1 or b.stride(1) != 1:
            raise ValueError("cast_bf16_tpair takes 2-D tensors with a contiguous last dim")
        (ra, ca), (rb, cb) = a.shape, b.shape
        rpa, rpb = (ra + row_pad - 1) // row_pad * row_pad, (rb + row_pad - 1) // row_pad * row_pad
        ta = torch.empty(ca, rpa, dtype=torch.bfloat16, device=a.device)
        tb = out_b if out_b is not None else torch.empty(cb, rpb, dtype=torch.bfloat16, device=b.device)
        if tuple(tb.shape) != (cb, rpb) or tb.dtype != torch.bfloat16 or tb.stride(1) != 1:
            raise ValueError("cast_bf16_tpair: bad destination")
        self._chk(self.lib.sat_cast_bf16_tpair(_ptr(a), a.stride(0), _ptr(ta), ta.stride(0), ra, ca, rpa, int(da == 0),
                                               _ptr(b), b.stride(0), _ptr(tb), tb.stride(0), rb, cb, rpb, int(db == 0), self._stream(a)))
        return ta, tb

    def cast_bf16_dual(self, src, row_pad=8):
        dt = self._dt(src)
        if src.dim() != 2 or src.stride(1) != 1:
            raise ValueError("cast_bf16_dual takes a 2-D tensor with a contiguous last dim")
        r, c = src.shape
        rp = (r + row_pad - 1) // row_pad * row_pad
        if c % 8 or rp % 8 or src.stride(0) % (4 if dt == 0 else 8) or src.data_ptr() % 16:
            return None
        dst = torch.empty(r, c, dtype=torch.bfloat16, device=src.device)
        dst_t = torch.empty(c, rp, dtype=torch.bfloat16, device=src.device)
        self._chk(self.lib.sat_cast_bf16_dual(_ptr(src), src.stride(0), _ptr(dst), dst.stride(0), _ptr(dst_t), dst_t.stride(0), r, c, rp,
                                              int(dt == 0), self._stream(src)))
        return dst, dst_t

    def split_bf16x3(self, src, side):
        self._f32(src)
        r, c = src.shape
        dst = torch.empty(r, 3 * c, dtype=torch.bfloat16, device=src.device)
        self._chk(self.lib.sat_split_bf16x3(_ptr(src), src.stride(0), _ptr(dst), 3 * c, r, c, side, self._stream(src)))
        return dst

    def adamw_step_dev(self, p, g, m, v, hyper, beta1, beta2, eps, weight_decay, ema=None):
        self._f32(p, g, m, v, ema, hyper)
        if hyper.numel() < 5:
            raise ValueError("adamw_step_dev: hyper holds 5 fp32 values")
        self._chk(self.lib.sat_adamw_step_dev(_ptr(p), _ptr(g), _ptr(m), _ptr(v), p.numel(), _ptr(hyper), beta1, beta2, eps, weight_decay,
                                              _ptr(ema), self._stream(p)))

    def allreduce_available(self):
        return bool(self.lib.sat_allreduce_available())

    def allreduce_unique_id(self):
        buf = ctypes.create_string_buffer(128)
        self._chk(self.lib.sat_allreduce_unique_id(buf))
        return buf.raw

    def allreduce_init(self, uid, world, rank):
        if len(uid) != 128:
            raise ValueError("allreduce_init: the unique id is 128 bytes")
        comm = ctypes.c_void_p()
        self._chk(self.lib.sat_allreduce_init(ctypes.create_string_buffer(bytes(uid), 128), int(world), int(rank), ctypes.byref(comm)))
        return comm

    def allreduce_bucket(self, comm, buf, mode=0):
        if buf.dtype not in (torch.float32, torch.bfloat16) or not buf.is_contiguous():
            raise TypeError("allreduce_bucket takes a contiguous fp32 or bf16 tensor")
        if not self.simulator and not buf.is_cuda:
            raise RuntimeError("stable_audio_tools_amd kernels need CUDA(HIP) tensors; there is no CPU path")
        self._chk(self.lib.sat_allreduce_bucket(comm, _ptr(buf), buf.numel(), 0 if buf.dtype == torch.float32 else 1, int(mode), self._stream(buf)))

    def allreduce_finalize(self, comm):
        self._chk(self.lib.sat_allreduce_finalize(comm))

    def multi_copy(self, srcs, dsts):
        import numpy as np
        n = len(srcs)
        if n == 0:
            return
        tab = np.empty((n, 3), dtype=np.int64)
        for i, (src, dst) in enumerate(zip(srcs, dsts)):
            if src.dtype != torch.float32 or dst.dtype != torch.float32 or not src.is_contiguous() or not dst.is_contiguous() \
                    or src.numel() != dst.numel() or src.device != dst.device:
                raise ValueError("multi_copy: sources and destinations must be contiguous fp32 tensors of equal sizes on one device")
            tab[i] = (src.data_ptr(), dst.data_ptr(), src.numel())
        self._chk(self.lib.sat_multi_copy(tab.ctypes.data, n, self._stream(srcs[0])))

    def adamw_step(self, p, g, m, v, lr, beta1, beta2, eps, weight_decay, step, grad_scale=1.0, ema=None, ema_decay=0.0):
        self._f32(p, g, m, v, ema)
        self._chk(self.lib.sat_adamw_step(_ptr(p), _ptr(g), _ptr(m), _ptr(v), p.numel(), lr, beta1, beta2, eps,
                                          weight_decay, step, grad_scale, _ptr(ema), ema_decay, self._stream(p)))


_ops = None


def get_ops():
    global _ops
    if _ops is None:
        _ops = SatOps(_lib.load())
    return _ops
```

Before: 8.150.

## Batch per-step parameter preparation into grouped fold, snake and pack kernels

Adds a per-stack parameter plan that, once per training step, runs weight-norm folding, snake constant computation and bf16x3 weight packing for all conv layers in three grouped launches driven by entry tables. Forward and backward reuse these prepared results through per-module plan slots instead of launching many small per-layer kernels. This targets launch and Python overhead from the many tiny parameter-derived ops. In exchange it adds plan bookkeeping and cache-validity tracking, which could return stale derived weights if invalidation is wrong.

```diff
diff --git a/include/sat_amd.h b/include/sat_amd.h
--- a/include/sat_amd.h
+++ b/include/sat_amd.h
@@ -149,6 +149,10 @@
 
 int sat_multi_copy(const void* entries, int nent, void* stream);
 
+int sat_prep_fold(const void* entries, int nent, void* stream);
+int sat_prep_snake(const void* entries, int nent, void* stream);
+int sat_prep_pack(const void* entries, int nent, void* stream);
+
 int sat_allreduce_available(void);
 int sat_allreduce_unique_id(void* id128);
 int sat_allreduce_init(const void* id128, int world, int rank, void** comm);
diff --git a/stable_audio_tools_amd/_lib.py b/stable_audio_tools_amd/_lib.py
--- a/stable_audio_tools_amd/_lib.py
+++ b/stable_audio_tools_amd/_lib.py
@@ -66,6 +66,9 @@
     "sat_vae_sample_fwd": (_I, [_P, _P, _P, _P, _I, _I, _I, _P]),
     "sat_vae_sample_bwd": (_I, [_P, _P, _P, _P, _P, _I, _I, _I, _P]),
     "sat_multi_copy": (_I, [_P, _I, _P]),
+    "sat_prep_fold": (_I, [_P, _I, _P]),
+    "sat_prep_snake": (_I, [_P, _I, _P]),
+    "sat_prep_pack": (_I, [_P, _I, _P]),
     "sat_adamw_step": (_I, [_P, _P, _P, _P, _L, _F, _F, _F, _F, _F, _I, _F, _P, _F, _P]),
     "sat_adamw_step_dev": (_I, [_P, _P, _P, _P, _L, _P, _F, _F, _F, _F, _P, _P]),
     "sat_allreduce_available": (_I, []),
diff --git a/stable_audio_tools_amd/autoencoders.py b/stable_audio_tools_amd/autoencoders.py
--- a/stable_audio_tools_amd/autoencoders.py
+++ b/stable_audio_tools_amd/autoencoders.py
@@ -137,14 +137,16 @@
 
     def derived_cache(self, *others):
         ps = list(self._parameters.values()) + list(others)
-        return self._derived if _inference_pass(*ps) else None
+        if _inference_pass(*ps):
+            return self._derived
+        return self.__dict__.get("_plan_slot") if Fn._ops(None).param_prep else None
 
 
 class WNConv1d(_WNConvBase):
     def forward(self, x, snake=None, res=None, tanh_out=False, next_snake=None):
         a, b = (self.p32("alpha", snake.alpha), self.p32("beta", snake.beta)) if snake is not None else (None, None)
         if next_snake is not None and next_snake[0].dtype != torch.float32:
-            next_snake = (self.p32("next_alpha", next_snake[0]), self.p32("next_beta", next_snake[1]), next_snake[2])
+            next_snake = (self.p32("next_alpha", next_snake[0]), self.p32("next_beta", next_snake[1]), *next_snake[2:])
         w, g = self.weight_args()
         return Fn.SnakeConv1dFn.apply(x, a, b, w, self.bias32(), res, self.stride, self.dilation,
                                       self.padding, tanh_out, None, self.derived_cache(a, b), next_snake, g)
@@ -158,6 +160,13 @@
         w, g = self.weight_args()
         return Fn.SnakeConvTr1dFn.apply(x, a, b, w, self.bias32(), self.stride, self.padding, None,
                                         self.derived_cache(a, b), g)
+
+
+def _attach_plan(stack):
+    plan = stack.__dict__["_prep"] = Fn.ParamPlan()
+    for name, m in stack.named_modules():
+        if isinstance(m, _WNConvBase):
+            m.__dict__["_plan_slot"] = plan.slot(name)
 
 
 def _require_snake(use_snake, antialias_activation=False):
@@ -185,14 +194,14 @@
         )
 
     def entry_snake(self):
-        s1 = self.layers[0]
-        return (s1.alpha, s1.beta, self.dilation)
+        s1, c1 = self.layers[0], self.layers[1]
+        return (s1.alpha, s1.beta, self.dilation, c1.derived_cache(s1.alpha, s1.beta))
 
     def forward(self, x, next_snake=None):
         s1, c1, s2, c2 = self.layers
         ca, cb = c1.derived_cache(s1.alpha, s1.beta), c2.derived_cache(s2.alpha, s2.beta)
         if next_snake is not None and next_snake[0].dtype != torch.float32:
-            next_snake = (c2.p32("next_alpha", next_snake[0]), c2.p32("next_beta", next_snake[1]), next_snake[2])
+            next_snake = (c2.p32("next_alpha", next_snake[0]), c2.p32("next_beta", next_snake[1]), *next_snake[2:])
         (w1, g1), (w2, g2) = c1.weight_args(), c2.weight_args()
         return Fn.ResidualUnitFn.apply(x, c1.p32("alpha", s1.alpha), c1.p32("beta", s1.beta), w1, c1.bias32(),
                                        c2.p32("alpha", s2.alpha), c2.p32("beta", s2.beta), w2, c2.bias32(), self.dilation, None,
@@ -256,6 +265,7 @@
         layers += [SnakeBeta(c_mults[-1] * channels),
                    WNConv1d(c_mults[-1] * channels, latent_dim, kernel_size=3, padding=1)]
         self.layers = nn.Sequential(*layers)
+        _attach_plan(self)
 
     def forward(self, x):
         mods = list(self.layers)
@@ -285,6 +295,7 @@
                    nn.Tanh() if final_tanh else nn.Identity()]
         self.final_tanh = final_tanh
         self.layers = nn.Sequential(*layers)
+        _attach_plan(self)
 
     def forward(self, x):
         mods = list(self.layers)
diff --git a/stable_audio_tools_amd/csrc/conv1d_bf16x3.hip b/stable_audio_tools_amd/csrc/conv1d_bf16x3.hip
--- a/stable_audio_tools_amd/csrc/conv1d_bf16x3.hip
+++ b/stable_audio_tools_amd/csrc/conv1d_bf16x3.hip
@@ -35,12 +35,6 @@
     float* ru_h = nullptr;
 };
 
-SAT_DEVICE void sat_split2(float x, short* hi, short* lo) {
-    const short h = sat_f32_to_bf16(x);
-    *hi = h;
-    *lo = sat_f32_to_bf16(x - sat_bf16_to_f32(h));
-}
-
 template <int NG, int CS, bool GATHER>
 __global__ void __launch_bounds__(256)
 #if !defined(SAT_HIPEMU)
@@ -635,6 +629,27 @@
 #include "conv1d_bf16x3_k7.h"
 #include "conv1d_planes.h"
 #include "conv1d_bf16x3_k7q.h"
+#include "param_prep.h"
+
+bool sat_prep_pack_geometry(int layout, int D0, int D1, int K, int stride, SatPrepGeom* g) {
+    if (layout >= SAT_PREP_BF_MODE0 && layout <= SAT_PREP_BF_MODE2) {
+        SatPackBfParams p{};
+        if (!sat_pack_bf_geometry(D0, D1, K, stride, layout - SAT_PREP_BF_MODE0, &p)) return false;
+        *g = SatPrepGeom{p.D1, p.K, p.S, p.ng, p.ng / p.cs, p.kv, p.m_v, p.v_v, p.out_pad, p.total};
+        return true;
+    }
+    if (layout == SAT_PREP_Q_MODE0 || layout == SAT_PREP_Q_MODE1) {
+        SatPackQParams p{};
+        if (stride != 1 || !sat_pack_q_geometry(D0, D1, K, layout - SAT_PREP_Q_MODE0, &p)) return false;
+        *g = SatPrepGeom{p.D1, p.K, 1, 2, 1, p.K, p.m_v, p.v_v, p.out_pad, p.total};
+        return true;
+    }
+    if (layout == SAT_PREP_K1T && D0 > 0 && D0 == D1 && K == 1 && stride == 1) {
+        *g = SatPrepGeom{D1, 1, 1, 1, 1, 1, D0, D0, D0, (long long)D0 * D0};
+        return true;
+    }
+    return false;
+}
 
 static int sat_bf_launch(const char* what, SatConvBfLaunch& a, const SatBfPlan& pl, void* stream) {
     if (pl.ng == 8 && pl.cs == 1 && a.sin_log2 == 0 && a.sout_log2 == 0) {
diff --git a/stable_audio_tools_amd/csrc/elementwise.hip b/stable_audio_tools_amd/csrc/elementwise.hip
--- a/stable_audio_tools_amd/csrc/elementwise.hip
+++ b/stable_audio_tools_amd/csrc/elementwise.hip
@@ -57,14 +57,6 @@
     float* dg;
     int D0, R;
 };
-
-SAT_DEVICE float sat_block_sum_256(float s, float* red) {
-    s = sat_wave_sum(s);
-    __syncthreads();
-    if ((threadIdx.x & 63) == 0) red[threadIdx.x >> 6] = s;
-    __syncthreads();
-    return red[0] + red[1] + red[2] + red[3];
-}
 
 __global__ void __launch_bounds__(256) sat_wn_fold_kernel(SatWnParams p) {
     __shared__ float red[4];
diff --git a/stable_audio_tools_amd/csrc/param_prep.h b/stable_audio_tools_amd/csrc/param_prep.h
--- /dev/null
+++ b/stable_audio_tools_amd/csrc/param_prep.h
@@ -0,0 +1,14 @@
+#pragma once
+
+#define SAT_PREP_BF_MODE0 0
+#define SAT_PREP_BF_MODE1 1
+#define SAT_PREP_BF_MODE2 2
+#define SAT_PREP_Q_MODE0 3
+#define SAT_PREP_Q_MODE1 4
+#define SAT_PREP_K1T 5
+
+struct SatPrepGeom {
+    int D1, K, S, ng, kt, kv, m_v, v_v, out_pad;
+    long long total;
+};
+bool sat_prep_pack_geometry(int layout, int D0, int D1, int K, int stride, SatPrepGeom* g);
diff --git a/stable_audio_tools_amd/csrc/param_prep.hip b/stable_audio_tools_amd/csrc/param_prep.hip
--- /dev/null
+++ b/stable_audio_tools_amd/csrc/param_prep.hip
@@ -0,0 +1,245 @@
+#include "sat_device.h"
+#include "param_prep.h"
+
+struct SatPrepFoldEntry { const float* v; const float* g; float* w; float* norm; long long D0, R; };
+struct SatPrepFoldArg { const float* v; const float* g; float* w; float* norm; unsigned R, block0; };
+#define SAT_PREP_FOLD_ARGS 96
+struct SatPrepFoldParams { SatPrepFoldArg e[SAT_PREP_FOLD_ARGS]; int nent; };
+static_assert(sizeof(SatPrepFoldParams) <= 4096, "kernel arguments are limited to 4 KiB");
+
+__global__ void __launch_bounds__(256) sat_prep_fold_kernel(SatPrepFoldParams p) {
+    __shared__ float red[4];
+    const unsigned b = blockIdx.x;
+    int lo = 0, hi = p.nent - 1;
+    while (lo < hi) {
+        const int mid = (lo + hi + 1) >> 1;
+        if (p.e[mid].block0 <= b) lo = mid;
+        else hi = mid - 1;
+    }
+    const int R = (int)p.e[lo].R;
+    const unsigned d = b - p.e[lo].block0;
+    const float* v = p.e[lo].v + (size_t)d * R;
+    float* w = p.e[lo].w + (size_t)d * R;
+    float s = 0.f;
+    for (int i = threadIdx.x; i < R; i += 256) s += v[i] * v[i];
+    s = sat_block_sum_256(s, red);
+    const float nrm = sqrtf(s);
+    const float sc = p.e[lo].g[d] / nrm;
+    if ((R & 3) == 0 && (((uintptr_t)v | (uintptr_t)w) & 15) == 0) {
+        const f32x4* v4 = reinterpret_cast<const f32x4*>(v);
+        f32x4* w4 = reinterpret_cast<f32x4*>(w);
+        for (int i = threadIdx.x; i < (R >> 2); i += 256) {
+            const f32x4 x = v4[i];
+            f32x4 y;
+            for (int j = 0; j < 4; ++j) y[j] = x[j] * sc;
+            w4[i] = y;
+        }
+    } else {
+        for (int i = threadIdx.x; i < R; i += 256) w[i] = v[i] * sc;
+    }
+    if (threadIdx.x == 0) p.e[lo].norm[d] = nrm;
+}
+
+extern "C" int sat_prep_fold(const void* entries, int nent, void* stream) {
+    if (nent <= 0) return 0;
+    if (!entries) { sat_set_error("sat_prep_fold: no table"); return 1; }
+    const SatPrepFoldEntry* tab = (const SatPrepFoldEntry*)entries;
+    for (int base = 0; base < nent; base += SAT_PREP_FOLD_ARGS) {
+        SatPrepFoldParams p;
+        const int cnt = nent - base < SAT_PREP_FOLD_ARGS ? nent - base : SAT_PREP_FOLD_ARGS;
+        unsigned blocks = 0;
+        int used = 0;
+        for (int i = 0; i < cnt; ++i) {
+            const SatPrepFoldEntry& e = tab[base + i];
+            if (e.D0 <= 0 || e.R <= 0) continue;
+            if (!e.v || !e.g || !e.w || !e.norm || e.R > 0x7fffffffLL || e.D0 > 0x7fffffffLL - (long long)blocks) {
+                sat_set_error("sat_prep_fold: bad entry");
+                return 1;
+            }
+            p.e[used] = SatPrepFoldArg{e.v, e.g, e.w, e.norm, (unsigned)e.R, blocks};
+            blocks += (unsigned)e.D0;
+            ++used;
+        }
+        if (!used) continue;
+        for (int i = used; i < SAT_PREP_FOLD_ARGS; ++i) p.e[i] = SatPrepFoldArg{nullptr, nullptr, nullptr, nullptr, 0u, 0u};
+        p.nent = used;
+        SAT_LAUNCH(sat_prep_fold_kernel, dim3(blocks), dim3(256), stream, p);
+        if (int rc = sat_check_launch("sat_prep_fold")) return rc;
+    }
+    return 0;
+}
+
+struct SatPrepSnakeEntry { const float* alpha; const float* beta; float* a; float* ib; long long C; };
+struct SatPrepSnakeArg { const float* alpha; const float* beta; float* a; float* ib; unsigned C, block0; };
+#define SAT_PREP_SNAKE_ARGS 96
+struct SatPrepSnakeParams { SatPrepSnakeArg e[SAT_PREP_SNAKE_ARGS]; int nent; };
+static_assert(sizeof(SatPrepSnakeParams) <= 4096, "kernel arguments are limited to 4 KiB");
+
+__global__ void __launch_bounds__(256) sat_prep_snake_kernel(SatPrepSnakeParams p) {
+    const unsigned b = blockIdx.x;
+    int lo = 0, hi = p.nent - 1;
+    while (lo < hi) {
+        const int mid = (lo + hi + 1) >> 1;
+        if (p.e[mid].block0 <= b) lo = mid;
+        else hi = mid - 1;
+    }
+    const unsigned i = (b - p.e[lo].block0) * 256 + threadIdx.x;
+    if (i >= p.e[lo].C) return;
+    p.e[lo].a[i] = expf(p.e[lo].alpha[i]);
+    p.e[lo].ib[i] = 1.0f / (expf(p.e[lo].beta[i]) + 1e-9f);
+}
+
+extern "C" int sat_prep_snake(const void* entries, int nent, void* stream) {
+    if (nent <= 0) return 0;
+    if (!entries) { sat_set_error("sat_prep_snake: no table"); return 1; }
+    const SatPrepSnakeEntry* tab = (const SatPrepSnakeEntry*)entries;
+    for (int base = 0; base < nent; base += SAT_PREP_SNAKE_ARGS) {
+        SatPrepSnakeParams p;
+        const int cnt = nent - base < SAT_PREP_SNAKE_ARGS ? nent - base : SAT_PREP_SNAKE_ARGS;
+        unsigned blocks = 0;
+        int used = 0;
+        for (int i = 0; i < cnt; ++i) {
+            const SatPrepSnakeEntry& e = tab[base + i];
+            if (e.C <= 0) continue;
+            if (!e.alpha || !e.beta || !e.a || !e.ib || e.C > 0x7fffffffLL) { sat_set_error("sat_prep_snake: bad entry"); return 1; }
+            p.e[used] = SatPrepSnakeArg{e.alpha, e.beta, e.a, e.ib, (unsigned)e.C, blocks};
+            blocks += (unsigned)((e.C + 255) / 256);
+            ++used;
+        }
+        if (!used) continue;
+        for (int i = used; i < SAT_PREP_SNAKE_ARGS; ++i) p.e[i] = SatPrepSnakeArg{nullptr, nullptr, nullptr, nullptr, 0u, 0u};
+        p.nent = used;
+        SAT_LAUNCH(sat_prep_snake_kernel, dim3(blocks), dim3(256), stream, p);
+        if (int rc = sat_check_launch("sat_prep_snake")) return rc;
+    }
+    return 0;
+}
+
+struct SatPrepPackEntry { const float* w; short* hi; short* lo; long long layout, D0, D1, K, stride; };
+struct SatPrepPackArg {
+    const float* w;
+    short* hi;
+    short* lo;
+    int D1, K, S, ng, kt, kv, m_v, v_v, out_pad, layout;
+    unsigned total, block0;
+};
+#define SAT_PREP_PACK_ARGS 56
+struct SatPrepPackParams { SatPrepPackArg e[SAT_PREP_PACK_ARGS]; int nent; };
+static_assert(sizeof(SatPrepPackParams) <= 4096, "kernel arguments are limited to 4 KiB");
+#define SAT_PREP_PACK_CHUNK 8192
+
+__global__ void __launch_bounds__(256) sat_prep_pack_kernel(SatPrepPackParams p) {
+    const unsigned b = blockIdx.x;
+    int lo = 0, hi = p.nent - 1;
+    while (lo < hi) {
+        const int mid = (lo + hi + 1) >> 1;
+        if (p.e[mid].block0 <= b) lo = mid;
+        else hi = mid - 1;
+    }
+    const SatPrepPackArg& a = p.e[lo];
+    const float* w = a.w;
+    const int D1 = a.D1, K = a.K, S = a.S, layout = a.layout;
+    const unsigned total = a.total;
+    const unsigned beg = (b - a.block0) * SAT_PREP_PACK_CHUNK;
+    for (unsigned o8 = beg + threadIdx.x * 8; o8 < beg + SAT_PREP_PACK_CHUNK && o8 < total; o8 += 256 * 8) {
+        float val[8];
+        unsigned q = o8 >> 3;
+        if (layout <= SAT_PREP_BF_MODE2) {
+            const int g = (int)(q % (unsigned)a.ng);
+            q /= (unsigned)a.ng;
+            const int m = (int)(q % (unsigned)a.out_pad), chunk = (int)(q / (unsigned)a.out_pad);
+            const int tap = g % a.kt, v0 = (chunk * (a.ng / a.kt) + g / a.kt) * 8;
+            const bool row_ok = tap < a.kv && m < a.m_v;
+            for (int e = 0; e < 8; ++e) {
+                const int v = v0 + e;
+                float x = 0.0f;
+                if (row_ok && v < a.v_v) {
+                    if (layout == SAT_PREP_BF_MODE0) x = w[((size_t)m * D1 + v / S) * K + tap * S + v % S];
+                    else if (layout == SAT_PREP_BF_MODE1) x = w[((size_t)v * D1 + m) * K + (K - 1 - tap)];
+                    else x = w[((size_t)v * D1 + m / S) * K + (m % S) + (tap == 0 ? S : 0)];
+                }
+                val[e] = x;
+            }
+        } else if (layout <= SAT_PREP_Q_MODE1) {
+            const int m = (int)(q % (unsigned)a.out_pad);
+            q /= (unsigned)a.out_pad;
+            const int g = (int)(q & 1u);
+            q >>= 1;
+            const int tap = (int)(q % (unsigned)K), chunk = (int)(q / (unsigned)K);
+            const int v0 = (chunk * 2 + g) * 8;
+            for (int e = 0; e < 8; ++e) {
+                const int v = v0 + e;
+                float x = 0.0f;
+                if (m < a.m_v && v < a.v_v) {
+                    if (layout == SAT_PREP_Q_MODE0) x = w[((size_t)m * D1 + v) * K + tap];
+                    else x = w[((size_t)v * D1 + m) * K + (K - 1 - tap)];
+                }
+                val[e] = x;
+            }
+        } else {
+            for (int e = 0; e < 8; ++e) {
+                const unsigned i = o8 + e;
+                float x = 0.0f;
+                if (i < total) {
+                    const unsigned ci = i / (unsigned)D1, co = i - ci * (unsigned)D1;
+                    x = w[(size_t)co * D1 + ci];
+                }
+                val[e] = x;
+            }
+        }
+        bf16x8 h, l;
+        for (int e = 0; e < 8; ++e) {
+            short hs, ls;
+            sat_split2(val[e], &hs, &ls);
+            h[e] = hs;
+            l[e] = ls;
+        }
+        if (o8 + 8 <= total) {
+            *reinterpret_cast<bf16x8*>(a.hi + o8) = h;
+            *reinterpret_cast<bf16x8*>(a.lo + o8) = l;
+        } else {
+            for (unsigned e = 0; o8 + e < total; ++e) {
+                a.hi[o8 + e] = h[e];
+                a.lo[o8 + e] = l[e];
+            }
+        }
+    }
+}
+
+extern "C" int sat_prep_pack(const void* entries, int nent, void* stream) {
+    if (nent <= 0) return 0;
+    if (!entries) { sat_set_error("sat_prep_pack: no table"); return 1; }
+    const SatPrepPackEntry* tab = (const SatPrepPackEntry*)entries;
+    for (int base = 0; base < nent; base += SAT_PREP_PACK_ARGS) {
+        SatPrepPackParams p;
+        const int cnt = nent - base < SAT_PREP_PACK_ARGS ? nent - base : SAT_PREP_PACK_ARGS;
+        unsigned blocks = 0;
+        int used = 0;
+        for (int i = 0; i < cnt; ++i) {
+            const SatPrepPackEntry& e = tab[base + i];
+            if (e.D0 == 0 || e.D1 == 0 || e.K == 0) continue;
+            SatPrepGeom g;
+            if (e.D0 < 0 || e.D1 < 0 || e.K < 0 || e.D0 > 0x7fffffffLL || e.D1 > 0x7fffffffLL || e.K > 0x7fffffffLL || e.stride > 0x7fffffffLL
+                    || !sat_prep_pack_geometry((int)e.layout, (int)e.D0, (int)e.D1, (int)e.K, (int)e.stride, &g)) {
+                sat_set_error("sat_prep_pack: an entry's layout does not serve its shape");
+                return 1;
+            }
+            const long long nb = sat_cdivll(g.total, SAT_PREP_PACK_CHUNK);
+            if (!e.w || !e.hi || !e.lo || ((((uintptr_t)e.hi) | ((uintptr_t)e.lo)) & 15) != 0 || g.total > 0x7fffffffLL
+                    || nb > 0x7fffffffLL - (long long)blocks) {
+                sat_set_error("sat_prep_pack: bad entry (null or unaligned planes, or more than 2^31 elements)");
+                return 1;
+            }
+            p.e[used] = SatPrepPackArg{e.w, e.hi, e.lo, g.D1, g.K, g.S, g.ng, g.kt, g.kv, g.m_v, g.v_v, g.out_pad, (int)e.layout,
+                                       (unsigned)g.total, blocks};
+            blocks += (unsigned)nb;
+            ++used;
+        }
+        if (!used) continue;
+        for (int i = used; i < SAT_PREP_PACK_ARGS; ++i) p.e[i] = SatPrepPackArg{nullptr, nullptr, nullptr, 1, 1, 1, 1, 1, 1, 0, 0, 1, 0, 0u, 0u};
+        p.nent = used;
+        SAT_LAUNCH(sat_prep_pack_kernel, dim3(blocks), dim3(256), stream, p);
+        if (int rc = sat_check_launch("sat_prep_pack")) return rc;
+    }
+    return 0;
+}
diff --git a/stable_audio_tools_amd/csrc/sat_device.h b/stable_audio_tools_amd/csrc/sat_device.h
--- a/stable_audio_tools_amd/csrc/sat_device.h
+++ b/stable_audio_tools_amd/csrc/sat_device.h
@@ -175,6 +175,12 @@
     return f;
 }
 
+SAT_DEVICE void sat_split2(float x, short* hi, short* lo) {
+    const short h = sat_f32_to_bf16(x);
+    *hi = h;
+    *lo = sat_f32_to_bf16(x - sat_bf16_to_f32(h));
+}
+
 SAT_DEVICE void sat_split2_pk(float a, float b, uint32_t* hi, uint32_t* lo) {
 #if defined(SAT_HIPEMU)
     const short ha = sat_f32_to_bf16(a), hb = sat_f32_to_bf16(b);
@@ -233,6 +239,13 @@
 SAT_DEVICE float sat_wave_sum(float v) {
     for (int m = 32; m >= 1; m >>= 1) v += __shfl_xor(v, m);
     return v;
+}
+SAT_DEVICE float sat_block_sum_256(float s, float* red) {
+    s = sat_wave_sum(s);
+    __syncthreads();
+    if ((threadIdx.x & 63) == 0) red[threadIdx.x >> 6] = s;
+    __syncthreads();
+    return red[0] + red[1] + red[2] + red[3];
 }
 SAT_DEVICE float sat_half_sum(float v) {
     for (int m = 16; m >= 1; m >>= 1) v += __shfl_xor(v, m);
diff --git a/stable_audio_tools_amd/functional.py b/stable_audio_tools_amd/functional.py
--- a/stable_audio_tools_amd/functional.py
+++ b/stable_audio_tools_amd/functional.py
@@ -33,7 +33,10 @@
     def __init__(self):
         self.items = {}
 
-    def get(self, name, sources, make):
+    def view(self):
+        return None
+
+    def get(self, name, sources, make, ops=None):
         from . import _caches
         if not _caches.trackable(*sources):
             return make()
@@ -45,8 +48,130 @@
         return hit[1]
 
 
-def _cached(cache, name, sources, make):
-    return make() if cache is None else cache.get(name, sources, make)
+def _cached(cache, name, sources, make, ops=None):
+    return make() if cache is None else cache.get(name, sources, make, ops)
+
+
+FOLD = ("fold",)
+SNAKE = ("snake",)
+K1T = ("k1t",)
+
+
+def _src_key(sources):
+    from . import _caches
+    return tuple((t.data_ptr(), _caches.version_of(t), t.device) for t in sources if t is not None) + _caches.epoch_of(*sources)
+
+
+class _PrepRequest:
+    __slots__ = ("name", "roots", "parent", "key", "ident", "value")
+
+    def __init__(self, name, roots, parent, key, value):
+        self.name, self.roots, self.parent, self.key, self.value = name, roots, parent, key, value
+        self.ident = tuple((t.data_ptr(), tuple(t.shape)) for t in roots)
+
+
+class ParamPlan:
+
+    def __init__(self):
+        self.reqs = {}
+        self.gen = {}
+
+    def __reduce__(self):
+        return (ParamPlan, ())
+
+    def slot(self, layer):
+        return PlanSlot(self, layer)
+
+    @staticmethod
+    def _batched(name, sources):
+        from . import _caches
+        return name[0] in ("fold", "snake", "bf", "q", "k1t") and _caches.trackable(*sources)
+
+    def _resolve(self, layer, name, sources, gen):
+        if name[0] in ("bf", "q", "k1t"):
+            fold = gen.get((layer, FOLD))
+            parent = self.reqs.get((layer, FOLD))
+            w = sources[0]
+            if fold is not None and parent is not None and fold[0].data_ptr() == w.data_ptr() and fold[0].shape == w.shape:
+                return parent.roots, parent
+        return tuple(sources), None
+
+    def request(self, layer, name, sources, make, ops):
+        if not self._batched(name, sources):
+            return make()
+        rid = (layer, name)
+        roots, parent = self._resolve(layer, name, sources, self.gen)
+        req = self.reqs.get(rid)
+        key = _src_key(roots)
+        if req is None or req.parent is not parent or req.ident != tuple((t.data_ptr(), tuple(t.shape)) for t in roots):
+            if name == FOLD:
+                for other in [r for r in self.reqs if r[0] == layer]:
+                    del self.reqs[other]
+                    self.gen.pop(other, None)
+            value = make()
+            self.reqs[rid] = _PrepRequest(name, roots, parent, key, value)
+            self.gen[rid] = value
+            return value
+        if req.key != key:
+            self.refresh(ops)
+        return req.value
+
+    def learn(self, view, name, sources, value):
+        if not self._batched(name, sources):
+            return
+        layer = view.slot.layer
+        roots, parent = self._resolve(layer, name, sources, view.gen)
+        current = view.gen is self.gen
+        key = None
+        if current:
+            key = parent.key if parent is not None else _src_key(roots)
+        self.reqs[(layer, name)] = _PrepRequest(name, roots, parent, key, value)
+        view.gen[(layer, name)] = value
+
+    def refresh(self, ops):
+        stale = [r for r in self.reqs.values() if r.key != _src_key(r.roots)]
+        folds = [r for r in stale if r.name == FOLD]
+        for r, value in zip(folds, ops.prep_fold([r.roots for r in folds])):
+            r.value = value
+        packs = [r for r in stale if r.name[0] in ("bf", "q", "k1t")]
+        items = []
+        for r in packs:
+            w = r.parent.value[0] if r.parent is not None else r.roots[0]
+            kind = r.name[0]
+            items.append((w.contiguous(), kind, r.name[1] if kind != "k1t" else 0, r.name[2] if kind == "bf" else 1))
+        for r, planes in zip(packs, ops.prep_pack(items)):
+            r.value = (*planes, "q") if r.name[0] == "q" and r.name[2] else planes
+        snakes = [r for r in stale if r.name == SNAKE]
+        for r, value in zip(snakes, ops.prep_snake([r.roots for r in snakes])):
+            r.value = value
+        for r in stale:
+            r.key = _src_key(r.roots)
+        self.gen = {rid: r.value for rid, r in self.reqs.items()}
+
+
+class PlanSlot:
+
+    def __init__(self, plan, layer):
+        self.plan, self.layer = plan, layer
+
+    def get(self, name, sources, make, ops=None):
+        return self.plan.request(self.layer, name, sources, make, _ops(ops))
+
+    def view(self):
+        return PlanView(self, self.plan.gen)
+
+
+class PlanView:
+
+    def __init__(self, slot, gen):
+        self.slot, self.gen = slot, gen
+
+    def get(self, name, sources, make, ops=None):
+        hit = self.gen.get((self.slot.layer, name))
+        if hit is None:
+            hit = make()
+            self.slot.plan.learn(self, name, sources, hit)
+        return hit
 
 
 class WeightNormFn(torch.autograd.Function):
@@ -68,22 +193,23 @@
         return dv, dg.view(ctx.g_shape), None
 
 
-def _conv_dgrad(ops, dy, w, k, stride, dil, pad, cin, tin, dsnake, res=None, out=None, emit=None):
+def _conv_dgrad(ops, dy, w, k, stride, dil, pad, cin, tin, dsnake, res=None, out=None, emit=None, cache=None):
     if stride == 1:
         if (res is None and out is None and not emit and ops.edge_ok(w.shape[0], cin, k, 1, dil, (k - 1) * dil - pad) and tin == dy.shape[2]
                 and (dsnake is None or w.shape[0] <= 2)):
             return ops.edge_conv(dy, w, (k - 1) * dil - pad, mode=1, dsnake=dsnake)
         if ops.bf16x3_ok(k, 1, dil):
             q = ops.k7q_applicable(w.shape[0], k, 1, dil, (k - 1) * dil - pad, cin)
-            return ops.conv1d_bf16x3(dy, ops.pack_bf16x3(w, mode=1, q=q), cin, k, 1, dil, (k - 1) * dil - pad, tout=tin,
+            planes = _cached(cache, ("q", 1, True) if q else ("bf", 1, 1), (w,), lambda: ops.pack_bf16x3(w, mode=1, q=q), ops)
+            return ops.conv1d_bf16x3(dy, planes, cin, k, 1, dil, (k - 1) * dil - pad, tout=tin,
                                      dsnake=dsnake, res=res, out=out, emit=emit)
         wpb = ops.pack(w, PACK_CONV_DGRAD)
         return ops.conv1d(dy, wpb, cin, k, 1, dil, (k - 1) * dil - pad, tout=tin, dsnake=dsnake, res=res, out=out)
     if out is not None:
         raise NotImplementedError("_conv_dgrad(out=...) is only plumbed through the stride-1 kernels")
     if ops.bf16x3_ok(k, stride, dil, transposed=True):
-        return ops.convtr1d_bf16x3(dy, ops.pack_bf16x3(w, mode=2, stride=stride), cin, k, stride, pad, tout=tin,
-                                   dsnake=dsnake, res=res)
+        planes = _cached(cache, ("bf", 2, stride), (w,), lambda: ops.pack_bf16x3(w, mode=2, stride=stride), ops)
+        return ops.convtr1d_bf16x3(dy, planes, cin, k, stride, pad, tout=tin, dsnake=dsnake, res=res)
     wpb = ops.pack(w, PACK_POLYPHASE, stride)
     return ops.convtr1d(dy, wpb, cin, k, stride, pad, tout=tin, dsnake=dsnake, res=res)
 
@@ -96,10 +222,10 @@
     return ops.conv_wgrad(dy, x, k, stride, dil, pad, snake=snake, snake_on=2, lo_rowsum=bias_grad, raw=raw)
 
 
-def _wn_forward(ops, v, g):
+def _wn_forward(ops, v, g, cache=None):
     v = v.contiguous()
     gf = g.contiguous().view(-1)
-    w, norm = ops.wn_fold(v, gf)
+    w, norm = _cached(cache if isinstance(cache, PlanSlot) else None, FOLD, (v, gf), lambda: ops.wn_fold(v, gf), ops)
     return w, (v, gf, norm)
 
 
@@ -117,12 +243,12 @@
         y = ops.edge_conv(x, w, pad, bias=bias, snake=snake, tanh_out=tanh_out, dsnake=dsnake, emit=emit)
     elif ops.bf16x3_ok(k, stride, dil):
         q = ops.k7q_applicable(cin, k, stride, dil, pad, cout)
-        planes = _cached(cache, "pack_fwd_q" if q else "pack_fwd", (w,), lambda: ops.pack_bf16x3(w, stride=stride, q=q))
-        sconsts = _cached(cache, "snake", snake, lambda: ops.snake_consts(snake[0], snake[1])) if snake is not None else None
+        planes = _cached(cache, ("q", 0, True) if q else ("bf", 0, stride), (w,), lambda: ops.pack_bf16x3(w, stride=stride, q=q), ops)
+        sconsts = _cached(cache, SNAKE, snake, lambda: ops.snake_consts(snake[0], snake[1]), ops) if snake is not None else None
         return ops.conv1d_bf16x3(x, planes, cout, k, stride, dil, pad, tout=tout, bias=bias,
                                  snake=snake, res=res, tanh_out=tanh_out, dsnake=dsnake, sconsts=sconsts, emit=emit, keep_planes=keep_planes)
     else:
-        y = ops.conv1d(x, _cached(cache, "pack_fwd32", (w,), lambda: ops.pack(w, PACK_CONV_FWD)), cout, k, stride, dil, pad, tout=tout,
+        y = ops.conv1d(x, _cached(cache, ("f32", PACK_CONV_FWD, 1), (w,), lambda: ops.pack(w, PACK_CONV_FWD)), cout, k, stride, dil, pad, tout=tout,
                        bias=bias, snake=snake, res=res, tanh_out=tanh_out, dsnake=dsnake)
     return (y, None) if keep_planes else y
 
@@ -130,11 +256,19 @@
 def _convtr_fwd(ops, x, w, stride, pad, bias=None, snake=None, cache=None):
     cin, cout, k = w.shape
     if ops.bf16x3_ok(k, stride, 1, transposed=True):
-        planes = _cached(cache, "pack_tr", (w,), lambda: ops.pack_bf16x3(w, mode=2, stride=stride))
-        sconsts = _cached(cache, "snake", snake, lambda: ops.snake_consts(snake[0], snake[1])) if snake is not None else None
+        planes = _cached(cache, ("bf", 2, stride), (w,), lambda: ops.pack_bf16x3(w, mode=2, stride=stride), ops)
+        sconsts = _cached(cache, SNAKE, snake, lambda: ops.snake_consts(snake[0], snake[1]), ops) if snake is not None else None
         return ops.convtr1d_bf16x3(x, planes, cout, k, stride, pad, bias=bias, snake=snake, sconsts=sconsts)
-    return ops.convtr1d(x, _cached(cache, "pack_tr32", (w,), lambda: ops.pack(w, PACK_POLYPHASE, stride)), cout, k, stride, pad,
+    return ops.convtr1d(x, _cached(cache, ("f32", PACK_POLYPHASE, stride), (w,), lambda: ops.pack(w, PACK_POLYPHASE, stride)), cout, k, stride, pad,
                         bias=bias, snake=snake)
+
+
+def _emit_for(ops, next_snake):
+    la, lb = next_snake[0].detach(), next_snake[1].detach()
+    slot = next_snake[3] if len(next_snake) > 3 else None
+    if isinstance(slot, PlanSlot):
+        return (la, lb, slot.get(SNAKE, (la, lb), lambda: ops.snake_consts(la, lb), ops))
+    return (la, lb)
 
 
 class SnakeConv1dFn(torch.autograd.Function):
@@ -145,7 +279,7 @@
         x = x.contiguous()
         wn = ()
         if g is not None:
-            w, wn = _wn_forward(ops, w, g)
+            w, wn = _wn_forward(ops, w, g, cache)
         w = w.contiguous()
         cout, cin, k = w.shape
         snake = (alpha.contiguous(), beta.contiguous()) if alpha is not None else None
@@ -154,12 +288,13 @@
             tout_ = (x.shape[2] + 2 * pad - dil * (k - 1) - 1) // stride + 1
             if ((ops.emit_ok(cout, k, stride, tout_, next_snake[2]) and ops.bf16x3_ok(k, stride, dil))
                     or (res is None and snake is None and ops.edge_emit_ok(cin, cout, k, stride, dil, pad, next_snake[2]))):
-                emit = (next_snake[0].detach(), next_snake[1].detach())
+                emit = _emit_for(ops, next_snake)
         y = _conv_fwd(ops, x, w, stride, dil, pad, bias=bias, snake=snake,
                       res=res.contiguous() if res is not None else None, tanh_out=tanh_out, cache=cache, emit=emit)
         ctx.ops = ops
         ctx.cfg = (stride, dil, pad, tanh_out, bias is not None, res is not None, alpha is not None)
         ctx.g_shape = g.shape if g is not None else None
+        ctx.prep = cache.view() if cache is not None else None
         ctx.save_for_backward(x, alpha, beta, w, y if tanh_out else None, *wn)
         return y
 
@@ -188,9 +323,9 @@
             dbias = ops.rowsum(dy)
         dx = da = db = None
         if has_snake:
-            dx, da, db = _conv_dgrad(ops, dy, w, k, stride, dil, pad, cin, x.shape[2], (x, alpha, beta))
+            dx, da, db = _conv_dgrad(ops, dy, w, k, stride, dil, pad, cin, x.shape[2], (x, alpha, beta), cache=ctx.prep)
         elif ctx.needs_input_grad[0]:
-            dx = _conv_dgrad(ops, dy, w, k, stride, dil, pad, cin, x.shape[2], None)
+            dx = _conv_dgrad(ops, dy, w, k, stride, dil, pad, cin, x.shape[2], None, cache=ctx.prep)
         return dx, da, db, dw, dbias, dres, None, None, None, None, None, None, None, dg
 
 
@@ -202,7 +337,7 @@
         x = x.contiguous()
         wn = ()
         if g is not None:
-            w, wn = _wn_forward(ops, w, g)
+            w, wn = _wn_forward(ops, w, g, cache)
         w = w.contiguous()
         cin, cout, k = w.shape
         snake = (alpha.contiguous(), beta.contiguous()) if alpha is not None else None
@@ -210,6 +345,7 @@
         ctx.ops = ops
         ctx.cfg = (stride, pad, bias is not None, alpha is not None)
         ctx.g_shape = g.shape if g is not None else None
+        ctx.prep = cache.view() if cache is not None else None
         ctx.save_for_backward(x, alpha, beta, w, *wn)
         return y
 
@@ -229,9 +365,9 @@
             dw, dg = _wn_backward(ops, dw, wn, ctx.g_shape)
         dx = da = db = None
         if has_snake:
-            dx, da, db = _conv_fwd(ops, dy, w, stride, 1, pad, dsnake=(x, alpha, beta), tout=x.shape[2])
+            dx, da, db = _conv_fwd(ops, dy, w, stride, 1, pad, dsnake=(x, alpha, beta), tout=x.shape[2], cache=ctx.prep)
         elif ctx.needs_input_grad[0]:
-            dx = _conv_fwd(ops, dy, w, stride, 1, pad, tout=x.shape[2])
+            dx = _conv_fwd(ops, dy, w, stride, 1, pad, tout=x.shape[2], cache=ctx.prep)
         return dx, da, db, dw, dbias, None, None, None, None, dg
 
 
@@ -243,25 +379,25 @@
         ops = _ops(ops)
         x = x.contiguous()
         wn1 = wn2 = ()
+        c1, c2 = caches if caches is not None else (None, None)
         if g1 is not None:
-            w1, wn1 = _wn_forward(ops, w1, g1)
+            w1, wn1 = _wn_forward(ops, w1, g1, c1)
         if g2 is not None:
-            w2, wn2 = _wn_forward(ops, w2, g2)
+            w2, wn2 = _wn_forward(ops, w2, g2, c2)
         w1 = w1.contiguous()
         w2 = w2.contiguous()
         c = x.shape[1]
         k1 = w1.shape[2]
         pad = dil * (k1 - 1) // 2
-        c1, c2 = caches if caches is not None else (None, None)
         emit = ctx.k7_planes = None
         if next_snake is not None and ops.emit_ok(c, w2.shape[2], 1, x.shape[2], next_snake[2]):
-            emit = (next_snake[0].detach(), next_snake[1].detach())
+            emit = _emit_for(ops, next_snake)
         if fuse and w2.shape[2] == 1 and w1.shape[0] == c and ops.ru_fused_ok(c, k1, dil, x.shape[2]):
-            w7q = _cached(c1, "pack_q7", (w1,), lambda: ops.pack_k7q(w1))
-            w1q = _cached(c2, "pack_q1", (w2,), lambda: ops.pack_k7q(w2))
+            w7q = _cached(c1, ("q", 0, False), (w1,), lambda: ops.pack_k7q(w1), ops)
+            w1q = _cached(c2, ("q", 0, False), (w2,), lambda: ops.pack_k7q(w2), ops)
             sc = None
             if c1 is not None and c2 is not None:
-                sc = (_cached(c1, "snake", (a1, b1), lambda: ops.snake_consts(a1, b1)), _cached(c2, "snake", (a2, b2), lambda: ops.snake_consts(a2, b2)))
+                sc = (_cached(c1, SNAKE, (a1, b1), lambda: ops.snake_consts(a1, b1), ops), _cached(c2, SNAKE, (a2, b2), lambda: ops.snake_consts(a2, b2), ops))
             h, y = ops.residual_unit_fwd(x, (a1, b1), w7q, bias1, (a2, b2), w1q, bias2, k1, dil, keep_h=ctx is not None and not recompute and fuse != "nokeep",
                                          emit=emit, sconsts=sc)
         else:
@@ -274,6 +410,7 @@
         ctx.dil = dil
         ctx.recompute = bool(recompute)
         ctx.g_shapes = (g1.shape if g1 is not None else None, g2.shape if g2 is not None else None)
+        ctx.prep = (c1.view() if c1 is not None else None, c2.view() if c2 is not None else None)
         ctx.save_for_backward(x, None if recompute else h, a1, b1, w1, a2, b2, w2, bias1 if recompute else None, *wn1, *wn2)
         return y
 
@@ -291,8 +428,9 @@
         pad1 = dil * (k1 - 1) // 2
         t = x.shape[2]
         dy = dy.contiguous()
+        p1, p2 = ctx.prep
         if ctx.recompute:
-            h = _conv_fwd(ops, x, w1, 1, dil, pad1, bias=bias1, snake=(a1, b1))
+            h = _conv_fwd(ops, x, w1, 1, dil, pad1, bias=bias1, snake=(a1, b1), cache=p1)
         want_emit = ops.emit_ok(w1.shape[0], k2, 1, t, dil) and ops.k7q_applicable(w1.shape[0], k1, 1, dil, pad1, c)
         kept = ctx.k7_planes if not ctx.recompute and want_emit and ops.kept_planes_valid(ctx.k7_planes, x, (a1, b1), dil, pad1) else None
         skip_dh = False
@@ -304,16 +442,17 @@
             return (dw, ops.rowsum(dh, partial=bool(wn1))) if bias_grad else dw
         if k2 == 1 and w2.shape[0] == c and w1.shape[0] == c and ops.ru_k1_bwd_ok(dy.shape[0], c, t):
             skip_dh = bool(kept is not None and ops.ru_k1_bwd_skip_dh)
-            dh, da2, db2, dw2, dbias2, dbias1 = ops.ru_k1_bwd(dy, h, w2, (a2, b2), emit=want_emit, raw=bool(wn2), skip_dh=skip_dh)
+            wt = _cached(p2, K1T, (w2,), lambda: ops.ru_k1_pack(w2), ops)
+            dh, da2, db2, dw2, dbias2, dbias1 = ops.ru_k1_bwd(dy, h, w2, (a2, b2), emit=want_emit, wt=wt, raw=bool(wn2), skip_dh=skip_dh)
             try:
                 dw1 = wgrad1(dh, False)
                 if skip_dh:
-                    dx, da1, db1 = _conv_dgrad(ops, dh, w1, k1, 1, dil, pad1, c, t, (x, a1, b1), res=dy)
+                    dx, da1, db1 = _conv_dgrad(ops, dh, w1, k1, 1, dil, pad1, c, t, (x, a1, b1), res=dy, cache=p1)
             finally:
                 ops.dh_written()
         else:
             dw2, dbias2 = ops.conv_wgrad(dy, h, k2, 1, 1, 0, snake=(a2, b2), snake_on=2, lo_rowsum=True, raw=bool(wn2))
-            dh, da2, db2 = _conv_dgrad(ops, dy, w2, k2, 1, 1, 0, c, t, (h, a2, b2), emit=want_emit)
+            dh, da2, db2 = _conv_dgrad(ops, dy, w2, k2, 1, 1, 0, c, t, (h, a2, b2), emit=want_emit, cache=p2)
             dw1, dbias1 = wgrad1(dh, True)
         dg1 = dg2 = None
         if wn1:
@@ -327,7 +466,7 @@
             else:
                 dw2, dg2 = _wn_backward(ops, dw2, wn2, gs2)
         if not skip_dh:
-            dx, da1, db1 = _conv_dgrad(ops, dh, w1, k1, 1, dil, pad1, c, t, (x, a1, b1), res=dy)
+            dx, da1, db1 = _conv_dgrad(ops, dh, w1, k1, 1, dil, pad1, c, t, (x, a1, b1), res=dy, cache=p1)
         return dx, da1, db1, dw1, dbias1, da2, db2, dw2, dbias2, None, None, None, None, None, None, dg1, dg2
 
 
diff --git a/stable_audio_tools_amd/ops.py b/stable_audio_tools_amd/ops.py
--- a/stable_audio_tools_amd/ops.py
+++ b/stable_audio_tools_amd/ops.py
@@ -370,14 +370,14 @@
     def _emit_args(self, emit, b, c, t, device, st, consts=True, owned=True):
         if not emit:
             return self._NO_PLANES, None, None
-        snake = None if emit is True else emit
-        ea, eb = (None, None) if snake is None else self.snake_consts(*snake) if consts else snake
+        snake = None if emit is True else tuple(emit[:2])
+        ea, eb = (None, None) if snake is None else snake if not consts else emit[2] if len(emit) > 2 else self.snake_consts(*snake)
         self._f32(ea, eb)
         return self._emit_planes(b, c, t, device, st, owner=snake if owned else None), ea, eb
 
     def _emit_done(self, emit, y, planes):
         if emit:
-            snake = None if emit is True else emit
+            snake = None if emit is True else tuple(emit[:2])
             self._emitted = planes.of(y, snake) if _caches.trackable(y, *(snake or ())) else None
 
     def _take_emitted(self, x, snake, peek=False):
@@ -1420,6 +1420,69 @@
             tab[i] = (src.data_ptr(), dst.data_ptr(), src.numel())
         self._chk(self.lib.sat_multi_copy(tab.ctypes.data, n, self._stream(srcs[0])))
 
+    param_prep = True
+
+    @staticmethod
+    def _prep_slices(sizes, dtype, device):
+        al = 512 // torch.empty((), dtype=dtype).element_size()
+        offs, n = [], 0
+        for s in sizes:
+            offs.append(n)
+            n += -(-s // al) * al
+        buf = torch.empty(n, dtype=dtype, device=device)
+        return [buf[o:o + s] for o, s in zip(offs, sizes)]
+
+    def _prep_launch(self, fn, rows, like):
+        import numpy as np
+        tab = np.array(rows, dtype=np.int64)
+        self._chk(fn(tab.ctypes.data, len(rows), self._stream(like)))
+
+    def prep_fold(self, pairs):
+        if not pairs:
+            return []
+        for v, g in pairs:
+            self._f32(v, g)
+        dev = pairs[0][0].device
+        out = self._prep_slices([v.numel() for v, _ in pairs] + [v.shape[0] for v, _ in pairs], torch.float32, dev)
+        ws, norms = [w.view(v.shape) for w, (v, _) in zip(out, pairs)], out[len(pairs):]
+        self._prep_launch(self.lib.sat_prep_fold, [(v.data_ptr(), g.data_ptr(), w.data_ptr(), nrm.data_ptr(), v.shape[0], v.numel() // max(v.shape[0], 1))
+                                                   for (v, g), w, nrm in zip(pairs, ws, norms)], pairs[0][0])
+        return list(zip(ws, norms))
+
+    def prep_snake(self, pairs):
+        if not pairs:
+            return []
+        for al, be in pairs:
+            self._f32(al, be)
+        out = self._prep_slices([t.numel() for pair in pairs for t in pair], torch.float32, pairs[0][0].device)
+        res = [(out[2 * i].view(al.shape), out[2 * i + 1].view(be.shape)) for i, (al, be) in enumerate(pairs)]
+        self._prep_launch(self.lib.sat_prep_snake, [(al.data_ptr(), be.data_ptr(), a.data_ptr(), ib.data_ptr(), al.numel())
+                                                    for (al, be), (a, ib) in zip(pairs, res)], pairs[0][0])
+        return res
+
+    PREP_LAYOUTS = {("bf", 0): 0, ("bf", 1): 1, ("bf", 2): 2, ("q", 0): 3, ("q", 1): 4, ("k1t", 0): 5}
+
+    def prep_pack(self, items):
+        if not items:
+            return []
+        sizes = []
+        for w, kind, mode, stride in items:
+            self._f32(w)
+            d0, d1, k = w.shape
+            if kind == "bf":
+                n = self.lib.sat_pack_weights_bf16x3_size(d0, d1, k, stride, mode)
+            elif kind == "q":
+                n = self.lib.sat_pack_weights_k7q_size(d0, d1, k, mode) if stride == 1 else -1
+            else:
+                n = d0 * d1 if (kind, mode, k, stride) == ("k1t", 0, 1, 1) and d0 == d1 else -1
+            if n <= 0:
+                raise RuntimeError("prep_pack: layout %s does not serve a %s weight" % ((kind, mode, stride), tuple(w.shape)))
+            sizes += [n, n]
+        out = self._prep_slices(sizes, torch.int16, items[0][0].device)
+        self._prep_launch(self.lib.sat_prep_pack, [(w.data_ptr(), out[2 * i].data_ptr(), out[2 * i + 1].data_ptr(), self.PREP_LAYOUTS[(kind, mode)], *w.shape, stride)
+                                                   for i, (w, kind, mode, stride) in enumerate(items)], items[0][0])
+        return [(out[2 * i], out[2 * i + 1]) for i in range(len(items))]
+
     def adamw_step(self, p, g, m, v, lr, beta1, beta2, eps, weight_decay, step, grad_scale=1.0, ema=None, ema_decay=0.0):
         self._f32(p, g, m, v, ema)
         self._chk(self.lib.sat_adamw_step(_ptr(p), _ptr(g), _ptr(m), _ptr(v), p.numel(), lr, beta1, beta2, eps,
```

After: 8.189, median of 6. About the same (+0.5%).
